# glmanhtu/vit-ed

Hardware: AMD Instinct MI355X
Metric: patch-pairs/sec fwd+bwd, div2k_erosion7_4bin_patch8_64 ViT-ED (higher is better)
Workload: dtype bf16

## Files before the change

include/vited.h:

```cpp
#ifndef VITED_H
#define VITED_H

#include <stdint.h>

#ifdef __cplusplus
extern "C" {
#endif

#define VITED_ABI_VERSION 1

#define VITED_OK 0
#define VITED_ERR_BAD_ARG 1
#define VITED_ERR_UNSUPPORTED 2
#define VITED_ERR_LAUNCH 3
#define VITED_ERR_WORKSPACE 4

#define VITED_F32 0
#define VITED_BF16 1
#define VITED_F16 2
#define VITED_I32 3
#define VITED_I64 4

#define VITED_EPI_STORE 0
#define VITED_EPI_GELU 1
#define VITED_EPI_RESIDUAL 2
#define VITED_EPI_MUL_GELU_GRAD 3
#define VITED_EPI_STORE_F32 4
#define VITED_EPI_MUL 5
#define VITED_EPI_GELU_GRAD 6

#define VITED_B_NK 0
#define VITED_B_KN 1

int vited_abi_version(void);
const char* vited_strerror(int code);

int vited_last_gemm_path(void);
int vited_last_attention_path(void);


int vited_cast(const void* src, int src_dtype, void* dst, int dst_dtype, int64_t n, void* stream);

int vited_cast_transpose(const float* src, void* dst, int dst_dtype, int64_t rows, int64_t cols, void* stream);

int vited_cast_weights(const int64_t* desc, int count, int64_t total_tiles, void* stream);

int vited_patchify(const float* img, int64_t img_bs, const int64_t* batch_index, void* out, int out_dtype,
                   int64_t batch, int chans, int img_size, int patch, void* stream);

int vited_patchify_u8(const uint8_t* img, int64_t img_bs, const int64_t* batch_index, void* out, int out_dtype,
                      int64_t batch, int chans, int img_size, int patch, const float* mean, const float* std, void* stream);

int vited_crop_pairs_u8(const uint8_t* src, int64_t src_bs, const int* cells, const int* erode, uint8_t* out, int64_t batch,
                        int chans, int img_size, void* stream);

int vited_div2k_regions_u8(const uint8_t* store, const int64_t* img_off, const int* img_hw, int n_images, const int* image,
                           const int* flags, const double* minv, const float* rgb, const int* crop, uint8_t* out, int64_t batch,
                           int img_size, void* stream);

int vited_hisfrag_windows_u8(const uint8_t* store, const int64_t* img_off, const int* img_hw, int n_images, const int* image,
                             const int* flags, const int64_t* afix, const double* minv, const int* origin, uint8_t* out, int64_t batch,
                             int img_size, void* stream);

int vited_hisfrag_jitter_u8(const uint8_t* in, const int* flags, const int* order, const float* factors, const int* hue, int64_t* sums,
                            uint8_t* out, int64_t batch, int img_size, void* stream);

int vited_hisfrag_blur_u8(const uint8_t* in, const int* flags, const float* weights, uint8_t* out, int64_t batch, int img_size,
                          void* stream);

int vited_michigan_windows_u8(const uint8_t* store, const int64_t* img_off, const int* img_hw, int n_images, const int* image,
                              const int* flags, const int* origin, const int* x0, const int* kx, const int* y0, const int* ky,
                              const int* holes, const int* n_holes, uint8_t* out, int64_t batch, int img_size, void* stream);

int vited_michigan_blur_gray_u8(const uint8_t* in, const int* flags, const int* weights, uint8_t* out, int64_t batch, int img_size,
                                void* stream);

int vited_slice_rows_cast(const float* in, void* out, int out_dtype, int64_t batch, int64_t in_rows,
                          int64_t row_offset, int64_t rows, int64_t dim, void* stream);

int vited_write_cls_row(float* x, const float* cls, const float* pos, int64_t batch, int64_t rows_per_batch,
                        int64_t dim, void* stream);

int64_t vited_sum_rows_workspace_bytes(int64_t batch, int64_t width);
int vited_sum_rows(const void* in, int in_dtype, int64_t in_ld, float* out, int64_t batch, int64_t width,
                   float* workspace, int64_t workspace_bytes, void* stream);


int vited_layernorm_fwd(const float* x, int64_t x_ld, const float* gamma, const float* beta, void* y,
                        int y_dtype, int64_t y_ld, float* mean, float* rstd, int64_t rows, int64_t dim,
                        float eps, void* stream);

int64_t vited_layernorm_bwd_workspace_bytes(int64_t rows, int64_t dim);
int vited_layernorm_bwd(const void* dy, int dy_dtype, int64_t dy_ld, const float* x, int64_t x_ld,
                        const float* gamma, const float* mean, const float* rstd, const float* dx_in,
                        int64_t dx_in_ld, float* dx_out, int64_t dx_out_ld, void* dx_lp, int dx_lp_dtype,
                        int64_t dx_lp_ld, float* dgamma, float* dbeta, int accumulate, int64_t rows, int64_t dim,
                        float* workspace, int64_t workspace_bytes, void* stream);

int vited_layernorm_bwd_scaled(const void* dy, int dy_dtype, int64_t dy_ld, const float* x, int64_t x_ld,
                               const float* gamma, const float* mean, const float* rstd, const float* dx_in,
                               int64_t dx_in_ld, float* dx_out, int64_t dx_out_ld, void* dx_lp, int dx_lp_dtype,
                               int64_t dx_lp_ld, const float* lp_scale, float* dgamma, float* dbeta, int accumulate,
                               int64_t rows, int64_t dim, float* workspace, int64_t workspace_bytes, void* stream);

int vited_scale_rows_cast(const float* src, int64_t src_ld, const float* row_scale, void* dst, int dst_dtype, int64_t dst_ld,
                          int64_t rows, int64_t dim, void* stream);


int vited_gemm(const void* A, int64_t lda, const void* B, int64_t ldb, int b_layout, int dtype, int64_t M,
               int64_t N, int64_t K, int epilogue, const float* bias, const void* aux,
               const float* residual, void* out, void* out2, int64_t ldo, int64_t rows_per_batch,
               int64_t out_rows_per_batch, int64_t row_offset, int residual_bcast, void* stream);

int vited_gemm_scaled(const void* A, int64_t lda, const void* B, int64_t ldb, int b_layout, int dtype, int64_t M, int64_t N,
                      int64_t K, const float* bias, const float* residual, const float* row_scale, float* out, int64_t ldo,
                      void* stream);

int64_t vited_linear_bwd_weight_workspace_bytes(int64_t M, int64_t N, int64_t K);
int vited_linear_bwd_weight(const void* dY, int64_t lddy, const void* X, int64_t ldx, int dtype, int64_t M,
                            int64_t N, int64_t K, float* dW, float* dbias, int accumulate, float* workspace,
                            int64_t workspace_bytes, void* stream);

int vited_linear_bwd_weight_batched_supported(int count, const int64_t* M, const int64_t* N, const int64_t* K, int dtype);
int64_t vited_linear_bwd_weight_batched_workspace_bytes(int count, const int64_t* M, const int64_t* N, const int64_t* K);
int vited_linear_bwd_weight_batched(int count, const void* const* dY, const int64_t* lddy, const void* const* X,
                                    const int64_t* ldx, const int64_t* M, const int64_t* N, const int64_t* K, float* const* dW,
                                    float* const* dbias, int dtype, int accumulate, float* workspace, int64_t workspace_bytes,
                                    void* stream);

int vited_linear_layernorm_supported(int64_t M, int64_t N, int64_t K);

int vited_linear_residual_layernorm_fwd(const void* a, int64_t lda, const void* w, int64_t ldw, const float* bias,
                                        const float* residual, int64_t ldr, float* y, int64_t ldy, const float* gamma,
                                        const float* beta, float eps, void* h, int64_t ldh, float* mean, float* rstd,
                                        int64_t M, int64_t N, int64_t K, void* stream);

int vited_linear_residual_layernorm_fwd_scaled(const void* a, int64_t lda, const void* w, int64_t ldw, const float* bias,
                                               const float* residual, int64_t ldr, const float* row_scale, float* y, int64_t ldy,
                                               const float* gamma, const float* beta, float eps, void* h, int64_t ldh, float* mean,
                                               float* rstd, int64_t M, int64_t N, int64_t K, void* stream);

int vited_linear_layernorm_bwd_segmented(const void* dy, int64_t lddy, int64_t seg_k, int64_t seg_stride, int64_t segments,
                                         const void* wt, int64_t ldwt, const float* x, int64_t ldx, const float* gamma,
                                         const float* mean, const float* rstd, const float* dx_in, int64_t dx_in_ld,
                                         float* dx_out, int64_t dx_out_ld, void* dx_lp, int64_t dx_lp_ld, float* dgamma,
                                         float* dbeta, int accumulate, int64_t M, int64_t N, float* workspace,
                                         int64_t workspace_bytes, void* stream);
int64_t vited_linear_layernorm_bwd_partial_rows(int64_t M);
int vited_layernorm_bwd_finish_batched(int count, const float* const* partial, const int* nparts, float* const* dgamma,
                                       float* const* dbeta, const int* accumulate, int64_t dim, void* stream);
int64_t vited_linear_layernorm_bwd_workspace_bytes(int64_t M, int64_t N);
int vited_linear_layernorm_bwd(const void* dy, int64_t lddy, const void* wt, int64_t ldwt, const float* x, int64_t ldx,
                               const float* gamma, const float* mean, const float* rstd, const float* dx_in,
                               int64_t dx_in_ld, float* dx_out, int64_t dx_out_ld, void* dx_lp, int64_t dx_lp_ld,
                               float* dgamma, float* dbeta, int accumulate, int64_t M, int64_t N, int64_t K,
                               float* workspace, int64_t workspace_bytes, void* stream);

int vited_linear_layernorm_bwd_scaled(const void* dy, int64_t lddy, const void* wt, int64_t ldwt, const float* x, int64_t ldx,
                                      const float* gamma, const float* mean, const float* rstd, const float* dx_in,
                                      int64_t dx_in_ld, float* dx_out, int64_t dx_out_ld, void* dx_lp, int64_t dx_lp_ld,
                                      const float* lp_scale, float* dgamma, float* dbeta, int accumulate, int64_t M, int64_t N,
                                      int64_t K, float* workspace, int64_t workspace_bytes, void* stream);

int vited_fold_context_weights(int count, const float* const* w, const float* const* bias, const float* const* gamma,
                               const float* const* beta, int64_t N, int64_t K, void* w_out, void* wt_out, float* bias_out,
                               void* stream);
int vited_unfold_context_grads(int count, const float* dwf, const float* dbf, const float* const* w, const float* const* gamma,
                               const float* const* beta, float* const* dw, float* const* dbias, float* const* dgamma, float* const* dbeta, int64_t N,
                               int64_t K, int accumulate, void* stream);


int vited_mlp_fwd(const float* x, int64_t ldx, const float* gamma, const float* beta, const void* w1, const float* b1,
                  const void* w2, const float* b2, float* y, int64_t ldy, void* h, void* gd, void* u, float* mean,
                  float* rstd, int64_t rows, int64_t dim, int64_t hidden, float eps, void* stream);

int64_t vited_block_workspace_bytes(int64_t batch, int64_t tokens, int64_t dim, int64_t hidden, int heads);
int vited_block_fwd(const float* x, float* y, int64_t batch, int64_t tokens, int64_t dim, int heads, int64_t hidden,
                    const float* ln1_g, const float* ln1_b, const void* wqkv, const float* bqkv, const void* wproj,
                    const float* bproj, const float* ln2_g, const float* ln2_b, const void* w1, const float* b1,
                    const void* w2, const float* b2, float eps, void* workspace, int64_t workspace_bytes, void* stream);

int64_t vited_cross_block_workspace_bytes(int64_t batch, int64_t tokens, int64_t ctx_tokens, int64_t dim, int64_t hidden, int heads);
int vited_cross_block_fwd(const float* x, const float* context, float* y, int64_t batch, int64_t tokens, int64_t ctx_tokens,
                          int64_t dim, int heads, int64_t hidden, const float* ln1_g, const float* ln1_b, const void* wqkv,
                          const float* bqkv, const void* wproj, const float* bproj, const float* lnq_g, const float* lnq_b,
                          const float* lnc_g, const float* lnc_b, const void* wq, const float* bq, const void* wkv,
                          const float* bkv, const void* wcproj, const float* bcproj, const float* ln2_g, const float* ln2_b,
                          const void* w1, const float* b1, const void* w2, const float* b2, float eps, void* workspace,
                          int64_t workspace_bytes, void* stream);


int64_t vited_adamw_workspace_bytes(void);
int vited_adamw_step(const int64_t* desc, int count, int64_t total_tiles, const float* grad_flat, int64_t grad_numel,
                     float* hyper, float max_norm, int zero_grad, float* norm_out, float* workspace,
                     int64_t workspace_bytes, void* stream);

int vited_sgd_step(const int64_t* desc, int count, int64_t total_tiles, const float* grad_flat, int64_t grad_numel,
                   float* hyper, float max_norm, int zero_grad, float* norm_out, float* workspace,
                   int64_t workspace_bytes, void* stream);


int vited_attention_fwd(const void* q, int64_t q_bs, int64_t q_ts, const void* k, int64_t k_bs, int64_t k_ts,
                        const void* v, int64_t v_bs, int64_t v_ts, void* o, int64_t o_bs, int64_t o_ts,
                        float* lse, int dtype, int64_t batch, int heads, int64_t nq, int64_t nk, int head_dim,
                        float scale, void* stream);

int vited_attention_fwd_indexed(const void* q, int64_t q_bs, int64_t q_ts, const void* k, int64_t k_bs, int64_t k_ts,
                                const void* v, int64_t v_bs, int64_t v_ts, const int64_t* kv_index, void* o, int64_t o_bs,
                                int64_t o_ts, float* lse, int dtype, int64_t batch, int heads, int64_t nq, int64_t nk,
                                int head_dim, float scale, void* stream);

int vited_attention_bwd(const void* q, int64_t q_bs, int64_t q_ts, const void* k, int64_t k_bs, int64_t k_ts,
                        const void* v, int64_t v_bs, int64_t v_ts, const void* o, const void* d_o,
                        int64_t o_bs, int64_t o_ts, const float* lse, float* delta, void* dq, int64_t dq_bs,
                        int64_t dq_ts, void* dk, int64_t dk_bs, int64_t dk_ts, void* dv, int64_t dv_bs,
                        int64_t dv_ts, int dtype, int64_t batch, int heads, int64_t nq, int64_t nk,
                        int head_dim, float scale, void* stream);

int64_t vited_attention_bwd_indexed_workspace_bytes(int dtype, int64_t batch, int heads, int64_t nk, int head_dim);
int vited_attention_bwd_indexed(const void* q, int64_t q_bs, int64_t q_ts, const void* k, int64_t k_bs, int64_t k_ts,
                                const void* v, int64_t v_bs, int64_t v_ts, const int64_t* kv_index, const int64_t* seg_order,
                                const int64_t* seg_offsets, int64_t kv_items, const void* o, const void* d_o, int64_t o_bs,
                                int64_t o_ts, const float* lse, float* delta, void* dq, int64_t dq_bs, int64_t dq_ts, void* dk,
                                int64_t dk_bs, int64_t dk_ts, void* dv, int64_t dv_bs, int64_t dv_ts, int dtype, int64_t batch,
                                int heads, int64_t nq, int64_t nk, int head_dim, float scale, void* workspace,
                                int64_t workspace_bytes, void* stream);

enum { VITED_CAM_GRAD = 0, VITED_CAM_PROB = 1 };
int vited_attention_cam(const void* q, int64_t q_bs, int64_t q_ts, const void* k, int64_t k_bs, int64_t k_ts,
                        const void* v, int64_t v_bs, int64_t v_ts, const void* d_o, int64_t do_bs, int64_t do_ts,
                        const float* lse, const float* head_weight, float* cam, int64_t cam_bs, int64_t cam_ld,
                        int mode, int dtype, int64_t batch, int heads, int64_t nq, int64_t nk, int head_dim,
                        float scale, void* stream);


int vited_retrieval_metrics(const void* D, int dtype, int64_t ld, int64_t n, int64_t r0, int64_t r1, const int* labels,
                            const int* offsets, const int* members, int num_classes, int remove_self_column, int from_similarity,
                            double* rows_out, double* sums, void* stream);


int vited_group_retrieval_metrics(const void* D, int dtype, int64_t ld, int64_t n, int64_t r0, int64_t r1, const int* labels,
                                  int num_labels, const int* col_offsets, const int* col_members, const int* pos_offsets,
                                  const int* pos_labels, const int* neg_offsets, const int* neg_labels, const int* ks, int nk,
                                  double* rows_out, double* sums, void* stream);


// ... 29 lines not shown
```

vit-ed_amd/csrc/context_fold.hip:

```cpp
#include "common.h"

#define CF_MAX_BLOCKS 16

struct FoldArgs {
    const float* w[CF_MAX_BLOCKS];
    const float* bias[CF_MAX_BLOCKS];
    const float* gamma[CF_MAX_BLOCKS];
    const float* beta[CF_MAX_BLOCKS];
    bf16* w_out;
    bf16* wt_out;
    float* bias_out;
    int count, N, K;
};

__global__ void __launch_bounds__(256) fold_context_kernel(const FoldArgs a) {
    const int lane = threadIdx.x & 63;
    const int row = blockIdx.x * 4 + (threadIdx.x >> 6);
    if (row >= a.count * a.N) return;
    const int l = row / a.N, n = row - l * a.N;
    const float* __restrict__ w = a.w[l] + (int64_t)n * a.K;
    const float* __restrict__ g = a.gamma[l];
    const float* __restrict__ be = a.beta[l];
    const int64_t ldt = (int64_t)a.count * a.N;
    float dot = 0.f;
    for (int k = lane; k < a.K; k += 64) {
        const float wv = w[k];
        const bf16 f = (bf16)(wv * g[k]);
        a.w_out[(int64_t)row * a.K + k] = f;
        a.wt_out[(int64_t)k * ldt + row] = f;
        dot = fmaf(wv, be[k], dot);
    }
    dot = wave_sum(dot);
    if (lane == 0) a.bias_out[row] = dot + (a.bias[l] ? a.bias[l][n] : 0.f);
}

extern "C" int vited_fold_context_weights(int count, const float* const* w, const float* const* bias, const float* const* gamma,
                                          const float* const* beta, int64_t N, int64_t K, void* w_out, void* wt_out, float* bias_out,
                                          void* stream) {
    if (count < 1 || count > CF_MAX_BLOCKS || !w || !bias || !gamma || !beta || !w_out || !wt_out || !bias_out || N <= 0 || K <= 0)
        return VITED_ERR_BAD_ARG;
    FoldArgs a = {};
    for (int i = 0; i < count; ++i) {
        if (!w[i] || !gamma[i] || !beta[i]) return VITED_ERR_BAD_ARG;
        a.w[i] = w[i]; a.bias[i] = bias[i]; a.gamma[i] = gamma[i]; a.beta[i] = beta[i];
    }
    a.w_out = (bf16*)w_out; a.wt_out = (bf16*)wt_out; a.bias_out = bias_out;
    a.count = count; a.N = (int)N; a.K = (int)K;
    hipLaunchKernelGGL(fold_context_kernel, dim3((unsigned)ceil_div64((int64_t)count * N, 4)), dim3(256), 0, (hipStream_t)stream, a);
    return vited_check_launch();
}

struct UnfoldArgs {
    const float* w[CF_MAX_BLOCKS];
    const float* gamma[CF_MAX_BLOCKS];
    const float* beta[CF_MAX_BLOCKS];
    float* dw[CF_MAX_BLOCKS];
    float* dbias[CF_MAX_BLOCKS];
    float* dgamma[CF_MAX_BLOCKS];
    float* dbeta[CF_MAX_BLOCKS];
    const float* dwf;
    const float* dbf;
    int count, N, K, accumulate;
};

#define UF_GROUPS 16
__global__ void __launch_bounds__(64 * UF_GROUPS) unfold_context_kernel(const UnfoldArgs a) {
    __shared__ float red[2][UF_GROUPS][64];
    const int l = blockIdx.y, kx = threadIdx.x & 63, ng = threadIdx.x >> 6;
    const int k = blockIdx.x * 64 + kx;
    const bool ok = k < a.K;
    const float* __restrict__ w = a.w[l];
    const float* __restrict__ dwf = a.dwf + (int64_t)l * a.N * a.K;
    const float* __restrict__ dbf = a.dbf + (int64_t)l * a.N;
    float* __restrict__ dw = a.dw[l];
    const float g = ok ? a.gamma[l][k] : 0.f, be = ok ? a.beta[l][k] : 0.f;
    float sg = 0.f, sb = 0.f;
#pragma unroll 4
    for (int n = ng; n < a.N; n += UF_GROUPS) {
        if (ok) {
            const int64_t o = (int64_t)n * a.K + k;
            const float d = dwf[o], wv = w[o], dbn = dbf[n];
            sg = fmaf(d, wv, sg);
            sb = fmaf(dbn, wv, sb);
            const float v = fmaf(d, g, dbn * be);
            dw[o] = a.accumulate ? dw[o] + v : v;
        }
    }
    red[0][ng][kx] = sg;
    red[1][ng][kx] = sb;
    __syncthreads();
    if (ng == 0 && ok) {
        float tg = 0.f, tb = 0.f;
#pragma unroll
        for (int w = 0; w < UF_GROUPS; ++w) {
            tg += red[0][w][kx];
            tb += red[1][w][kx];
        }
        a.dgamma[l][k] = a.accumulate ? a.dgamma[l][k] + tg : tg;
        a.dbeta[l][k] = a.accumulate ? a.dbeta[l][k] + tb : tb;
    }
    if (blockIdx.x == 0 && a.dbias[l]) {
        for (int n = threadIdx.x; n < a.N; n += 64 * UF_GROUPS) a.dbias[l][n] = a.accumulate ? a.dbias[l][n] + dbf[n] : dbf[n];
    }
}

extern "C" int vited_unfold_context_grads(int count, const float* dwf, const float* dbf, const float* const* w, const float* const* gamma,
                                          const float* const* beta, float* const* dw, float* const* dbias, float* const* dgamma, float* const* dbeta, int64_t N,
                                          int64_t K, int accumulate, void* stream) {
    if (count < 1 || count > CF_MAX_BLOCKS || !dwf || !dbf || !w || !gamma || !beta || !dw || !dbias || !dgamma || !dbeta || N <= 0 || K <= 0)
        return VITED_ERR_BAD_ARG;
    UnfoldArgs a = {};
    for (int i = 0; i < count; ++i) {
        if (!w[i] || !gamma[i] || !beta[i] || !dw[i] || !dgamma[i] || !dbeta[i]) return VITED_ERR_BAD_ARG;
        a.w[i] = w[i]; a.gamma[i] = gamma[i]; a.beta[i] = beta[i]; a.dw[i] = dw[i]; a.dbias[i] = dbias[i]; a.dgamma[i] = dgamma[i]; a.dbeta[i] = dbeta[i];
    }
    a.dwf = dwf; a.dbf = dbf; a.count = count; a.N = (int)N; a.K = (int)K; a.accumulate = accumulate;
    hipLaunchKernelGGL(unfold_context_kernel, dim3((unsigned)ceil_div64(K, 64), (unsigned)count), dim3(64 * UF_GROUPS), 0, (hipStream_t)stream, a);
    return vited_check_launch();
}
```

vit-ed_amd/csrc/elementwise.hip:

```cpp
#include "common.h"

template <typename S, typename D>
__global__ void cast_kernel(const S* __restrict__ src, D* __restrict__ dst, int64_t n) {
    int64_t i = ((int64_t)blockIdx.x * blockDim.x + threadIdx.x) * 4;
    const int64_t stride = (int64_t)gridDim.x * blockDim.x * 4;
    for (; i + 3 < n; i += stride) {
        S a = src[i], b = src[i + 1], c = src[i + 2], d = src[i + 3];
        dst[i] = from_f32<D>(to_f32(a));
        dst[i + 1] = from_f32<D>(to_f32(b));
        dst[i + 2] = from_f32<D>(to_f32(c));
        dst[i + 3] = from_f32<D>(to_f32(d));
    }
    for (; i < n; ++i) dst[i] = from_f32<D>(to_f32(src[i]));
}

extern "C" int vited_cast(const void* src, int src_dtype, void* dst, int dst_dtype, int64_t n, void* stream) {
    if (!src || !dst || n < 0) return VITED_ERR_BAD_ARG;
    if (n == 0) return VITED_OK;
    hipStream_t s = (hipStream_t)stream;
    const int threads = 256;
    int64_t blocks = ceil_div64(n, threads * 4);
    if (blocks > 4096) blocks = 4096;
    if (src_dtype == VITED_F32 && dst_dtype == VITED_BF16)
        hipLaunchKernelGGL((cast_kernel<float, bf16>), dim3(blocks), dim3(threads), 0, s, (const float*)src, (bf16*)dst, n);
// ... 84 lines not shown
        const int mid = (lo + hi + 1) >> 1;
        if (desc[(int64_t)mid * WS_DESC_WORDS + 5] <= blk) lo = mid; else hi = mid - 1;
    }
    const int64_t* d = desc + (int64_t)lo * WS_DESC_WORDS;
    const float* __restrict__ src = (const float*)d[0];
    bf16* __restrict__ dst = (bf16*)d[1];
    bf16* __restrict__ dst_t = (bf16*)d[2];
    const int64_t rows = d[3], cols = d[4];
    const int64_t t = blk - d[5], tiles_c = (cols + 63) >> 6;
    const int64_t r0 = (t / tiles_c) << 6, c0 = (t % tiles_c) << 6;
    const int tx = threadIdx.x & 15, ty = threadIdx.x >> 4;
    const bool vec = (cols & 3) == 0;
#pragma unroll
    for (int j = 0; j < 4; ++j) {
        const int lr = ty + 16 * j;
        const int64_t r = r0 + lr, c = c0 + tx * 4;
        float v[4] = {0.f, 0.f, 0.f, 0.f};
        if (r < rows) {
            if (vec && c + 3 < cols) {
                const f32x4 q = *(const f32x4*)(src + r * cols + c);
                v[0] = q[0]; v[1] = q[1]; v[2] = q[2]; v[3] = q[3];
            } else {
#pragma unroll
                for (int e = 0; e < 4; ++e) if (c + e < cols) v[e] = src[r * cols + c + e];
            }
        }
        bf16 b[4];
#pragma unroll
        for (int e = 0; e < 4; ++e) { b[e] = (bf16)v[e]; tile[lr][tx * 4 + e] = b[e]; }
        if (dst && r < rows) {
            if (vec && c + 3 < cols) *(bf16x4*)(dst + r * cols + c) = bf16x4{b[0], b[1], b[2], b[3]};
            else {
#pragma unroll
                for (int e = 0; e < 4; ++e) if (c + e < cols) dst[r * cols + c + e] = b[e];
            }
        }
    }
    if (!dst_t) return;
    __syncthreads();
    const bool vec_t = (rows & 3) == 0;
#pragma unroll
    for (int j = 0; j < 4; ++j) {
        const int lc = ty + 16 * j;
        const int64_t c = c0 + lc, r = r0 + tx * 4;
        if (c >= cols) continue;
        bf16 b[4];
#pragma unroll
        for (int e = 0; e < 4; ++e) b[e] = tile[tx * 4 + e][lc];
        if (vec_t && r + 3 < rows) *(bf16x4*)(dst_t + c * rows + r) = bf16x4{b[0], b[1], b[2], b[3]};
        else {
#pragma unroll
            for (int e = 0; e < 4; ++e) if (r + e < rows) dst_t[c * rows + r + e] = b[e];
        }
    }
}

extern "C" int vited_cast_weights(const int64_t* desc, int count, int64_t total_tiles, void* stream) {
    if (!desc || count <= 0 || total_tiles <= 0 || total_tiles > 0x7fffffff) return VITED_ERR_BAD_ARG;
    hipLaunchKernelGGL(cast_weights_kernel, dim3((unsigned)total_tiles), dim3(256), 0, (hipStream_t)stream, desc, count);
    return vited_check_launch();
}

template <typename D>
__global__ void patchify_kernel(const float* __restrict__ img, int64_t img_bs, const int64_t* __restrict__ bidx,
                                D* __restrict__ out, int chans, int S, int p) {
    const int G = S / p;
    const int64_t b = blockIdx.y;
    const int py = blockIdx.x;
    const int64_t src_b = bidx ? bidx[b] : b;
    const float* base = img + src_b * img_bs;
    const int Kp = chans * p * p;
    const int total = chans * p * S;
    D* obase = out + (b * G * G + (int64_t)py * G) * Kp;
    for (int e = threadIdx.x; e < total; e += blockDim.x) {
        const int x = e % S;
        const int ci = e / S;
        const int i = ci % p, c = ci / p;
        const float v = base[((int64_t)c * S + (py * p + i)) * S + x];
        const int px = x / p, j = x - px * p;
        obase[(int64_t)px * Kp + (c * p + i) * p + j] = from_f32<D>(v);
    }
}

extern "C" int vited_patchify(const float* img, int64_t img_bs, const int64_t* batch_index, void* out, int out_dtype,
                              int64_t batch, int chans, int img_size, int patch, void* stream) {
    if (!img || !out || batch <= 0 || chans <= 0 || img_size <= 0 || patch <= 0 || img_size % patch) return VITED_ERR_BAD_ARG;
    dim3 grid(img_size / patch, (unsigned)batch);
    hipStream_t s = (hipStream_t)stream;
    if (out_dtype == VITED_BF16)
        hipLaunchKernelGGL((patchify_kernel<bf16>), grid, dim3(256), 0, s, img, img_bs, batch_index, (bf16*)out, chans, img_size, patch);
    else if (out_dtype == VITED_F32)
        hipLaunchKernelGGL((patchify_kernel<float>), grid, dim3(256), 0, s, img, img_bs, batch_index, (float*)out, chans, img_size, patch);
    else
        return VITED_ERR_UNSUPPORTED;
    return vited_check_launch();
}

struct U8Norm { float scale[4], shift[4]; };

template <typename D>
__global__ void patchify_u8_kernel(const uint8_t* __restrict__ img, int64_t img_bs, const int64_t* __restrict__ bidx,
                                   D* __restrict__ out, int chans, int S, int p, U8Norm nrm) {
    const int G = S / p;
    const int64_t b = blockIdx.y;
    const int py = blockIdx.x;
    const int64_t src_b = bidx ? bidx[b] : b;
    const uint8_t* base = img + src_b * img_bs;
    const int Kp = chans * p * p;
    const int total = chans * p * S;
    D* obase = out + (b * G * G + (int64_t)py * G) * Kp;
    for (int e = threadIdx.x; e < total; e += blockDim.x) {
        const int x = e % S;
        const int ci = e / S;
        const int i = ci % p, c = ci / p;
        const float v = fmaf((float)base[((int64_t)c * S + (py * p + i)) * S + x], nrm.scale[c], nrm.shift[c]);
        const int px = x / p, j = x - px * p;
        obase[(int64_t)px * Kp + (c * p + i) * p + j] = from_f32<D>(v);
    }
}

extern "C" int vited_patchify_u8(const uint8_t* img, int64_t img_bs, const int64_t* batch_index, void* out, int out_dtype,
                                 int64_t batch, int chans, int img_size, int patch, const float* mean, const float* std,
                                 void* stream) {
    if (!img || !out || !mean || !std || batch <= 0 || chans <= 0 || chans > 4 || img_size <= 0 || patch <= 0 || img_size % patch)
        return VITED_ERR_BAD_ARG;
    U8Norm nrm = {};
    for (int c = 0; c < chans; ++c) {
        if (!(std[c] > 0.f)) return VITED_ERR_BAD_ARG;
        nrm.scale[c] = 1.0f / (255.0f * std[c]);
        nrm.shift[c] = -mean[c] / std[c];
    }
    dim3 grid(img_size / patch, (unsigned)batch);
    hipStream_t s = (hipStream_t)stream;
    if (out_dtype == VITED_BF16)
        hipLaunchKernelGGL((patchify_u8_kernel<bf16>), grid, dim3(256), 0, s, img, img_bs, batch_index, (bf16*)out, chans, img_size, patch, nrm);
    else if (out_dtype == VITED_F32)
        hipLaunchKernelGGL((patchify_u8_kernel<float>), grid, dim3(256), 0, s, img, img_bs, batch_index, (float*)out, chans, img_size, patch, nrm);
    else
        return VITED_ERR_UNSUPPORTED;
    return vited_check_launch();
}

struct ResampleTaps {
    int x0, n;
    int k0, k1;
};

__device__ __forceinline__ ResampleTaps resample_taps(int xx, int in_size, int out_size) {
    constexpr int PRECISION_BITS = 32 - 8 - 2;
    const double scale = (double)in_size / (double)out_size;
    const double center = (xx + 0.5) * scale;
    int xmin = (int)(center - 1.0 + 0.5);
    xmin = xmin < 0 ? 0 : xmin;
    int xmax = (int)(center + 1.0 + 0.5);
    xmax = (xmax < in_size ? xmax : in_size) - xmin;
    double w0 = 1.0 - fabs((double)xmin - center + 0.5), w1 = xmax > 1 ? 1.0 - fabs((double)xmin + 1.0 - center + 0.5) : 0.0;
    w0 = w0 < 0.0 ? 0.0 : w0;
    w1 = w1 < 0.0 ? 0.0 : w1;
    const double ww = w0 + w1;
    ResampleTaps t;
    t.x0 = xmin;
    t.n = xmax > 1 ? 2 : 1;
    t.k0 = (int)(0.5 + (w0 / ww) * (double)(1 << PRECISION_BITS));
    t.k1 = (int)(0.5 + (w1 / ww) * (double)(1 << PRECISION_BITS));
    return t;
}

__device__ __forceinline__ int resample_px(int p0, int p1, const ResampleTaps& t) {
    constexpr int PRECISION_BITS = 32 - 8 - 2;
    int acc = (1 << (PRECISION_BITS - 1)) + p0 * t.k0 + (t.n > 1 ? p1 * t.k1 : 0);
    acc >>= PRECISION_BITS;
    return acc < 0 ? 0 : (acc > 255 ? 255 : acc);
}

__global__ void __launch_bounds__(256)
crop_pairs_u8_kernel(const uint8_t* __restrict__ src, int64_t src_bs, const int* __restrict__ cells, const int* __restrict__ erode,
                     uint8_t* __restrict__ out, int chans, int S) {
    const int64_t b = blockIdx.z;
    const int img = blockIdx.y / chans, c = blockIdx.y % chans;
    int cell = cells[b * 2 + img], e = erode[b];
    cell = cell < 0 ? 0 : (cell > 5 ? 5 : cell);
    e = e < 1 ? 1 : (e > S ? S : e);
    const int off = (int)rint((S - e) / 2.0);
    const int r0 = (cell / 3) * S + off, c0 = (cell % 3) * S + off;
    const uint8_t* base = src + b * src_bs + ((int64_t)c * 2 * S + r0) * (3 * S) + c0;
    uint8_t* o = out + (((b * 2 + img) * chans + c) * (int64_t)S) * S;
    for (int i = blockIdx.x * blockDim.x + threadIdx.x; i < S * S; i += gridDim.x * blockDim.x) {
        const int y = i / S, x = i - y * S;
        const ResampleTaps tx = resample_taps(x, e, S), ty = resample_taps(y, e, S);
        const uint8_t* ra = base + (int64_t)ty.x0 * (3 * S) + tx.x0;
        const int h0 = resample_px(ra[0], tx.n > 1 ? ra[1] : 0, tx);
        int h1 = 0;
        if (ty.n > 1) {
            const uint8_t* rb = ra + 3 * S;
            h1 = resample_px(rb[0], tx.n > 1 ? rb[1] : 0, tx);
        }
        o[i] = (uint8_t)resample_px(h0, h1, ty);
    }
}

extern "C" int vited_crop_pairs_u8(const uint8_t* src, int64_t src_bs, const int* cells, const int* erode, uint8_t* out, int64_t batch,
                                   int chans, int img_size, void* stream) {
    if (!src || !cells || !erode || !out || batch <= 0 || chans <= 0 || img_size <= 0 || batch > 65535) return VITED_ERR_BAD_ARG;
    if (src_bs < (int64_t)chans * 6 * img_size * img_size) return VITED_ERR_BAD_ARG;
    const int per = img_size * img_size;
    dim3 grid((unsigned)((per + 1023) / 1024 < 8 ? (per + 1023) / 1024 : 8), (unsigned)(2 * chans), (unsigned)batch);
    hipLaunchKernelGGL(crop_pairs_u8_kernel, grid, dim3(256), 0, (hipStream_t)stream, src, src_bs, cells, erode, out, chans, img_size);
    return vited_check_launch();
}

template <typename D>
__global__ void slice_rows_cast_kernel(const float* __restrict__ in, D* __restrict__ out, int64_t in_rows,
                                       int64_t row_offset, int64_t rows, int64_t dim, int64_t total) {
    int64_t i = (int64_t)blockIdx.x * blockDim.x + threadIdx.x;
    const int64_t stride = (int64_t)gridDim.x * blockDim.x;
    const int64_t per_b = rows * dim;
    for (; i < total; i += stride) {
        const int64_t b = i / per_b, rem = i - b * per_b;
        out[i] = from_f32<D>(in[(b * in_rows + row_offset) * dim + rem]);
    }
}

extern "C" int vited_slice_rows_cast(const float* in, void* out, int out_dtype, int64_t batch, int64_t in_rows,
                                     int64_t row_offset, int64_t rows, int64_t dim, void* stream) {
    if (!in || !out || batch <= 0 || rows <= 0 || dim <= 0 || row_offset < 0 || row_offset + rows > in_rows) return VITED_ERR_BAD_ARG;
    const int64_t total = batch * rows * dim;
    int64_t blocks = ceil_div64(total, 256);
    if (blocks > 8192) blocks = 8192;
    hipStream_t s = (hipStream_t)stream;
    if (out_dtype == VITED_BF16)
        hipLaunchKernelGGL((slice_rows_cast_kernel<bf16>), dim3(blocks), dim3(256), 0, s, in, (bf16*)out, in_rows, row_offset, rows, dim, total);
    else if (out_dtype == VITED_F32)
        hipLaunchKernelGGL((slice_rows_cast_kernel<float>), dim3(blocks), dim3(256), 0, s, in, (float*)out, in_rows, row_offset, rows, dim, total);
    else
        return VITED_ERR_UNSUPPORTED;
    return vited_check_launch();
}

__global__ void write_cls_row_kernel(float* __restrict__ x, const float* __restrict__ cls, const float* __restrict__ pos,
                                     int64_t batch, int64_t rows_per_batch, int64_t dim) {
    int64_t i = (int64_t)blockIdx.x * blockDim.x + threadIdx.x;
    const int64_t total = batch * dim;
    if (i >= total) return;
    const int64_t b = i / dim, d = i - b * dim;
    x[b * rows_per_batch * dim + d] = cls[d] + pos[d];
}

extern "C" int vited_write_cls_row(float* x, const float* cls, const float* pos, int64_t batch, int64_t rows_per_batch,
                                   int64_t dim, void* stream) {
    if (!x || !cls || !pos || batch <= 0 || rows_per_batch <= 0 || dim <= 0) return VITED_ERR_BAD_ARG;
    const int64_t total = batch * dim;
    hipLaunchKernelGGL(write_cls_row_kernel, dim3((unsigned)ceil_div64(total, 256)), dim3(256), 0, (hipStream_t)stream,
                       x, cls, pos, batch, rows_per_batch, dim);
    return vited_check_launch();
}

template <typename S_>
__global__ void sum_rows_kernel(const S_* __restrict__ in, int64_t in_ld, float* __restrict__ out, int64_t batch,
                                int64_t width, int64_t rows_per_split) {
    const int64_t r = (int64_t)blockIdx.x * blockDim.x + threadIdx.x;
    if (r >= width) return;
    const int64_t b0 = (int64_t)blockIdx.y * rows_per_split;
    int64_t b1 = b0 + rows_per_split;
    if (b1 > batch) b1 = batch;
    float acc0 = 0.f, acc1 = 0.f, acc2 = 0.f, acc3 = 0.f;
    int64_t b = b0;
    for (; b + 3 < b1; b += 4) {
        acc0 += to_f32(in[b * in_ld + r]);
        acc1 += to_f32(in[(b + 1) * in_ld + r]);
        acc2 += to_f32(in[(b + 2) * in_ld + r]);
        acc3 += to_f32(in[(b + 3) * in_ld + r]);
    }
    for (; b < b1; ++b) acc0 += to_f32(in[b * in_ld + r]);
    out[(int64_t)blockIdx.y * width + r] = (acc0 + acc1) + (acc2 + acc3);
}

static inline int64_t sum_rows_splits(int64_t batch, int64_t width) {
    const int64_t col_blocks = ceil_div64(width, 256);
    int64_t s = ceil_div64(1024, col_blocks);
    const int64_t max_s = ceil_div64(batch, 16);
    if (s > max_s) s = max_s;
    if (s < 1) s = 1;
    return s;
}

extern "C" int64_t vited_sum_rows_workspace_bytes(int64_t batch, int64_t width) {
    return sum_rows_splits(batch, width) * width * (int64_t)sizeof(float);
}

extern "C" int vited_sum_rows(const void* in, int in_dtype, int64_t in_ld, float* out, int64_t batch, int64_t width,
                              float* workspace, int64_t workspace_bytes, void* stream) {
    if (!in || !out || batch <= 0 || width <= 0 || in_ld < width) return VITED_ERR_BAD_ARG;
    const int64_t S = sum_rows_splits(batch, width);
    hipStream_t s = (hipStream_t)stream;
    const unsigned col_blocks = (unsigned)ceil_div64(width, 256);
    float* pass1_out = out;
    if (S > 1) {
        if (!workspace || workspace_bytes < S * width * (int64_t)sizeof(float)) return VITED_ERR_WORKSPACE;
        pass1_out = workspace;
    }
    const int64_t rps = ceil_div64(batch, S);
    if (in_dtype == VITED_F32)
        hipLaunchKernelGGL((sum_rows_kernel<float>), dim3(col_blocks, (unsigned)S), dim3(256), 0, s, (const float*)in, in_ld, pass1_out, batch, width, rps);
    else if (in_dtype == VITED_BF16)
        hipLaunchKernelGGL((sum_rows_kernel<bf16>), dim3(col_blocks, (unsigned)S), dim3(256), 0, s, (const bf16*)in, in_ld, pass1_out, batch, width, rps);
    else
        return VITED_ERR_UNSUPPORTED;
    if (S > 1)
        hipLaunchKernelGGL((sum_rows_kernel<float>), dim3(col_blocks, 1), dim3(256), 0, s, (const float*)workspace, width, out, S, width, S);
    return vited_check_launch();
}

__device__ __forceinline__ void sum_slabs_body(const float* __restrict__ in, int64_t in_ld, float* __restrict__ out, int64_t batch,
                                               int64_t width, int accumulate, int64_t r) {
    if (r >= width) return;
    if (r + 3 < width) {
        f32x4 acc = accumulate ? *(const f32x4*)(out + r) : f32x4{0.f, 0.f, 0.f, 0.f};
        int64_t b = 0;
        for (; b + 4 <= batch; b += 4) {
// ... 133 lines not shown
```

vit-ed_amd/csrc/gemm.hip:

```cpp
#include <stdlib.h>
#include <string.h>

#include "gemm_kernels.h"

static thread_local int g_last_gemm_path = 0;
extern "C" int vited_last_gemm_path(void) { return g_last_gemm_path; }

static int gemm_impl(const void* A, int64_t lda, const void* B, int64_t ldb, int b_layout, int dtype, int64_t M, int64_t N, int64_t K,
                     int epilogue, const float* bias, const void* aux, const float* residual, void* out, void* out2, int64_t ldo,
                     int64_t rows_per_batch, int64_t out_rows_per_batch, int64_t row_offset, int residual_bcast,
                     const float* row_scale, void* stream) {
    if (!A || !B || !out || M <= 0 || N <= 0 || K <= 0 || lda < K || ldo < N) return VITED_ERR_BAD_ARG;
    if (b_layout != VITED_B_NK && b_layout != VITED_B_KN) return VITED_ERR_BAD_ARG;
    if (ldb < (b_layout == VITED_B_NK ? K : N)) return VITED_ERR_BAD_ARG;
    if (epilogue < VITED_EPI_STORE || epilogue > VITED_EPI_GELU_GRAD) return VITED_ERR_BAD_ARG;
    if ((epilogue == VITED_EPI_GELU || epilogue == VITED_EPI_GELU_GRAD) && !out2) return VITED_ERR_BAD_ARG;
    if (epilogue == VITED_EPI_RESIDUAL && !residual) return VITED_ERR_BAD_ARG;
    if ((epilogue == VITED_EPI_MUL_GELU_GRAD || epilogue == VITED_EPI_MUL) && !aux) return VITED_ERR_BAD_ARG;
    if (rows_per_batch < 0 || (rows_per_batch > 0 && (out_rows_per_batch < rows_per_batch + row_offset || row_offset < 0)))
        return VITED_ERR_BAD_ARG;
    if (row_scale) {
        if (epilogue != VITED_EPI_RESIDUAL || rows_per_batch != 0) return VITED_ERR_BAD_ARG;
        epilogue = EPI_RESIDUAL_SCALED;
    }
// ... 47 lines not shown

extern "C" int64_t vited_linear_bwd_weight_workspace_bytes(int64_t M, int64_t N, int64_t K) {
    const int64_t s = max64(tn_portable_splits(M, N, K), gemm_tn_mfma_splits(M, N, K));
    return (s * N * K + s * N + N) * (int64_t)sizeof(float) + vited_sum_rows_workspace_bytes(M, N) + 256;
}

extern "C" int vited_linear_bwd_weight(const void* dY, int64_t lddy, const void* X, int64_t ldx, int dtype, int64_t M,
                                       int64_t N, int64_t K, float* dW, float* dbias, int accumulate, float* workspace,
                                       int64_t workspace_bytes, void* stream) {
    if (!dY || !X || !dW || M <= 0 || N <= 0 || K <= 0 || lddy < N || ldx < K) return VITED_ERR_BAD_ARG;
    if (dtype != VITED_F32 && dtype != VITED_BF16) return VITED_ERR_UNSUPPORTED;
    if (!workspace || workspace_bytes < vited_linear_bwd_weight_workspace_bytes(M, N, K)) return VITED_ERR_WORKSPACE;
    hipStream_t s = (hipStream_t)stream;
    const bool mfma = dtype == VITED_BF16 && gemm_tn_mfma_supported(dY, lddy, X, ldx, M, N, K);
    const int64_t splits = mfma ? gemm_tn_mfma_splits(M, N, K) : tn_portable_splits(M, N, K);
    const bool via_slabs = splits > 1 || accumulate;
    float* slab = via_slabs ? workspace : dW;
    float* bias_tmp = workspace + splits * N * K;
    int rc;
    if (mfma) {
        g_last_gemm_path = 2;
        float* bias_slab = !dbias ? nullptr : (via_slabs ? bias_tmp : dbias);
        rc = gemm_tn_mfma(dY, lddy, X, ldx, M, N, K, splits, slab, bias_slab, s);
        if (rc != VITED_OK) return rc;
        if (via_slabs) {
            rc = dbias ? sum_slabs_pair(workspace, N * K, dW, N * K, bias_slab, N, dbias, N, splits, s, accumulate)
                       : sum_rows_f32_single_pass(workspace, N * K, dW, splits, N * K, s, accumulate);
        }
        return rc;
    }
    g_last_gemm_path = 1;
    rc = gemm_tn_portable(dY, lddy, X, ldx, dtype, M, N, K, splits, slab, s);
    if (rc != VITED_OK) return rc;
    if (via_slabs) {
        rc = sum_rows_f32_single_pass(workspace, N * K, dW, splits, N * K, s, accumulate);
        if (rc != VITED_OK) return rc;
    }
    if (dbias) {
        float* ws2 = bias_tmp + N;
        const int64_t ws2_bytes = workspace_bytes - (splits * N * K + N) * (int64_t)sizeof(float);
        if (accumulate) {
            rc = vited_sum_rows(dY, dtype, lddy, bias_tmp, M, N, ws2, ws2_bytes, stream);
            if (rc == VITED_OK) rc = sum_rows_f32_single_pass(bias_tmp, N, dbias, 1, N, s, 1);
        } else {
            rc = vited_sum_rows(dY, dtype, lddy, dbias, M, N, ws2, ws2_bytes, stream);
        }
    }
    return rc;
}

extern "C" int vited_linear_bwd_weight_batched_supported(int count, const int64_t* M, const int64_t* N, const int64_t* K, int dtype) {
    return dtype == VITED_BF16 && gemm_tn_batch_supported(count, M, N, K) ? 1 : 0;
}

extern "C" int64_t vited_linear_bwd_weight_batched_workspace_bytes(int count, const int64_t* M, const int64_t* N, const int64_t* K) {
    if (!gemm_tn_batch_supported(count, M, N, K)) return 0;
    int64_t splits, ws, bs;
    gemm_tn_batch_layout(count, M, N, K, &splits, &ws, &bs);
    return splits * (ws + bs) * (int64_t)sizeof(float) + 256;
}

extern "C" int vited_linear_bwd_weight_batched(int count, const void* const* dY, const int64_t* lddy, const void* const* X,
                                               const int64_t* ldx, const int64_t* M, const int64_t* N, const int64_t* K,
                                               float* const* dW, float* const* dbias, int dtype, int accumulate, float* workspace,
                                               int64_t workspace_bytes, void* stream) {
    if (count < 1 || !dY || !lddy || !X || !ldx || !M || !N || !K || !dW || !dbias || !workspace) return VITED_ERR_BAD_ARG;
    if (dtype != VITED_BF16 || !gemm_tn_batch_supported(count, M, N, K)) return VITED_ERR_UNSUPPORTED;
    if (workspace_bytes < vited_linear_bwd_weight_batched_workspace_bytes(count, M, N, K)) return VITED_ERR_WORKSPACE;
    int64_t splits, ws, bs;
    gemm_tn_batch_layout(count, M, N, K, &splits, &ws, &bs);
    int has_bias[40];
    int64_t widths[40], nbias[40];
    for (int i = 0; i < count; ++i) {
        if (!dY[i] || !X[i] || !dW[i] || lddy[i] < N[i] || ldx[i] < K[i]) return VITED_ERR_BAD_ARG;
        has_bias[i] = dbias[i] != nullptr;
        widths[i] = N[i] * K[i];
        nbias[i] = N[i];
    }
    float* base = (float*)(((uintptr_t)workspace + 15) & ~(uintptr_t)15);
    float* slabs = base;
    float* bias_slabs = base + splits * ws;
    hipStream_t s = (hipStream_t)stream;
    g_last_gemm_path = 2;
    int rc = gemm_tn_batch(count, dY, lddy, X, ldx, M, N, K, has_bias, slabs, bias_slabs, s);
    if (rc != VITED_OK) return rc;
    return sum_slabs_batch(count, slabs, ws, bias_slabs, bs, splits, widths, dW, nbias, dbias, accumulate, s);
}
```

vit-ed_amd/csrc/gemm_kernels.h:

```cpp
#pragma once
#include "gemm_epilogue.h"

int gemm_portable(const void* A, int64_t lda, const void* B, int64_t ldb, int b_layout, int dtype, int64_t M, int64_t N,
                  int64_t K, int epilogue, const EpiParams& ep, hipStream_t s);
int gemm_tn_portable(const void* dY, int64_t lddy, const void* X, int64_t ldx, int dtype, int64_t M, int64_t N, int64_t K,
                     int64_t splits, float* out, hipStream_t s);

bool gemm_nt_mfma_supported(const void* A, int64_t lda, const void* B, int64_t ldb, int64_t M, int64_t N, int64_t K,
                            int epilogue, const EpiParams& ep);
int gemm_nt_mfma(const void* A, int64_t lda, const void* B, int64_t ldb, int64_t M, int64_t N, int64_t K, int epilogue,
                 const EpiParams& ep, hipStream_t s);
bool gemm_nt_areg_supported(int64_t ldw, int64_t M, int64_t N, int64_t K, int epilogue);
int gemm_nt_areg(const void* A, int64_t lda, const void* W, int64_t ldw, int64_t M, int64_t N, int epilogue, int waves,
                 const EpiParams& ep, hipStream_t s);
bool gemm_tn_mfma_supported(const void* dY, int64_t lddy, const void* X, int64_t ldx, int64_t M, int64_t N, int64_t K);
int64_t gemm_tn_mfma_splits(int64_t M, int64_t N, int64_t K);
int gemm_tn_mfma(const void* dY, int64_t lddy, const void* X, int64_t ldx, int64_t M, int64_t N, int64_t K, int64_t splits,
                 float* out, float* bias_out , hipStream_t s);

bool gemm_tn_batch_supported(int count, const int64_t* M, const int64_t* N, const int64_t* K);
void gemm_tn_batch_layout(int count, const int64_t* M, const int64_t* N, const int64_t* K, int64_t* splits, int64_t* slab_stride,
                          int64_t* bias_stride);
int gemm_tn_batch(int count, const void* const* dY, const int64_t* lddy, const void* const* X, const int64_t* ldx, const int64_t* M,
                  const int64_t* N, const int64_t* K, const int* has_bias, float* slabs, float* bias_slabs, hipStream_t s);
int sum_slabs_batch(int count, const float* slabs, int64_t slab_stride, const float* bias_slabs, int64_t bias_stride, int64_t splits,
                    const int64_t* widths, float* const* dW, const int64_t* nbias, float* const* dbias, int accumulate, hipStream_t s);

int sum_rows_f32_single_pass(const float* in, int64_t in_ld, float* out, int64_t batch, int64_t width, hipStream_t s,
                             int accumulate = 0);
int sum_slabs_pair(const float* in_a, int64_t ld_a, float* out_a, int64_t width_a, const float* in_b, int64_t ld_b, float* out_b,
                   int64_t width_b, int64_t batch, hipStream_t s, int accumulate);
```

vit-ed_amd/csrc/gemm_mfma.hip:

```cpp
#include <stdlib.h>

#include <mutex>

#include "gemm_kernels.h"
#include "gemm_nt_epilogue.h"
#include "gemm_lds.h"

template <int BKT, int WM, bool ASM_DMA = false>
__device__ __forceinline__ void nt_stage_load(const bf16* __restrict__ A, int64_t lda, const bf16* __restrict__ B,
                                              int64_t ldb, int64_t m0, int64_t n0, int64_t M, int64_t N, int64_t k0,
                                              char* stage, int wave, int lane) {
    using C = NtCfg<BKT, WM>;
    const int rsub = lane / C::CHUNKS, cp = lane % C::CHUNKS;
#ifndef NT_DBG_NO_A_DMA
#pragma unroll
    for (int i = 0; i < 32 / C::ROWS_PER_DMA; ++i) {
        const int r = wave * 32 + i * C::ROWS_PER_DMA + rsub;
        const int c = cp ^ C::swz(r);
        int64_t gm = m0 + r;
        gm = gm < M ? gm : M - 1;
        const bf16* asrc = A + gm * lda + k0 + c * 8;
        if constexpr (ASM_DMA) glds16_asm(asrc, stage + (wave * 32 + i * C::ROWS_PER_DMA) * C::ROW_BYTES);
        else glds16(asrc, stage + (wave * 32 + i * C::ROWS_PER_DMA) * C::ROW_BYTES);
    }
// ... 376 lines not shown
                for (int i = 0; i < 4; ++i) {
#pragma unroll
                    for (int e = 0; e < 4; ++e)
                        bsum[i] = __builtin_amdgcn_fdot2_f32_bf16(bf16x2_t{af[i][2 * e], af[i][2 * e + 1]}, one2, bsum[i], false);
                }
            }
        }
    }
    float* o = out + (int64_t)split * N * K;
    const int fr = lane & 15, fq = lane >> 4;
#pragma unroll
    for (int i = 0; i < 4; ++i) {
#pragma unroll
        for (int j = 0; j < 4; ++j) {
            const int64_t n = n0 + wr * 64 + i * 16 + fr;
            const int64_t k = kc0 + wc * 64 + j * 16 + fq * 4;
#ifdef TN_DBG_NO_STORE
            asm volatile("" ::"v"(acc[i][j]));
#else
            if (n < N && k < K) *(f32x4*)(o + n * K + k) = acc[i][j];
#endif
        }
    }
    if constexpr (BIAS) {
        if (kc0 == 0 && wc == 0) {
            float* bo = bias_out + (int64_t)split * N;
#pragma unroll
            for (int i = 0; i < 4; ++i) {
                float v = bsum[i];
                v += __shfl_xor(v, 16);
                v += __shfl_xor(v, 32);
                const int64_t n = n0 + wr * 64 + i * 16 + fr;
                if (fq == 0 && n < N) bo[n] = v;
            }
        }
    }
}

#define TW_STAGES 4
#define TW_PANEL_BYTES (32 * 256)
#define TW_STAGE_BYTES (4 * TW_PANEL_BYTES)
#define TW_PER 4

__device__ __forceinline__ void tw_stage_issue(const bf16* const (&src)[4], char* stage, int panel, int rbase) {
#pragma unroll
    for (int i = 0; i < 4; ++i) glds16_asm(src[i], stage + panel * TW_PANEL_BYTES + (rbase + i * 4) * 256);
}

struct TwFrags {
    bf16x8 a[4], b[6];
};

__device__ __forceinline__ void tw_read_frags(TwFrags& f, const char* st, const int (&ya_lo)[4], const int (&ya_hi)[4],
                                              const int (&xb_lo)[6], const int (&xb_hi)[6]) {
#pragma unroll
    for (int i = 0; i < 4; ++i) {
        const bf16x4 lo = tr_read(st + ya_lo[i]);
        const bf16x4 hi = tr_read(st + ya_hi[i]);
        f.a[i] = bf16x8{lo[0], lo[1], lo[2], lo[3], hi[0], hi[1], hi[2], hi[3]};
    }
#pragma unroll
    for (int j = 0; j < 6; ++j) {
        const bf16x4 lo = tr_read(st + xb_lo[j]);
        const bf16x4 hi = tr_read(st + xb_hi[j]);
        f.b[j] = bf16x8{lo[0], lo[1], lo[2], lo[3], hi[0], hi[1], hi[2], hi[3]};
    }
}

#define TW_MAX_PROBLEMS 40
struct TwProblem {
    const bf16* dY;
    const bf16* X;
    int64_t lddy, ldx, M, rows_per_split;
    int64_t slab_off, bias_off;
    int N, K, tiles_k, tile0;
    int has_bias, pad_;
};
struct TwBatch {
    TwProblem p[TW_MAX_PROBLEMS];
    int64_t slab_stride, bias_stride;
    int count, total_tiles;
};

template <bool BIAS>
__global__ void __launch_bounds__(512)
gemm_tn_wide_kernel(const TwBatch batch, float* __restrict__ out_base, float* __restrict__ bias_base) {
    extern __shared__ __attribute__((aligned(16))) char smem[];
    const int lane = threadIdx.x & 63;
    const int wave = __builtin_amdgcn_readfirstlane(threadIdx.x >> 6);
    const int wr = wave >> 2, wc = wave & 3;
    const int ntile = batch.total_tiles;
    const int lin = xcd_remap(blockIdx.x + blockIdx.y * ntile, ntile * gridDim.y);
    const int split = lin / ntile;
    int tile_id = lin - split * ntile;
    int pi = 0;
    for (int i = 1; i < batch.count; ++i)
        if (batch.p[i].tile0 <= tile_id) pi = i;
    const TwProblem& pr = batch.p[pi];
    tile_id -= pr.tile0;
    const bf16* __restrict__ dY = pr.dY;
    const bf16* __restrict__ X = pr.X;
    const int64_t lddy = pr.lddy, ldx = pr.ldx, M = pr.M, N = pr.N, K = pr.K, rows_per_split = pr.rows_per_split;
    const int tiles_k = pr.tiles_k;
    const bool with_bias = BIAS && pr.has_bias;
    float* __restrict__ out = out_base + pr.slab_off;
    float* __restrict__ bias_out = bias_base + pr.bias_off;
    const int64_t n0 = (int64_t)(tile_id / tiles_k) * 128, kc0 = (int64_t)(tile_id % tiles_k) * 384;
    const int64_t mb = (int64_t)split * rows_per_split;
    int64_t me = mb + rows_per_split;
    me = me < M ? me : M;
    const int nsteps = me > mb ? (int)((me - mb + 31) / 32) : 0;

    f32x4 acc[4][6];
    float bsum[4] = {0.f, 0.f, 0.f, 0.f};
#pragma unroll
    for (int i = 0; i < 4; ++i) {
#pragma unroll
        for (int j = 0; j < 6; ++j) acc[i][j] = f32x4{0.f, 0.f, 0.f, 0.f};
    }

    const int panel = wave >> 1, rbase = (wave & 1) * 16;
    const int rsub = lane >> 4, cp = lane & 15;
    const bf16* const pbase = panel == 0 ? dY : X;
    const int64_t ld = panel == 0 ? lddy : ldx;
    const int64_t col0 = panel == 0 ? n0 : kc0 + (panel - 1) * 128;
    const int64_t colmax = panel == 0 ? N - 8 : col0 + 120;
    int64_t coff[4];
#pragma unroll
    for (int i = 0; i < 4; ++i) {
        int64_t c = col0 + ((cp ^ tn_f(rbase + i * 4 + rsub)) << 3);
        coff[i] = c <= colmax ? c : colmax;
    }
    const bf16* p0[4];
#pragma unroll
    for (int i = 0; i < 4; ++i) p0[i] = pbase + (mb + rbase + i * 4 + rsub) * ld + coff[i];
    const int64_t stage_stride = 32 * ld;
    const int rows_here = (int)(me - mb);
    auto issue = [&](int stage_idx) {
        char* dst = smem + (stage_idx & (TW_STAGES - 1)) * TW_STAGE_BYTES;
        if ((stage_idx + 1) * 32 <= rows_here) {
            const int64_t adv = (int64_t)stage_idx * stage_stride;
            const bf16* src[4];
#pragma unroll
            for (int i = 0; i < 4; ++i) src[i] = p0[i] + adv;
            tw_stage_issue(src, dst, panel, rbase);
        } else {
            const bf16* src[4];
#pragma unroll
            for (int i = 0; i < 4; ++i) {
                int r = stage_idx * 32 + rbase + i * 4 + rsub;
                r = r < rows_here ? r : rows_here - 1;
                src[i] = pbase + (mb + r) * ld + coff[i];
            }
            tw_stage_issue(src, dst, panel, rbase);
        }
    };
    auto wait_landed = [&](int idx) {
        const int later = (nsteps - 1 < idx + TW_STAGES - 2 ? nsteps - 1 : idx + TW_STAGES - 2) - idx;
        if (later >= 3 && TW_STAGES > 4) asm volatile("s_waitcnt vmcnt(%0)" ::"n"(3 * TW_PER) : "memory");
        else if (later >= 2) asm volatile("s_waitcnt vmcnt(%0)" ::"n"(2 * TW_PER) : "memory");
        else if (later == 1) asm volatile("s_waitcnt vmcnt(%0)" ::"n"(TW_PER) : "memory");
        else asm volatile("s_waitcnt vmcnt(0)" ::: "memory");
        if ((idx + 1) * 32 > rows_here) {
            char* st = smem + (idx & (TW_STAGES - 1)) * TW_STAGE_BYTES;
#pragma unroll
            for (int i = 0; i < 4; ++i) {
                const int r = rbase + i * 4 + rsub;
                if (idx * 32 + r >= rows_here) *(f32x4*)(st + panel * TW_PANEL_BYTES + r * 256 + cp * 16) = f32x4{0.f, 0.f, 0.f, 0.f};
            }
        }
    };

    const int g = lane >> 4, q = (lane & 15) >> 2, p = lane & 3;
    const int r_lo = 8 * g + q, r_hi = r_lo + 4;
    const int f_lo = tn_f(r_lo), f_hi = tn_f(r_hi);
    int ya_lo[4], ya_hi[4], xb_lo[6], xb_hi[6];
#pragma unroll
    for (int i = 0; i < 4; ++i) {
        const int ch = ((wr * 64 + i * 16) >> 3) + (p >> 1);
        ya_lo[i] = r_lo * 256 + ((ch ^ f_lo) << 4) + 8 * (p & 1);
        ya_hi[i] = r_hi * 256 + ((ch ^ f_hi) << 4) + 8 * (p & 1);
    }
#pragma unroll
    for (int j = 0; j < 6; ++j) {
        const int col = wc * 96 + j * 16;
        const int ch = ((col & 127) >> 3) + (p >> 1);
        const int base = (1 + (col >> 7)) * TW_PANEL_BYTES;
        xb_lo[j] = base + r_lo * 256 + ((ch ^ f_lo) << 4) + 8 * (p & 1);
        xb_hi[j] = base + r_hi * 256 + ((ch ^ f_hi) << 4) + 8 * (p & 1);
    }

    auto slot_l = [&](int t, TwFrags& f) {
#ifndef TW_DBG_NO_READS
        tw_read_frags(f, smem + (t & (TW_STAGES - 1)) * TW_STAGE_BYTES, ya_lo, ya_hi, xb_lo, xb_hi);
#endif
#ifndef TW_DBG_NO_DMA
        if (t + TW_STAGES - 1 < nsteps) issue(t + TW_STAGES - 1);
#endif
        __builtin_amdgcn_s_waitcnt(0xc07f);
    };
    auto slot_m = [&](const TwFrags& cur) {
        __builtin_amdgcn_s_setprio(1);
#pragma unroll
        for (int j = 0; j < 6; ++j)
#pragma unroll
            for (int i = 0; i < 4; ++i) {
#ifdef TW_DBG_NO_MFMA
                asm volatile("" ::"v"(cur.b[j]), "v"(cur.a[i]));
#else
                acc[i][j] = __builtin_amdgcn_mfma_f32_16x16x32_bf16(cur.b[j], cur.a[i], acc[i][j], 0, 0, 0);
#endif
            }
        __builtin_amdgcn_s_setprio(0);
        if (with_bias && kc0 == 0) {
            typedef __attribute__((ext_vector_type(2))) __bf16 bf16x2_t;
            const bf16x2_t one2 = {(__bf16)1.0f, (__bf16)1.0f};
#pragma unroll
            for (int i = 0; i < 4; ++i) {
#pragma unroll
                for (int e = 0; e < 4; ++e)
                    bsum[i] = __builtin_amdgcn_fdot2_f32_bf16(bf16x2_t{cur.a[i][2 * e], cur.a[i][2 * e + 1]}, one2, bsum[i], false);
            }
        }
    };
    auto barrier = [&]() {
        __builtin_amdgcn_s_barrier();
        asm volatile("" ::: "memory");
    };
    auto certify_barrier = [&](int idx) {
        __builtin_amdgcn_sched_barrier(0);
        if (idx < nsteps) {
            wait_landed(idx);
            asm volatile("s_waitcnt lgkmcnt(0)" ::: "memory");
        }
        barrier();
    };

    if (nsteps > 0) {
#pragma unroll
        for (int pre = 0; pre < TW_STAGES - 1; ++pre)
            if (nsteps > pre) issue(pre);
        certify_barrier(0);
        TwFrags f;
        if (wr == 0) {
            for (int t = 0; t < nsteps; ++t) {
                slot_l(t, f);
                barrier();
                slot_m(f);
                certify_barrier(t + 1);
            }
            barrier();
        } else {
            barrier();
            for (int t = 0; t < nsteps; ++t) {
                slot_l(t, f);
                certify_barrier(t + 1);
                slot_m(f);
                barrier();
            }
        }
    }

    float* o = out + (int64_t)split * batch.slab_stride;
    const int fr = lane & 15, fq = lane >> 4;
#pragma unroll
    for (int i = 0; i < 4; ++i) {
        const int64_t n = n0 + wr * 64 + i * 16 + fr;
#pragma unroll
        for (int j = 0; j < 6; ++j) {
            const int64_t k = kc0 + wc * 96 + j * 16 + fq * 4;
            if (n < N) *(f32x4*)(o + n * K + k) = acc[i][j];
        }
    }
    if constexpr (BIAS) {
        if (with_bias && kc0 == 0 && wc == 0) {
            float* bo = bias_out + (int64_t)split * batch.bias_stride;
#pragma unroll
            for (int i = 0; i < 4; ++i) {
                float v = bsum[i];
                v += __shfl_xor(v, 16);
                v += __shfl_xor(v, 32);
                const int64_t n = n0 + wr * 64 + i * 16 + fr;
                if (fq == 0 && n < N) bo[n] = v;
            }
        }
    }
}

bool gemm_tn_mfma_supported(const void* dY, int64_t lddy, const void* X, int64_t ldx, int64_t M, int64_t N, int64_t K) {
    auto al16 = [](const void* p) { return ((uintptr_t)p & 15) == 0; };
    return N % 8 == 0 && K % 8 == 0 && N >= 8 && K >= 8 && lddy % 8 == 0 && ldx % 8 == 0 && al16(dY) && al16(X) && M >= 1;
}

static inline bool tn_use_ring(int64_t M, int64_t N, int64_t K) {
    if (TN_FORCE_TM) return TN_FORCE_STAGES >= 3;
#ifdef VITED_TUNING
    static const char* env = getenv("VITED_TN_RING");
    if (env) return atoi(env) != 0;
#endif
    return N * K >= 1536 * 384 && M >= 16384;
}

static inline bool tn_use_wide(int64_t M, int64_t N, int64_t K) {
    if (TN_FORCE_TM) return false;
    if (K % 384 != 0) return false;
#ifdef VITED_TUNING
    static const char* env = getenv("VITED_TN_WIDE");
    if (env) return atoi(env) != 0;
#endif
    return M >= 4096;
}

int64_t gemm_tn_mfma_splits(int64_t M, int64_t N, int64_t K) {
    if (tn_use_wide(M, N, K)) {
        const int64_t tiles = ceil_div64(N, 128) * (K / 384);
        int64_t slots = 256;
#ifdef VITED_TUNING
        static const int64_t slots_env = getenv("VITED_TN_WIDE_SLOTS") ? atoi(getenv("VITED_TN_WIDE_SLOTS")) : 0;
        if (slots_env) slots = slots_env;
#endif
        int64_t s = slots / tiles;
        const int64_t max_s = ceil_div64(M, 256);
        if (s > max_s) s = max_s;
        if (s < 1) s = 1;
        const int64_t rps = ceil_div64(ceil_div64(M, s), 32) * 32;
        return ceil_div64(M, rps);
    }
    const bool ring = tn_use_ring(M, N, K);
    const int tm = TN_FORCE_TM ? TN_FORCE_TM : (ring ? 32 : 64);
    const int64_t tiles = ceil_div64(N, 128) * ceil_div64(K, 128);
    int64_t slots = tm == 64 ? 512 : 768;
#ifdef VITED_TUNING
    static const int64_t slots_env = getenv("VITED_TN_SLOTS") ? atoi(getenv("VITED_TN_SLOTS")) : 0;
    if (slots_env) slots = slots_env;
#endif
    int64_t s = slots / tiles;
    const int64_t max_s = ceil_div64(M, 512);
    if (s > max_s) s = max_s;
    if (s < 1) s = 1;
    const int64_t rps = ceil_div64(ceil_div64(M, s), tm) * tm;
    return ceil_div64(M, rps);
}

template <int TM, int STAGES>
static int launch_tn(const void* dY, int64_t lddy, const void* X, int64_t ldx, int64_t M, int64_t N, int64_t K, int64_t splits,
                      float* out, float* bias_out, hipStream_t s) {
    constexpr int LDS = STAGES * 2 * TM * 128 * 2;
    const int tiles_k = (int)ceil_div64(K, 128);
    const int tiles = (int)ceil_div64(N, 128) * tiles_k;
    const int64_t rps = ceil_div64(ceil_div64(M, splits), TM) * TM;
    if (LDS > 65536) {
        static std::once_flag once;
        static hipError_t status = hipSuccess;
        std::call_once(once, [&] {
            status = hipFuncSetAttribute((const void*)gemm_tn_mfma_kernel<true, TM, STAGES>, hipFuncAttributeMaxDynamicSharedMemorySize, LDS);
            if (status == hipSuccess)
                status = hipFuncSetAttribute((const void*)gemm_tn_mfma_kernel<false, TM, STAGES>, hipFuncAttributeMaxDynamicSharedMemorySize, LDS);
        });
        if (status != hipSuccess) return VITED_ERR_LAUNCH;
    }
    if (bias_out)
        hipLaunchKernelGGL((gemm_tn_mfma_kernel<true, TM, STAGES>), dim3(tiles, (unsigned)splits), dim3(256), LDS, s,
                           (const bf16*)dY, lddy, (const bf16*)X, ldx, M, N, K, rps, tiles_k, out, bias_out);
    else
        hipLaunchKernelGGL((gemm_tn_mfma_kernel<false, TM, STAGES>), dim3(tiles, (unsigned)splits), dim3(256), LDS, s,
                           (const bf16*)dY, lddy, (const bf16*)X, ldx, M, N, K, rps, tiles_k, out, bias_out);
    return VITED_OK;
}

static int launch_tn_wide_batch(const TwBatch& b, int64_t splits, bool any_bias, float* out, float* bias_out, hipStream_t s) {
    constexpr int LDS = TW_STAGES * TW_STAGE_BYTES;
    static std::once_flag once;
    static hipError_t status = hipSuccess;
    std::call_once(once, [&] {
        status = hipFuncSetAttribute((const void*)gemm_tn_wide_kernel<true>, hipFuncAttributeMaxDynamicSharedMemorySize, LDS);
        if (status == hipSuccess)
            status = hipFuncSetAttribute((const void*)gemm_tn_wide_kernel<false>, hipFuncAttributeMaxDynamicSharedMemorySize, LDS);
    });
    if (status != hipSuccess) return VITED_ERR_LAUNCH;
    if (any_bias)
        hipLaunchKernelGGL((gemm_tn_wide_kernel<true>), dim3(b.total_tiles, (unsigned)splits), dim3(512), LDS, s, b, out, bias_out);
    else
        hipLaunchKernelGGL((gemm_tn_wide_kernel<false>), dim3(b.total_tiles, (unsigned)splits), dim3(512), LDS, s, b, out, bias_out);
    return VITED_OK;
}

static int launch_tn_wide(const void* dY, int64_t lddy, const void* X, int64_t ldx, int64_t M, int64_t N, int64_t K, int64_t splits,
                          float* out, float* bias_out, hipStream_t s) {
    TwBatch b = {};
    TwProblem& p = b.p[0];
    p.dY = (const bf16*)dY; p.X = (const bf16*)X; p.lddy = lddy; p.ldx = ldx; p.M = M;
    p.rows_per_split = ceil_div64(ceil_div64(M, splits), 32) * 32;
    p.N = (int)N; p.K = (int)K; p.tiles_k = (int)(K / 384); p.tile0 = 0; p.has_bias = bias_out != nullptr;
    b.count = 1;
    b.total_tiles = (int)ceil_div64(N, 128) * p.tiles_k;
    b.slab_stride = N * K;
    b.bias_stride = N;
    return launch_tn_wide_batch(b, splits, bias_out != nullptr, out, bias_out, s);
}

bool gemm_tn_batch_supported(int count, const int64_t* M, const int64_t* N, const int64_t* K) {
    if (count < 1 || count > TW_MAX_PROBLEMS) return false;
    for (int i = 0; i < count; ++i)
        if (!tn_use_wide(M[i], N[i], K[i]) || N[i] % 8 || N[i] > (1 << 20) || K[i] > (1 << 20)) return false;
    return true;
}

static inline int64_t tn_batch_splits(int count, const int64_t* M, const int64_t* N, const int64_t* K) {
    int64_t tiles = 0, mmin = M[0];
    for (int i = 0; i < count; ++i) {
        tiles += ceil_div64(N[i], 128) * (K[i] / 384);
        mmin = M[i] < mmin ? M[i] : mmin;
    }
    int64_t s = 256 / tiles;
    const int64_t max_s = ceil_div64(mmin, 256);
    if (s > max_s) s = max_s;
    return s < 1 ? 1 : s;
}

void gemm_tn_batch_layout(int count, const int64_t* M, const int64_t* N, const int64_t* K, int64_t* splits, int64_t* slab_stride,
                          int64_t* bias_stride) {
    *splits = tn_batch_splits(count, M, N, K);
    int64_t w = 0, b = 0;
    for (int i = 0; i < count; ++i) {
        w += N[i] * K[i];
        b += N[i];
    }
    *slab_stride = w;
    *bias_stride = b;
}

int gemm_tn_batch(int count, const void* const* dY, const int64_t* lddy, const void* const* X, const int64_t* ldx, const int64_t* M,
                  const int64_t* N, const int64_t* K, const int* has_bias, float* slabs, float* bias_slabs, hipStream_t s) {
    TwBatch b = {};
    int64_t splits;
    gemm_tn_batch_layout(count, M, N, K, &splits, &b.slab_stride, &b.bias_stride);
    int tile = 0;
    int64_t woff = 0, boff = 0;
    bool any_bias = false;
    for (int i = 0; i < count; ++i) {
        TwProblem& p = b.p[i];
        if (!gemm_tn_mfma_supported(dY[i], lddy[i], X[i], ldx[i], M[i], N[i], K[i])) return VITED_ERR_UNSUPPORTED;
        p.dY = (const bf16*)dY[i]; p.X = (const bf16*)X[i]; p.lddy = lddy[i]; p.ldx = ldx[i]; p.M = M[i];
        p.rows_per_split = ceil_div64(ceil_div64(M[i], splits), 32) * 32;
        p.N = (int)N[i]; p.K = (int)K[i]; p.tiles_k = (int)(K[i] / 384); p.tile0 = tile; p.has_bias = has_bias[i];
        p.slab_off = woff; p.bias_off = boff;
        tile += (int)ceil_div64(N[i], 128) * p.tiles_k;
        woff += N[i] * K[i];
        boff += N[i];
        any_bias = any_bias || has_bias[i];
    }
    b.count = count;
    b.total_tiles = tile;
    const int rc = launch_tn_wide_batch(b, splits, any_bias, slabs, bias_slabs, s);
    return rc != VITED_OK ? rc : vited_check_launch();
}

int gemm_tn_mfma(const void* dY, int64_t lddy, const void* X, int64_t ldx, int64_t M, int64_t N, int64_t K, int64_t splits,
                 float* out, float* bias_out, hipStream_t s) {
    int rc;
    if (tn_use_wide(M, N, K)) rc = launch_tn_wide(dY, lddy, X, ldx, M, N, K, splits, out, bias_out, s);
#if TN_FORCE_TM
    else rc = launch_tn<TN_FORCE_TM, TN_FORCE_STAGES>(dY, lddy, X, ldx, M, N, K, splits, out, bias_out, s);
#else
    else if (tn_use_ring(M, N, K)) rc = launch_tn<32, 3>(dY, lddy, X, ldx, M, N, K, splits, out, bias_out, s);
    else rc = launch_tn<64, 2>(dY, lddy, X, ldx, M, N, K, splits, out, bias_out, s);
#endif
    return rc != VITED_OK ? rc : vited_check_launch();
}
```

vit-ed_amd/csrc/gemm_row.hip:

```cpp
#include <mutex>
#include <type_traits>

#include "gemm_kernels.h"
#include "gemm_lds.h"

#define ROW_N 384
#define ROW_LD 388

enum { ROW_MODE_FWD = 0, ROW_MODE_BWD = 1 };

struct RowArgs {
    const bf16* A; int64_t lda;
    int seg_k; int64_t seg_stride;
    const bf16* W; int64_t ldw;
    int64_t M; int K;
    const float* bias; const float* residual; int64_t ldr;
    float* y; int64_t ldy;
    const float* gamma; const float* beta; float eps;
    bf16* h; int64_t ldh; float* mean; float* rstd;
    const float* x; int64_t ldx; const float* mean_in; const float* rstd_in;
    const float* dx_in; int64_t ldxi; float* dx; int64_t lddx; bf16* dx_lp; int64_t ldlp;
    float* partial;
    const float* row_scale;
    const float* lp_scale;
};

template <int MT> struct RowCfg {
    static_assert(MT == 6 || MT == 8 || MT == 9 || MT == 10, "tile heights: 96, 128, 144 or 160 rows");
    static constexpr int BM = 16 * MT;
    static constexpr int A_BYTES = BM * 128;
    static constexpr int W_BYTES = ROW_N * 128;
    static constexpr int W_BASE = 3 * A_BYTES;
    static constexpr int LDS_BYTES = 3 * A_BYTES + 2 * W_BYTES;
    static constexpr int P0 = (MT + 1) / 2;
    static constexpr int A_PIECES = 2 * MT;
    static constexpr int A_J = (A_PIECES + 3) / 4;
    static constexpr int PASS_SUB = MT == 8 ? 4 : MT == 10 ? 5 : 3;
    static constexpr int PASS_ROWS = 16 * PASS_SUB;
    static constexpr int NPASS = MT / PASS_SUB;
    static constexpr int ROWS_PER_HALF = PASS_ROWS / 16;
    static constexpr bool EPI_ALL_ROWS = MT <= 9;
    static_assert(MT % PASS_SUB == 0, "passes cover the tile");
    static_assert(LDS_BYTES <= 160 * 1024, "LDS");
    static_assert(LDS_BYTES >= PASS_ROWS * ROW_LD * 4, "epilogue scratch must fit the staging buffers");
    static_assert(LDS_BYTES >= 16 * 2 * ROW_N * 4, "column-partial combine must fit the staging buffers");
};

__device__ __forceinline__ float row_half_sum(float v) { return half_wave_sum(v); }

#define ROW_STORE(ptr, val) __builtin_nontemporal_store(val, ptr)
#define ROW_STORE_LP(ptr, val) (*(ptr) = (val))
#define ROW_LOAD(ptr) __builtin_nontemporal_load(ptr)

template <int SC> struct RowFwdIn { f32x4 res[3]; float scale[SC]; };
template <int SC> struct RowBwdIn { f32x4 x[3], din[3]; float mu, rs; float lps[SC]; };

template <int MODE, int MT, bool SCALED>
__global__ void __launch_bounds__(512)
gemm_row_kernel(const RowArgs a) {
    extern __shared__ __attribute__((aligned(16))) char smem[];
    using R = RowCfg<MT>;
    const int lane = threadIdx.x & 63;
    const int wave = __builtin_amdgcn_readfirstlane(threadIdx.x >> 6);
    const int64_t m0 = (int64_t)blockIdx.x * R::BM;

    f32x4 acc[MT][3];
#pragma unroll
    for (int i = 0; i < MT; ++i)
#pragma unroll
        for (int j = 0; j < 3; ++j) acc[i][j] = f32x4{0.f, 0.f, 0.f, 0.f};

    const int grp = wave >> 2, u = wave & 3;
    const int nt = a.K / 64;
    const int r8 = lane >> 3, c8 = lane & 7;
    const int cs_even = (c8 ^ (r8 >> 1)) * 8, cs_odd = (c8 ^ (r8 >> 1) ^ 4) * 8;
    const int cs_u = (u & 1) ? cs_odd : cs_even;
    const int a_per = (R::A_PIECES - u + 3) / 4;
    const bf16* pa[R::A_J];
#pragma unroll
    for (int j = 0; j < R::A_J; ++j) {
        int64_t ar = m0 + 8 * (4 * j + u) + r8;
#ifdef ROW_DBG_A_RESIDENT
        ar -= m0;
#endif
        ar = ar < a.M ? ar : a.M - 1;
        pa[j] = a.A + ar * a.lda + cs_u;
    }
    const bf16* pw = a.W + (int64_t)(8 * u + r8) * a.ldw + cs_u;
    auto issue_a = [&](int t) {
#ifdef ROW_DBG_NO_DMA
        return;
#endif
        if (t >= nt) return;
        char* dst = smem + (t % 3) * R::A_BYTES;
        const int k0 = t * 64;
        const int seg = k0 / a.seg_k;
        const int64_t ka = (int64_t)seg * a.seg_stride + (k0 - seg * a.seg_k);
#pragma unroll
        for (int j = 0; j < R::A_J; ++j)
            if (4 * j + 3 < R::A_PIECES || j < a_per) glds16_asm(pa[j] + ka, dst + (4 * j + u) * 1024);
    };
    auto issue_w = [&](int t, int part) {
#ifdef ROW_DBG_NO_DMA
        return;
#endif
        if (t >= nt) return;
        char* dst = smem + R::W_BASE + (t & 1) * R::W_BYTES + (16 * part + u) * 1024;
        const int64_t off = (int64_t)(128 * part) * a.ldw + t * 64;
#pragma unroll
        for (int j = 0; j < 4; ++j) glds16_asm(pw + off + (int64_t)(32 * j) * a.ldw, dst + 4 * j * 1024);
    };
    const int fr = lane & 15, fq = lane >> 4;
    const int loff0 = fr * 128 + ((fq ^ ((fr >> 1) & 7)) << 4), loff1 = fr * 128 + (((4 + fq) ^ ((fr >> 1) & 7)) << 4);
    bf16x8 fa[R::P0][2] = {}, fb[3][2] = {};
    auto read_b = [&](int t) {
#ifdef ROW_DBG_NO_READS
        return;
#endif
        const char* wb = smem + R::W_BASE + (t & 1) * R::W_BYTES + wave * 48 * 128;
#pragma unroll
        for (int j = 0; j < 3; ++j) {
            fb[j][0] = *(const bf16x8*)(wb + j * 2048 + loff0);
            fb[j][1] = *(const bf16x8*)(wb + j * 2048 + loff1);
        }
    };
    auto read_a = [&](int t, auto i0_tag, auto n_tag) {
        constexpr int I0 = decltype(i0_tag)::value, NR = decltype(n_tag)::value;
#ifdef ROW_DBG_NO_READS
        return;
#endif
        const char* ab = smem + (t % 3) * R::A_BYTES + I0 * 2048;
#pragma unroll
        for (int i = 0; i < NR; ++i) {
            fa[i][0] = *(const bf16x8*)(ab + i * 2048 + loff0);
            fa[i][1] = *(const bf16x8*)(ab + i * 2048 + loff1);
        }
    };
    auto mfmas = [&](auto i0_tag, auto n_tag) {
        constexpr int I0 = decltype(i0_tag)::value, NR = decltype(n_tag)::value;
        __builtin_amdgcn_s_setprio(1);
// ... 29 lines not shown
    };
    using I0 = std::integral_constant<int, 0>;
    using IP0 = std::integral_constant<int, R::P0>;
    using IP1 = std::integral_constant<int, MT - R::P0>;
    if (grp == 0) {
        issue_a(0);
        issue_w(0, 1);
        issue_a(1);
        certify_barrier(nt > 1);
        for (int t = 0; t < nt; ++t) {
            read_b(t);
            read_a(t, I0{}, IP0{});
            issue_w(t + 1, 1);
            landed();
            barrier();
            mfmas(I0{}, IP0{});
            barrier();
            read_a(t, IP0{}, IP1{});
            issue_a(t + 2);
            landed();
            barrier();
            mfmas(IP0{}, IP1{});
            certify_barrier(t + 2 < nt);
        }
        barrier();
    } else {
        issue_w(0, 0);
        issue_w(0, 2);
        issue_w(1, 0);
        certify_barrier(nt > 1);
        barrier();
        for (int t = 0; t < nt; ++t) {
            read_b(t);
            read_a(t, I0{}, IP0{});
            issue_w(t + 1, 2);
            landed();
            barrier();
            mfmas(I0{}, IP0{});
            barrier();
            read_a(t, IP0{}, IP1{});
            issue_w(t + 2, 0);
            landed();
            certify_barrier(t + 2 < nt);
            mfmas(IP0{}, IP1{});
            barrier();
        }
    }
#ifdef ROW_DBG_NO_EPI
#pragma unroll
    for (int i = 0; i < MT; ++i)
#pragma unroll
        for (int j = 0; j < 3; ++j) asm volatile("" ::"v"(acc[i][j]));
    return;
#endif

    float* sc = (float*)smem;
    const int hl = lane & 31;
    const int hw = wave * 2 + (lane >> 5);
    const float inv_d = 1.0f / ROW_N;
    f32x4 gm[3], bt[3], bs[3];
#pragma unroll
    for (int j = 0; j < 3; ++j) {
        const int c = (j * 32 + hl) * 4;
        gm[j] = a.gamma ? *(const f32x4*)(a.gamma + c) : f32x4{1.f, 1.f, 1.f, 1.f};
        bt[j] = (MODE == ROW_MODE_FWD && a.beta) ? *(const f32x4*)(a.beta + c) : f32x4{0.f, 0.f, 0.f, 0.f};
        bs[j] = (MODE == ROW_MODE_FWD && a.bias) ? *(const f32x4*)(a.bias + c) : f32x4{0.f, 0.f, 0.f, 0.f};
    }
    f32x4 dg[3], db[3];
#pragma unroll
    for (int j = 0; j < 3; ++j) {
        dg[j] = f32x4{0.f, 0.f, 0.f, 0.f};
        db[j] = f32x4{0.f, 0.f, 0.f, 0.f};
    }
    auto load_fwd = [&](RowFwdIn<SCALED>& in, int64_t m) {
        const bool ok = m < a.M;
        if constexpr (SCALED) in.scale[0] = ok ? a.row_scale[m] : 0.f;
#pragma unroll
        for (int j = 0; j < 3; ++j)
            in.res[j] = ok ? ROW_LOAD((const f32x4*)(a.residual + m * a.ldr + (j * 32 + hl) * 4)) : f32x4{0.f, 0.f, 0.f, 0.f};
    };
    auto load_bwd = [&](RowBwdIn<SCALED>& in, int64_t m) {
        const bool ok = m < a.M;
        if constexpr (SCALED) in.lps[0] = ok ? a.lp_scale[m] : 0.f;
#pragma unroll
        for (int j = 0; j < 3; ++j) {
            const int c = (j * 32 + hl) * 4;
            in.x[j] = ok ? ROW_LOAD((const f32x4*)(a.x + m * a.ldx + c)) : f32x4{0.f, 0.f, 0.f, 0.f};
            in.din[j] = (ok && a.dx_in) ? ROW_LOAD((const f32x4*)(a.dx_in + m * a.ldxi + c)) : f32x4{0.f, 0.f, 0.f, 0.f};
        }
        in.mu = ok ? a.mean_in[m] : 0.f;
        in.rs = ok ? a.rstd_in[m] : 0.f;
    };
    auto row_fwd = [&](const RowFwdIn<SCALED>& in, int r, int64_t m) {
        if (m >= a.M) return;
        f32x4 v[3];
        float s = 0.f;
#pragma unroll
        for (int j = 0; j < 3; ++j) {
            const int c = (j * 32 + hl) * 4;
            v[j] = *(const f32x4*)(sc + r * ROW_LD + c);
#pragma unroll
            for (int e = 0; e < 4; ++e) {
                v[j][e] += bs[j][e];
                if constexpr (SCALED) v[j][e] = in.res[j][e] + in.scale[0] * v[j][e];
                else v[j][e] += in.res[j][e];
            }
            ROW_STORE((f32x4*)(a.y + m * a.ldy + c), v[j]);
            s += (v[j][0] + v[j][1]) + (v[j][2] + v[j][3]);
        }
        if (!a.h) return;
        const float mu = row_half_sum(s) * inv_d;
        float q = 0.f;
#pragma unroll
        for (int j = 0; j < 3; ++j)
#pragma unroll
            for (int e = 0; e < 4; ++e) {
                const float d = v[j][e] - mu;
                q = fmaf(d, d, q);
            }
        const float rs = rsqrtf(row_half_sum(q) * inv_d + a.eps);
#pragma unroll
        for (int j = 0; j < 3; ++j) {
            const int c = (j * 32 + hl) * 4;
            bf16x4 o;
#pragma unroll
            for (int e = 0; e < 4; ++e) o[e] = (bf16)((v[j][e] - mu) * rs * gm[j][e] + bt[j][e]);
            ROW_STORE_LP((bf16x4*)(a.h + m * a.ldh + c), o);
        }
        if (hl == 0) {
            a.mean[m] = mu;
            a.rstd[m] = rs;
        }
    };
    auto row_bwd = [&](const RowBwdIn<SCALED>& in, int r, int64_t m) {
        if (m >= a.M) return;
        f32x4 xh[3], gg[3];
        float s1 = 0.f, s2 = 0.f;
#pragma unroll
        for (int j = 0; j < 3; ++j) {
            const int c = (j * 32 + hl) * 4;
            const f32x4 d = *(const f32x4*)(sc + r * ROW_LD + c);
#pragma unroll
            for (int e = 0; e < 4; ++e) {
                xh[j][e] = (in.x[j][e] - in.mu) * in.rs;
                gg[j][e] = d[e] * gm[j][e];
                s1 += gg[j][e];
                s2 = fmaf(gg[j][e], xh[j][e], s2);
                dg[j][e] = fmaf(d[e], xh[j][e], dg[j][e]);
                db[j][e] += d[e];
            }
        }
        const float c1 = row_half_sum(s1) * inv_d, c2 = row_half_sum(s2) * inv_d;
#pragma unroll
        for (int j = 0; j < 3; ++j) {
            const int c = (j * 32 + hl) * 4;
            f32x4 v;
#pragma unroll
            for (int e = 0; e < 4; ++e) v[e] = in.rs * (gg[j][e] - c1 - xh[j][e] * c2) + in.din[j][e];
            ROW_STORE((f32x4*)(a.dx + m * a.lddx + c), v);
            if constexpr (SCALED) {
#pragma unroll
                for (int e = 0; e < 4; ++e) v[e] *= in.lps[0];
            }
            if (a.dx_lp) ROW_STORE_LP((bf16x4*)(a.dx_lp + m * a.ldlp + c), (bf16x4{(bf16)v[0], (bf16)v[1], (bf16)v[2], (bf16)v[3]}));
        }
    };

#pragma unroll
    for (int p = 0; p < R::NPASS; ++p) {
        const int64_t mp = m0 + p * R::PASS_ROWS;
        constexpr int AHEAD = R::EPI_ALL_ROWS ? R::ROWS_PER_HALF : 1;
        RowFwdIn<SCALED> fin[AHEAD + (R::EPI_ALL_ROWS ? 0 : 1)];
        RowBwdIn<SCALED> bin[AHEAD + (R::EPI_ALL_ROWS ? 0 : 1)];
#pragma unroll
        for (int k = 0; k < AHEAD; ++k) {
            if (MODE == ROW_MODE_FWD) load_fwd(fin[k], mp + hw + 16 * k);
            else load_bwd(bin[k], mp + hw + 16 * k);
        }
        __syncthreads();
#pragma unroll
        for (int ii = 0; ii < R::PASS_SUB; ++ii) {
            const int i = R::PASS_SUB * p + ii;
#pragma unroll
            for (int j = 0; j < 3; ++j) *(f32x4*)(sc + (ii * 16 + fr) * ROW_LD + wave * 48 + j * 16 + fq * 4) = acc[i][j];
        }
        __syncthreads();
#pragma unroll
        for (int k = 0; k < R::ROWS_PER_HALF; ++k) {
            const int r = hw + 16 * k;
            if constexpr (R::EPI_ALL_ROWS) {
                if (MODE == ROW_MODE_FWD) row_fwd(fin[k], r, mp + r);
                else row_bwd(bin[k], r, mp + r);
            } else {
                const bool more = k + 1 < R::ROWS_PER_HALF;
                if (MODE == ROW_MODE_FWD) {
                    if (more) load_fwd(fin[(k + 1) & 1], mp + r + 16);
                    row_fwd(fin[k & 1], r, mp + r);
                } else {
                    if (more) load_bwd(bin[(k + 1) & 1], mp + r + 16);
                    row_bwd(bin[k & 1], r, mp + r);
                }
            }
        }
    }

    if (MODE == ROW_MODE_BWD) {
        __syncthreads();
        float* my = sc + hw * 2 * ROW_N;
#pragma unroll
        for (int j = 0; j < 3; ++j) {
            const int c = (j * 32 + hl) * 4;
            *(f32x4*)(my + c) = dg[j];
            *(f32x4*)(my + ROW_N + c) = db[j];
        }
        __syncthreads();
        float* out = a.partial + (int64_t)blockIdx.x * 2 * ROW_N;
        for (int c = threadIdx.x; c < 2 * ROW_N; c += 512) {
            float s = 0.f;
#pragma unroll
            for (int w = 0; w < 16; ++w) s += sc[w * 2 * ROW_N + c];
            out[c] = s;
        }
    }
}

static inline int row_mt(int64_t M) {
    static const int heights[] = {10, 9, 8, 6};
    int best = 8;
    int64_t cost = -1;
    for (int mt : heights) {
        const int64_t c = ceil_div64(ceil_div64(M, 16 * mt), 256) * mt;
        if (cost < 0 || c < cost) {
            cost = c;
            best = mt;
        }
    }
    return best;
}

static inline int64_t row_tiles(int64_t M) { return ceil_div64(M, 16 * row_mt(M)); }

static bool row_shape_ok(int64_t M, int64_t N, int64_t K) { return N == ROW_N && K >= 64 && K % 64 == 0 && K <= (1 << 20) && M >= 1 && M < ((int64_t)1 << 31); }

extern "C" int vited_linear_layernorm_supported(int64_t M, int64_t N, int64_t K) { return row_shape_ok(M, N, K) ? 1 : 0; }

template <int MODE, int MT, bool SCALED>
static int row_launch_scaled(const RowArgs& a, unsigned tiles, hipStream_t s) {
    auto kernel = gemm_row_kernel<MODE, MT, SCALED>;
    static std::once_flag once;
    static hipError_t status = hipSuccess;
    std::call_once(once, [&] { status = hipFuncSetAttribute((const void*)kernel, hipFuncAttributeMaxDynamicSharedMemorySize, RowCfg<MT>::LDS_BYTES); });
    if (status != hipSuccess) return VITED_ERR_LAUNCH;
    hipLaunchKernelGGL(kernel, dim3(tiles), dim3(512), RowCfg<MT>::LDS_BYTES, s, a);
    return vited_check_launch();
}

template <int MODE, int MT>
static int row_launch_mt(const RowArgs& a, unsigned tiles, hipStream_t s) {
    if (MODE == ROW_MODE_FWD ? a.row_scale != nullptr : a.lp_scale != nullptr) return row_launch_scaled<MODE, MT, true>(a, tiles, s);
    return row_launch_scaled<MODE, MT, false>(a, tiles, s);
}

template <int MODE>
static int row_launch(const RowArgs& a, hipStream_t s) {
    const unsigned tiles = (unsigned)row_tiles(a.M);
    switch (row_mt(a.M)) {
        case 6: return row_launch_mt<MODE, 6>(a, tiles, s);
        case 9: return row_launch_mt<MODE, 9>(a, tiles, s);
        case 10: return row_launch_mt<MODE, 10>(a, tiles, s);
        default: return row_launch_mt<MODE, 8>(a, tiles, s);
    }
}

static inline bool al16(const void* p) { return ((uintptr_t)p & 15) == 0; }

static int linear_residual_layernorm_fwd_impl(const void* a, int64_t lda, const void* w, int64_t ldw, const float* bias,
                                             const float* residual, int64_t ldr, const float* row_scale, float* y, int64_t ldy,
                                             const float* gamma, const float* beta, float eps, void* h, int64_t ldh, float* mean,
                                             float* rstd, int64_t M, int64_t N, int64_t K, void* stream) {
    if (!a || !w || !residual || !y || M <= 0 || N <= 0 || K <= 0 || lda < K || ldw < K || ldr < N || ldy < N) return VITED_ERR_BAD_ARG;
    if (h && (!gamma || !beta || !mean || !rstd || ldh < N)) return VITED_ERR_BAD_ARG;
    if (!row_shape_ok(M, N, K)) return VITED_ERR_UNSUPPORTED;
    if ((lda & 7) || (ldw & 7) || (ldr & 3) || (ldy & 3) || (h && (ldh & 3))) return VITED_ERR_UNSUPPORTED;
    if (!al16(a) || !al16(w) || !al16(residual) || !al16(y) || !al16(bias) || !al16(gamma) || !al16(beta) || ((uintptr_t)h & 7))
        return VITED_ERR_BAD_ARG;
    RowArgs r = {};
    r.A = (const bf16*)a; r.lda = lda; r.seg_k = (int)K; r.seg_stride = 0; r.W = (const bf16*)w; r.ldw = ldw; r.M = M; r.K = (int)K;
    r.bias = bias; r.residual = residual; r.ldr = ldr; r.y = y; r.ldy = ldy;
    r.gamma = gamma; r.beta = beta; r.eps = eps; r.h = (bf16*)h; r.ldh = ldh; r.mean = mean; r.rstd = rstd;
    r.row_scale = row_scale;
    return row_launch<ROW_MODE_FWD>(r, (hipStream_t)stream);
}

extern "C" int vited_linear_residual_layernorm_fwd(const void* a, int64_t lda, const void* w, int64_t ldw, const float* bias,
                                                   const float* residual, int64_t ldr, float* y, int64_t ldy, const float* gamma,
                                                   const float* beta, float eps, void* h, int64_t ldh, float* mean, float* rstd,
                                                   int64_t M, int64_t N, int64_t K, void* stream) {
    return linear_residual_layernorm_fwd_impl(a, lda, w, ldw, bias, residual, ldr, nullptr, y, ldy, gamma, beta, eps, h, ldh, mean, rstd,
                                              M, N, K, stream);
}

extern "C" int vited_linear_residual_layernorm_fwd_scaled(const void* a, int64_t lda, const void* w, int64_t ldw, const float* bias,
                                                          const float* residual, int64_t ldr, const float* row_scale, float* y,
                                                          int64_t ldy, const float* gamma, const float* beta, float eps, void* h,
                                                          int64_t ldh, float* mean, float* rstd, int64_t M, int64_t N, int64_t K,
                                                          void* stream) {
    return linear_residual_layernorm_fwd_impl(a, lda, w, ldw, bias, residual, ldr, row_scale, y, ldy, gamma, beta, eps, h, ldh, mean,
                                              rstd, M, N, K, stream);
}

int ln_bwd_finish(const float* partial, int nparts, int dim, float* dgamma, float* dbeta, int accumulate, hipStream_t s);

extern "C" int64_t vited_linear_layernorm_bwd_partial_rows(int64_t M) { return M >= 1 ? row_tiles(M) : 0; }

extern "C" int64_t vited_linear_layernorm_bwd_workspace_bytes(int64_t M, int64_t N) {
    return N == ROW_N && M >= 1 ? row_tiles(M) * 2 * ROW_N * (int64_t)sizeof(float) : 0;
}

static int linear_layernorm_bwd_impl(const void* dy, int64_t lddy, int64_t seg_k, int64_t seg_stride, const void* wt, int64_t ldwt,
                                    const float* x, int64_t ldx, const float* gamma, const float* mean, const float* rstd,
                                    const float* dx_in, int64_t dx_in_ld, float* dx_out, int64_t dx_out_ld, void* dx_lp, int64_t dx_lp_ld,
                                    const float* lp_scale, float* dgamma, float* dbeta, int accumulate, int64_t M, int64_t N, int64_t K,
                                    float* workspace, int64_t workspace_bytes, void* stream) {
    if (lp_scale && !dx_lp) return VITED_ERR_BAD_ARG;
    if (!dy || !wt || !x || !gamma || !mean || !rstd || !dx_out || M <= 0 || N <= 0 || K <= 0) return VITED_ERR_BAD_ARG;
    if ((dgamma == nullptr) != (dbeta == nullptr)) return VITED_ERR_BAD_ARG;
    if (seg_k <= 0 || K % seg_k || lddy < seg_k || ldwt < K || ldx < N || dx_out_ld < N || (dx_in && dx_in_ld < N) || (dx_lp && dx_lp_ld < N))
        return VITED_ERR_BAD_ARG;
    if (!row_shape_ok(M, N, K) || seg_k % 64 || (seg_stride & 7)) return VITED_ERR_UNSUPPORTED;
    if ((lddy & 7) || (ldwt & 7) || (ldx & 3) || (dx_out_ld & 3) || (dx_in && (dx_in_ld & 3)) || (dx_lp && (dx_lp_ld & 3))) return VITED_ERR_UNSUPPORTED;
    if (!al16(dy) || !al16(wt) || !al16(x) || !al16(gamma) || !al16(dx_in) || !al16(dx_out) || ((uintptr_t)dx_lp & 7)) return VITED_ERR_BAD_ARG;
    if (!workspace || workspace_bytes < vited_linear_layernorm_bwd_workspace_bytes(M, N)) return VITED_ERR_WORKSPACE;
    RowArgs r = {};
    r.A = (const bf16*)dy; r.lda = lddy; r.seg_k = (int)seg_k; r.seg_stride = seg_stride; r.W = (const bf16*)wt; r.ldw = ldwt; r.M = M; r.K = (int)K;
    r.gamma = gamma; r.x = x; r.ldx = ldx; r.mean_in = mean; r.rstd_in = rstd;
    r.dx_in = dx_in; r.ldxi = dx_in_ld; r.dx = dx_out; r.lddx = dx_out_ld; r.dx_lp = (bf16*)dx_lp; r.ldlp = dx_lp_ld;
    r.partial = workspace;
    r.lp_scale = lp_scale;
    const int rc = row_launch<ROW_MODE_BWD>(r, (hipStream_t)stream);
    if (rc != VITED_OK || !dgamma) return rc;
    return ln_bwd_finish(workspace, (int)row_tiles(M), ROW_N, dgamma, dbeta, accumulate, (hipStream_t)stream);
}

extern "C" int vited_linear_layernorm_bwd(const void* dy, int64_t lddy, const void* wt, int64_t ldwt, const float* x, int64_t ldx,
                                          const float* gamma, const float* mean, const float* rstd, const float* dx_in,
                                          int64_t dx_in_ld, float* dx_out, int64_t dx_out_ld, void* dx_lp, int64_t dx_lp_ld,
                                          float* dgamma, float* dbeta, int accumulate, int64_t M, int64_t N, int64_t K,
                                          float* workspace, int64_t workspace_bytes, void* stream) {
    return linear_layernorm_bwd_impl(dy, lddy, K, 0, wt, ldwt, x, ldx, gamma, mean, rstd, dx_in, dx_in_ld, dx_out, dx_out_ld, dx_lp, dx_lp_ld,
                                     nullptr, dgamma, dbeta, accumulate, M, N, K, workspace, workspace_bytes, stream);
}

extern "C" int vited_linear_layernorm_bwd_segmented(const void* dy, int64_t lddy, int64_t seg_k, int64_t seg_stride, int64_t segments,
                                                    const void* wt, int64_t ldwt, const float* x, int64_t ldx, const float* gamma,
                                                    const float* mean, const float* rstd, const float* dx_in, int64_t dx_in_ld,
                                                    float* dx_out, int64_t dx_out_ld, void* dx_lp, int64_t dx_lp_ld, float* dgamma,
                                                    float* dbeta, int accumulate, int64_t M, int64_t N, float* workspace,
                                                    int64_t workspace_bytes, void* stream) {
    if (segments <= 0) return VITED_ERR_BAD_ARG;
    return linear_layernorm_bwd_impl(dy, lddy, seg_k, seg_stride, wt, ldwt, x, ldx, gamma, mean, rstd, dx_in, dx_in_ld, dx_out, dx_out_ld, dx_lp,
                                     dx_lp_ld, nullptr, dgamma, dbeta, accumulate, M, N, segments * seg_k, workspace, workspace_bytes, stream);
}

extern "C" int vited_linear_layernorm_bwd_scaled(const void* dy, int64_t lddy, const void* wt, int64_t ldwt, const float* x, int64_t ldx,
                                                 const float* gamma, const float* mean, const float* rstd, const float* dx_in,
                                                 int64_t dx_in_ld, float* dx_out, int64_t dx_out_ld, void* dx_lp, int64_t dx_lp_ld,
                                                 const float* lp_scale, float* dgamma, float* dbeta, int accumulate, int64_t M, int64_t N,
                                                 int64_t K, float* workspace, int64_t workspace_bytes, void* stream) {
    return linear_layernorm_bwd_impl(dy, lddy, K, 0, wt, ldwt, x, ldx, gamma, mean, rstd, dx_in, dx_in_ld, dx_out, dx_out_ld, dx_lp, dx_lp_ld,
                                     lp_scale, dgamma, dbeta, accumulate, M, N, K, workspace, workspace_bytes, stream);
}
```

vit-ed_amd/functions.py:

```python
from __future__ import annotations

import contextlib
import os
from collections import namedtuple

import torch

from . import ops
from ._lib import (B_KN, B_NK, EPI_GELU_GRAD, EPI_MUL, EPI_RESIDUAL, EPI_STORE, EPI_STORE_F32)

LN_EPS = 1e-6


def _bundle(name, table):
    fields, keys = zip(*(pair.split('=') for pair in table.split()))
    return namedtuple(name, fields), keys


_ATTN = 'g1=norm1.weight b1=norm1.bias wqkv=attn.qkv.weight bqkv=attn.qkv.bias wproj=attn.proj.weight bproj=attn.proj.bias '
_CROSS = ('gc=norm_cross.weight bc=norm_cross.bias gx=norm_context.weight bx=norm_context.bias wq=cross_attn.q.weight '
          'bq=cross_attn.q.bias wkv=cross_attn.kv.weight bkv=cross_attn.kv.bias wcp=cross_attn.proj.weight bcp=cross_attn.proj.bias ')
_MLP = 'g2=norm2.weight b2=norm2.bias w1=mlp.fc1.weight bb1=mlp.fc1.bias w2=mlp.fc2.weight bb2=mlp.fc2.bias'
_PATCH = 'pw=patch_embed.proj.weight pb=patch_embed.proj.bias pos=pos_embed '
EncBlock, ENC_BLOCK_KEYS = _bundle('EncBlock', _ATTN + _MLP)
# ... 224 lines not shown

    def __enter__(self):
        self.outer = self.rt.dw_queue
        self.rt.dw_queue = [] if (self.rt.batch_dw and not self.rt.exact) else None
        self.mark = 0
        return self

    @contextlib.contextmanager
    def block(self):
        yield
        self._end_of_block()

    @staticmethod
    def _tiles(items):
        return sum(-(-dy.shape[1] // 128) * (x.shape[1] // 384) for dy, x, _dw, _db, _a in items)

    def _end_of_block(self):
        q = self.rt.dw_queue
        if q is None:
            return
        if not self.blocks:
            self.flush()
            return
        this, count = self._tiles(q[self.mark:]), len(q) - self.mark
        self.mark = len(q)
        if self._tiles(q) + this > self.ROUND or len(q) + count > ops.MAX_BATCHED_WEIGHT_GRADS:
            self.flush()

    def flush(self):
        q = self.rt.dw_queue
        if not q:
            return
        self.rt.dw_queue, self.mark = [], 0
        with _BlockSpan(self.rt, self.kind, len(q), 'dw'):
            for acc in (True, False):
                _launch_weight_grads([(dy, x, dw, db) for dy, x, dw, db, a in q if a == acc], acc)

    def __exit__(self, exc_type, *exc):
        if exc_type is None:
            self.flush()
        self.rt.dw_queue = self.outer
        return False


def _launch_weight_grads(items, accumulate):
    for i in range(0, len(items), ops.MAX_BATCHED_WEIGHT_GRADS):
        part = items[i: i + ops.MAX_BATCHED_WEIGHT_GRADS]
        if len(part) > 1 and ops.linear_bwd_weight_batched(part, accumulate):
            continue
        for dy, x, dw, db in part:
            if accumulate:
                ops.linear_bwd_weight(dy, x, want_bias=db is not None, dw_out=dw, db_out=db)
                continue
            got_w, got_b = ops.linear_bwd_weight(dy, x, want_bias=db is not None)
            dw.copy_(got_w)
            if db is not None:
                db.copy_(got_b)


def _linear_bwd(rt, dy, x_saved, w, b=None, aux=None):
    wt, layout = rt.weight_t(w)
    if aux is not None:
        dx = ops.gemm(dy, wt, b_layout=layout, epilogue=EPI_MUL, aux=aux)
    else:
        dx = ops.gemm(dy, wt, b_layout=layout)
    dw, db = _weight_grads(rt, dy, x_saved, w, b)
    return dx, dw, db


def _row_kernel_ok(rt, m, n, k, dtype, *rowwise):
    return (rt.fused_ln and not rt.exact and ops.linear_layernorm_supported(m, n, k, dtype)
            and all(t is None or (t.dim() == 2 and t.stride(1) == 1 and t.stride(0) % 4 == 0) for t in rowwise))


def _res_linear(rt, a, w, bias, residual, ln=None, scale=None):
    wsh = rt.weight(w)
    if ln is not None and _row_kernel_ok(rt, a.shape[0], wsh.shape[0], a.shape[1], a.dtype, a, residual):
        y, h, mean, rstd = ops.linear_residual_layernorm_fwd(a, wsh, bias, residual, ln[0], ln[1], LN_EPS, row_scale=scale)
        return y, (h, mean, rstd)
    y = ops.gemm(a, wsh, epilogue=EPI_RESIDUAL, bias=bias, residual=residual, row_scale=scale)
    return y, (ops.layernorm_fwd(y, ln[0], ln[1], LN_EPS, rt.act_dtype) if ln is not None else None)


def _linear_ln_bwd(rt, dy, h_saved, w, bias, x, gamma, beta, mean, rstd, dx_in=None, dx_out=None, want_lp=True, lp_scale=None):
    want_lp = want_lp and not rt.exact
    wt, layout = rt.weight_t(w)
    if layout == B_NK and _row_kernel_ok(rt, dy.shape[0], wt.shape[0], dy.shape[1], dy.dtype, dy, x, dx_in, dx_out):
        gg, gb = _gtarget(rt, gamma), _gtarget(rt, beta)
        direct = gg is not None and gb is not None
        dx, dx_lp, dg, db = ops.linear_layernorm_bwd(dy, wt, x, gamma, mean, rstd, dx_in=dx_in, dx_out=dx_out, want_lp=want_lp,
                                                     dgamma=gg if direct else None, dbeta=gb if direct else None, defer=rt.ln_queue,
                                                     lp_scale=lp_scale)
        if direct:
            dg = db = None
    else:
        dh = ops.gemm(dy, wt, b_layout=layout)
        dx, dx_lp, dg, db = _ln_bwd(rt, dh, x, gamma, beta, mean, rstd, dx_in=dx_in, dx_out=dx_out, want_lp=want_lp, lp_scale=lp_scale,
                                    lp_dtype=rt.act_dtype)
    dw, dbias = _weight_grads(rt, dy, h_saved, w, bias)
    return dx, (dx if rt.exact and lp_scale is None else dx_lp), dg, db, dw, dbias


@contextlib.contextmanager
def _ln_sums(rt):
    rt.ln_queue = [] if not rt.exact else None
    try:
        yield
        ops.layernorm_bwd_finish(rt.ln_queue)
    finally:
        rt.ln_queue = None


def _keep_attention(rt, key, q, k):
    b, nq, d = q.shape
    qh = q.float().reshape(b, nq, rt.heads, rt.head_dim).transpose(1, 2)
    kh = k.float().reshape(b, k.shape[1], rt.heads, rt.head_dim).transpose(1, 2)
    rt.attn_store.setdefault(key, {})['attn'] = torch.softmax((qh * rt.scale) @ kh.transpose(-2, -1), dim=-1)


def _keep_attention_grad(rt, key, do, v):
    b, nq, d = do.shape
    doh = do.float().reshape(b, nq, rt.heads, rt.head_dim).transpose(1, 2)
    vh = v.float().reshape(b, v.shape[1], rt.heads, rt.head_dim).transpose(1, 2)
    rt.attn_store.setdefault(key, {})['grad'] = doh @ vh.transpose(-2, -1)


def _keep_attention_cam(rt, key, q, k, v, do, lse):
    ent = rt.attn_store.setdefault(key, {})
    ent['cam'] = ops.attention_cam(q, k, v, do, lse, rt.heads, rt.scale, mode='grad')
    if key == ('cross_blocks', rt.c_depth - 1, 'cross_attn'):
        ent['cam_operands'] = (q, k, v, do, lse)


def _cam_only(rt, grads):
    return [None] * len(grads) if rt.keep_cam else grads


def _self_attn_fwd(rt, h, wqkv, bqkv, batch, n, key=None):
    d = rt.dim
    qkv = ops.gemm(h, rt.weight(wqkv), bias=bqkv)
    qkv3 = qkv.view(batch, n, 3 * d)
    o, lse = ops.attention_fwd(qkv3[:, :, 0:d], qkv3[:, :, d:2 * d], qkv3[:, :, 2 * d:3 * d], rt.heads, rt.scale)
    if rt.keep_attn and key is not None:
        _keep_attention(rt, key, qkv3[:, :, 0:d], qkv3[:, :, d:2 * d])
    return qkv, o.view(batch * n, d), lse


def _self_attn_bwd(rt, do, qkv, o, lse, batch, n, key=None):
    d = rt.dim
    qkv3 = qkv.view(batch, n, 3 * d)
    if rt.keep_attn and key is not None:
        _keep_attention_grad(rt, key, do.view(batch, n, d), qkv3[:, :, 2 * d:3 * d])
    if rt.keep_cam and key is not None:
        _keep_attention_cam(rt, key, qkv3[:, :, 0:d], qkv3[:, :, d:2 * d], qkv3[:, :, 2 * d:3 * d], do.view(batch, n, d), lse)
    dqkv = torch.empty_like(qkv)
    dqkv3 = dqkv.view(batch, n, 3 * d)
    ops.attention_bwd(qkv3[:, :, 0:d], qkv3[:, :, d:2 * d], qkv3[:, :, 2 * d:3 * d], o.view(batch, n, d),
                      do.view(batch, n, d), lse, rt.heads, rt.scale, dqkv3[:, :, 0:d], dqkv3[:, :, d:2 * d],
                      dqkv3[:, :, 2 * d:3 * d])
    return dqkv


FUSED_MLP_TILE = 128
FUSED_MLP_CUS = 256


def _fused_mlp_rows(rt, x, w1, grad):
    if grad or rt.exact or not rt.fused_mlp or x.shape[1] != 384 or tuple(w1.shape) != (1536, 384) or x.stride(0) != 384:
        return 0
    tiles = x.shape[0] // FUSED_MLP_TILE
    rem = tiles % FUSED_MLP_CUS
    if tiles >= FUSED_MLP_CUS and rem < FUSED_MLP_CUS // 4:
        tiles -= rem
    elif x.shape[0] % FUSED_MLP_TILE:
        tiles += 1
    return min(tiles * FUSED_MLP_TILE, x.shape[0])


def _hand_over_ln(rt, x, P, grad):
    return grad or not _fused_mlp_rows(rt, x, P.w1, grad)


def _mlp_fwd(rt, x, P, grad=True, ln=None, next_ln=None, scale=None):
    g, b, w1, b1, w2, b2 = P.g2, P.b2, P.w1, P.bb1, P.w2, P.bb2
    rows = _fused_mlp_rows(rt, x, w1, grad) if ln is None and scale is None else 0
    if rows:
        y = torch.empty_like(x)
        ops.mlp_fwd(x[:rows], g, b, rt.weight(w1), b1, rt.weight(w2), b2, LN_EPS, save=False, out=(y[:rows], None, None, None, None, None))
        if rows < x.shape[0]:
            xt = x[rows:]
            ht, _, _ = ops.layernorm_fwd(xt, g, b, LN_EPS, rt.act_dtype)
            _, ut = ops.gemm(ht, rt.weight(w1), epilogue=EPI_GELU_GRAD, bias=b1)
            ops.gemm(ut, rt.weight(w2), epilogue=EPI_RESIDUAL, bias=b2, residual=xt, out=y[rows:])
        nxt = ops.layernorm_fwd(y, next_ln[0], next_ln[1], LN_EPS, rt.act_dtype) if next_ln is not None else None
        return y, None, nxt
    h, mean, rstd = ln if ln is not None else ops.layernorm_fwd(x, g, b, LN_EPS, rt.act_dtype)
    gd, u = ops.gemm(h, rt.weight(w1), epilogue=EPI_GELU_GRAD, bias=b1)
    y, nxt = _res_linear(rt, u, w2, b2, x, next_ln, scale)
    return y, (mean, rstd, h, gd, u), nxt


def _mlp_bwd(rt, dy, dy_lp, x, P, saved, lp_scale=None):
    mean, rstd, h, gd, u = saved
    dz, dw2, dbb2 = _linear_bwd(rt, dy_lp, u, P.w2, P.bb2, aux=gd)
    dx, dx_lp, dg2, db2, dw1, dbb1 = _linear_ln_bwd(rt, dz, h, P.w1, P.bb1, x, P.g2, P.b2, mean, rstd, dx_in=dy, lp_scale=lp_scale)
    return dx, dx_lp, dict(g2=dg2, b2=db2, w1=dw1, bb1=dbb1, w2=dw2, bb2=dbb2)


def _attn_branch_fwd(rt, x, P, batch, n, key=None, ln=None, next_ln=None, scale=None):
    h, mean, rstd = ln if ln is not None else ops.layernorm_fwd(x, P.g1, P.b1, LN_EPS, rt.act_dtype)
    qkv, o, lse = _self_attn_fwd(rt, h, P.wqkv, P.bqkv, batch, n, key)
    y, nxt = _res_linear(rt, o, P.wproj, P.bproj, x, next_ln, scale)
    return y, (mean, rstd, h, qkv, o, lse), nxt


def _attn_branch_bwd(rt, dy, dy_lp, x, P, saved, batch, n, key=None, lp_scale=None):
    mean, rstd, h, qkv, o, lse = saved
    do, dwproj, dbproj = _linear_bwd(rt, dy_lp, o, P.wproj, P.bproj)
    dqkv = _self_attn_bwd(rt, do, qkv, o, lse, batch, n, key)
    dx, dx_lp, dg1, db1, dwqkv, dbqkv = _linear_ln_bwd(rt, dqkv, h, P.wqkv, P.bqkv, x, P.g1, P.b1, mean, rstd, dx_in=dy, lp_scale=lp_scale)
    return dx, dx_lp, dict(g1=dg1, b1=db1, wqkv=dwqkv, bqkv=dbqkv, wproj=dwproj, bproj=dbproj)


def _patch_tokens_fwd(rt, img, S, with_cls, batch_index=None):
    patches = ops.patchify(img, rt.patch_size, rt.act_dtype, batch_index, mean=rt.input_mean, std=rt.input_std)
    batch = patches.shape[0] // rt.n1
    pos2 = S.pos.view(rt.n2, rt.dim)
    rows, first = (rt.n2, 1) if with_cls else (rt.n1, 0)
    x = ops.gemm(patches, rt.weight(S.pw), epilogue=EPI_RESIDUAL, bias=S.pb, residual=pos2[1 - first:], rows_per_batch=rt.n1,
                 out_rows_per_batch=rows, row_offset=first, residual_bcast=True, out_rows=batch * rows)
    if with_cls:
        ops.write_cls_row(x.view(batch, rt.n2, rt.dim), S.cls.view(-1), pos2)
    return x, patches, batch, rows


def _patch_tokens_bwd(rt, dx, patches, S, with_cls, batch):
    rows = rt.n2 if with_cls else rt.n1
    dx3 = dx.view(batch, rows, rt.dim)
    dpos_rows = ops.sum_rows(dx3.view(batch, rows * rt.dim)).view(rows, rt.dim)
    dpos = torch.zeros_like(S.pos)
    grads = dict(pos=dpos)
    if with_cls:
        dpos[0] = dpos_rows
        grads['cls'] = dpos_rows[0].clone().view_as(S.cls)
        dtok = ops.slice_rows_cast(dx3, 1, rt.n1, rt.act_dtype)
    else:
        dpos[0, 1:] = dpos_rows
        dtok = dx if rt.exact else ops.cast(dx, rt.act_dtype)
    grads['pw'], grads['pb'] = _weight_grads(rt, dtok, patches, S.pw, S.pb)
    return grads


def _norm1_of(blocks, i):
    return (blocks[i].g1, blocks[i].b1) if i < len(blocks) else None


class EncoderFn(torch.autograd.Function):
    @staticmethod
    def forward(ctx, rt: Runtime, img, *params):
        shared, blocks = split_params(params, EncShared, EncBlock)
        grad = any(ctx.needs_input_grad)
        x, patches, batch, n = _patch_tokens_fwd(rt, img, shared, with_cls=False)
        drop = _take_drop_rows(rt, 0, len(blocks), 2, batch, n, x.device)
        tape = []
        ln1 = None
        for i, P in enumerate(blocks):
            s_attn, s_mlp = drop.block(i) if drop is not None else (None, None)
            chain = _hand_over_ln(rt, x, P, grad or s_mlp is not None)
            with _BlockSpan(rt, 'enc', i, 'fwd'):
                xa, sa, ln2 = _attn_branch_fwd(rt, x, P, batch, n, key=('blocks', i, 'attn'), ln=ln1, next_ln=(P.g2, P.b2) if chain else None,
                                               scale=s_attn)
                xb, sm, ln1 = _mlp_fwd(rt, xa, P, grad, ln=ln2, next_ln=_norm1_of(blocks, i + 1) if chain else None, scale=s_mlp)
            if grad:
                tape.append((x, sa, xa, sm))
            x = xb
            if rt.tap is not None:
                rt.tap[f'enc.x.{len(tape) - 1 if grad else 0}'] = x.clone()
        if grad:
            ctx.rt, ctx.tape, ctx.patches, ctx.batch, ctx.params = rt, tape, patches, batch, (shared, blocks)
            ctx.drop = drop
        return x.view(batch, n, rt.dim)

    @staticmethod
    def backward(ctx, dout):
        rt, batch, n = ctx.rt, ctx.batch, ctx.rt.n1
        shared, blocks = ctx.params
        dx = dout.contiguous().view(batch * n, rt.dim).float()
        drop = ctx.drop
        scale_of = (lambda i, j: drop.get(i, j)) if drop is not None else (lambda i, j: None)
        dx_lp = _lp_scaled(rt, dx, scale_of(len(blocks) - 1, 1))
        gblocks = [None] * len(blocks)
        with _ln_sums(rt), _DwBatch(rt, kind='enc') as dwg:
            for i in reversed(range(len(blocks))):
                x, sa, xa, sm = ctx.tape[i]
                ctx.tape[i] = None
                with _BlockSpan(rt, 'enc', i, 'bwd'), dwg.block():
                    dx, dx_lp, gm = _mlp_bwd(rt, dx, dx_lp, xa, blocks[i], sm, lp_scale=scale_of(i, 0))
                    dx, dx_lp, ga = _attn_branch_bwd(rt, dx, dx_lp, x, blocks[i], sa, batch, n, key=('blocks', i, 'attn'),
                                                     lp_scale=scale_of(i - 1, 1))
                if rt.tap is not None:
                    rt.tap[f'enc.dx.{i}'] = dx.clone()
                gblocks[i] = EncBlock(**ga, **gm)
        gshared = EncShared(**_patch_tokens_bwd(rt, dx, ctx.patches, shared, with_cls=False, batch=batch))
        ctx.tape = ctx.patches = ctx.drop = None
        return (None, None, *_cam_only(rt, flatten_params(gshared, gblocks)))


def _dense_rows(t):
    out = torch.empty(t.shape, dtype=t.dtype, device=t.device)
    out.copy_(t)
    return out


def _dec_self_fwd(rt, x, P, batch, n, cls_only, key=None, ln1=None, fuse_ln=True, scale=None):
    next_ln = (P.gc, P.bc) if fuse_ln else None
    if not cls_only:
        return _attn_branch_fwd(rt, x, P, batch, n, key=key, ln=ln1, next_ln=next_ln, scale=scale)
    d = rt.dim
    h1, m1, r1 = ln1 if ln1 is not None else ops.layernorm_fwd(x, P.g1, P.b1, LN_EPS, rt.act_dtype)
    qkv = ops.gemm(h1, rt.weight(P.wqkv), bias=P.bqkv)
    qkv3 = qkv.view(batch, n, 3 * d)
    o0, lse0 = ops.attention_fwd(qkv3[:, 0:1, 0:d], qkv3[:, :, d:2 * d], qkv3[:, :, 2 * d:3 * d], rt.heads, rt.scale)
    o0 = o0.view(batch, d)
    x0 = _dense_rows(x.view(batch, n, d)[:, 0, :])
    xa, lnq = _res_linear(rt, o0, P.wproj, P.bproj, x0, next_ln, scale)
    return xa, (m1, r1, h1, qkv, o0, lse0), lnq


def _dec_self_bwd(rt, dx, dx_lp, x, P, saved, batch, n, cls_only, key=None, lp_scale=None):
    if not cls_only:
        return _attn_branch_bwd(rt, dx, dx_lp, x, P, saved, batch, n, key=key, lp_scale=lp_scale)
    d = rt.dim
    m1, r1, h1, qkv, o0, lse0 = saved
    do0, dwproj, dbproj = _linear_bwd(rt, dx_lp, o0, P.wproj, P.bproj)
    qkv3 = qkv.view(batch, n, 3 * d)
    dqkv = torch.zeros_like(qkv)
    dqkv3 = dqkv.view(batch, n, 3 * d)
    ops.attention_bwd(qkv3[:, 0:1, 0:d], qkv3[:, :, d:2 * d], qkv3[:, :, 2 * d:3 * d], o0.view(batch, 1, d), do0.view(batch, 1, d),
                      lse0, rt.heads, rt.scale, dqkv3[:, 0:1, 0:d], dqkv3[:, :, d:2 * d], dqkv3[:, :, 2 * d:3 * d])
    dres = torch.zeros((batch * n, d), dtype=torch.float32, device=dx.device)
    dres.view(batch, n, d)[:, 0, :].copy_(dx)
    dx, dx_lp, dg1, db1, dwqkv, dbqkv = _linear_ln_bwd(rt, dqkv, h1, P.wqkv, P.bqkv, x, P.g1, P.b1, m1, r1, dx_in=dres, lp_scale=lp_scale)
    return dx, dx_lp, dict(g1=dg1, b1=db1, wqkv=dwqkv, bqkv=dbqkv, wproj=dwproj, bproj=dbproj)


def _cross_q(rt, xa, P, lnq=None):
    hq, mq, rq = lnq if lnq is not None else ops.layernorm_fwd(xa, P.gc, P.bc, LN_EPS, rt.act_dtype)
    return ops.gemm(hq, rt.weight(P.wq), bias=P.bq), (hq, mq, rq)


def _dec_cross_fwd(rt, xa, P, batch, lnq=None, q=None, kv3=None, ctxf=None, kv_index=None, key=None, fuse_ln=True, scale=None, items=None):
    d, nq = rt.dim, xa.shape[0] // batch
    hq = mq = rq = hc = mc = rc = None
    if q is None:
        q, (hq, mq, rq) = _cross_q(rt, xa, P, lnq)
    kv = kv3
    if kv3 is None:
        hc, mc, rc = ops.layernorm_fwd(ctxf, P.gx, P.bx, LN_EPS, rt.act_dtype)
        kv = ops.gemm(hc, rt.weight(P.wkv), bias=P.bkv)
        kv3 = kv.view(batch if items is None else items, rt.n1, 2 * d)
    oc, lse_c = ops.attention_fwd(q.view(batch, nq, d), kv3[:, :, 0:d], kv3[:, :, d:2 * d], rt.heads, rt.scale, kv_index=kv_index)
    if rt.keep_attn and key is not None:
        _keep_attention(rt, key, q.view(batch, nq, d), kv3[:, :, 0:d])
    oc = oc.view(batch * nq, d)
    xb, ln2 = _res_linear(rt, oc, P.wcp, P.bcp, xa, (P.g2, P.b2) if fuse_ln else None, scale)
    return xb, (mq, rq, hq, mc, rc, hc, q, kv, oc, lse_c), ln2


def _dec_cross_bwd(rt, dx, dx_lp, xa, P, saved, ctxf, dctx, batch, index, dkv3=None, lp_scale=None, seg=None):
    d, nq = rt.dim, xa.shape[0] // batch
    items = batch if seg is None else seg.items
    mq, rq, hq, mc, rc, hc, q, kv, oc, lse_c = saved
    doc, dwcp, dbcp = _linear_bwd(rt, dx_lp, oc, P.wcp, P.bcp)
    dq = torch.empty_like(q)
    folded = hc is None
    if folded:
        kv3, dkv = kv, dkv3
    else:
        dkv = torch.empty_like(kv)
        kv3, dkv3 = kv.view(items, rt.n1, 2 * d), dkv.view(items, rt.n1, 2 * d)
    if rt.keep_attn:
        _keep_attention_grad(rt, ('cross_blocks', index, 'cross_attn'), doc.view(batch, nq, d), kv3[:, :, d:2 * d])
    if rt.keep_cam:
        _keep_attention_cam(rt, ('cross_blocks', index, 'cross_attn'), q.view(batch, nq, d), kv3[:, :, 0:d], kv3[:, :, d:2 * d],
                            doc.view(batch, nq, d), lse_c)
    ops.attention_bwd(q.view(batch, nq, d), kv3[:, :, 0:d], kv3[:, :, d:2 * d], oc.view(batch, nq, d),
                      doc.view(batch, nq, d), lse_c, rt.heads, rt.scale, dq.view(batch, nq, d), dkv3[:, :, 0:d],
                      dkv3[:, :, d:2 * d], segments=seg)
    if rt.tap is not None:
        i = index
        rt.tap[f'dec.doc.{i}'], rt.tap[f'dec.dq.{i}'], rt.tap[f'dec.dkv.{i}'] = doc.clone(), dq.clone(), dkv.clone()
        rt.tap[f'dec.q.{i}'], rt.tap[f'dec.kv.{i}'], rt.tap[f'dec.oc.{i}'] = q.clone(), kv.clone(), oc.clone()
    dx, dx_lp, dgc, dbc, dwq, dbq = _linear_ln_bwd(rt, dq, hq, P.wq, P.bq, xa, P.gc, P.bc, mq, rq, dx_in=dx, lp_scale=lp_scale)
    dgx = dbx = dwkv = dbkv = None
    if not folded:
        dctx, _, dgx, dbx, dwkv, dbkv = _linear_ln_bwd(rt, dkv, hc, P.wkv, P.bkv, ctxf, P.gx, P.bx, mc, rc, dx_in=dctx, dx_out=dctx, want_lp=False)
    return dx, dx_lp, dctx, dict(gc=dgc, bc=dbc, gx=dgx, bx=dbx, wq=dwq, bq=dbq, wkv=dwkv, bkv=dbkv, wcp=dwcp, bcp=dbcp)


def _dec_block_fwd(rt, x, ctxf, P, batch, n, grad, cls_only, index=0, ln1=None, next_ln=None, kv3=None, scales=(None, None, None),
                   seg=None):
    xa, sa, lnq = _dec_self_fwd(rt, x, P, batch, n, cls_only, key=('cross_blocks', index, 'attn'), ln1=ln1, scale=scales[0])
    xb, sc, ln2 = _dec_cross_fwd(rt, xa, P, batch, lnq=lnq, kv3=kv3, ctxf=ctxf, key=('cross_blocks', index, 'cross_attn'),
                                 fuse_ln=_hand_over_ln(rt, xa, P, grad or scales[2] is not None), scale=scales[1],
                                 kv_index=seg.index if seg is not None else None, items=seg.items if seg is not None else None)
    xc, sm, nxt = _mlp_fwd(rt, xb, P, grad, ln=ln2, next_ln=next_ln, scale=scales[2])
    return xc, ((x, sa, xa, sc, xb, sm) if grad else None), nxt


def _dec_block_bwd(rt, dx, dx_lp, ctxf, dctx, P, entry, batch, n, cls_only, index, dkv3=None, lp_scales=(None, None, None), seg=None):
    x, sa, xa, sc, xb, sm = entry
    dx, dx_lp, gm = _mlp_bwd(rt, dx, dx_lp, xb, P, sm, lp_scale=lp_scales[0])
    dx, dx_lp, dctx, gc = _dec_cross_bwd(rt, dx, dx_lp, xa, P, sc, ctxf, dctx, batch, index, dkv3, lp_scale=lp_scales[1], seg=seg)
    dx, dx_lp, ga = _dec_self_bwd(rt, dx, dx_lp, x, P, sa, batch, n, cls_only, key=('cross_blocks', index, 'attn'), lp_scale=lp_scales[2])
    return dx, dx_lp, dctx, DecBlock(**ga, **gc, **gm)


@torch.no_grad()
def image2_tokens(rt: Runtime, img, params):
    shared, blocks = split_params(params, DecShared, DecBlock)
    x, _, batch, _ = _patch_tokens_fwd(rt, img, shared, with_cls=True)
    if not blocks or (rt.cls_tail and rt.c_depth == 1):
        return x.view(batch, rt.n2, rt.dim), None
    xa, _, lnq = _dec_self_fwd(rt, x, blocks[0], batch, rt.n2, cls_only=False)
    q, _ = _cross_q(rt, xa, blocks[0], lnq)
# ... 100 lines not shown
        d = rt.dim
        cls_tail = rt.cls_tail and rt.c_depth > 0 and not (rt.keep_attn or rt.keep_cam)
        drop = _take_drop_rows(rt, 1, len(blocks), 3, batch, n, x.device, cls_block=rt.c_depth - 1 if cls_tail else None)
        ln1 = None
        fold = rt.fold_context and not rt.exact and rt.c_depth > 1 and rt.c_depth <= ops.MAX_FOLDED_BLOCKS and rt.dim % 32 == 0
        kv_all = kv_saved = fold_bufs = None
        if fold:
            kv_all, kv_saved, fold_bufs = _context_kv_folded(rt, ctxf, blocks)
        for i, P in enumerate(blocks):
            x, entry, ln1 = _dec_block_fwd(rt, x, ctxf, P, batch, n, grad, cls_tail and i == rt.c_depth - 1, index=i, ln1=ln1,
                                           next_ln=_norm1_of(blocks, i + 1), kv3=kv_all[i].view(b1, rt.n1, 2 * d) if fold else None,
                                           scales=drop.block(i) if drop is not None else (None, None, None), seg=seg)
            if grad:
                tape.append(entry)
            if rt.tap is not None:
                rt.tap[f'dec.x.{i}'] = x.clone()
        xcls = x if cls_tail else x.view(batch, n, d)[:, 0, :]
        y, mN, rN = ops.layernorm_fwd(xcls, shared.gN, shared.bN, LN_EPS, rt.act_dtype)
        logits = ops.gemm(y, rt.weight(shared.wh), epilogue=EPI_STORE_F32, bias=shared.bh)
        if grad:
            ctx.rt, ctx.tape, ctx.patches, ctx.batch, ctx.params = rt, tape, patches, batch, (shared, blocks)
            ctx.ctxf, ctx.final, ctx.cls_tail = ctxf, (xcls, y, mN, rN), cls_tail
            ctx.feats_needs_grad = feats.requires_grad
            ctx.fold = (kv_all, kv_saved, fold_bufs) if fold else None
            ctx.drop = drop
            ctx.seg = seg
        return logits

    @staticmethod
    def backward(ctx, dlogits):
        rt, batch, n, d = ctx.rt, ctx.batch, ctx.rt.n2, ctx.rt.dim
        shared, blocks = ctx.params
        xcls, y, mN, rN = ctx.final
        dl = _lp(rt, dlogits.contiguous().float())
        wh_act = rt.weight(shared.wh)
        dy = ops.gemm(dl, wh_act, b_layout=B_KN)
        dwh, dbh = _weight_grads(rt, dl, y, shared.wh, shared.bh)
        drop, last = ctx.drop, len(blocks) - 1
        seg = ctx.seg
        b1 = batch if seg is None else seg.items
        scale_of = (lambda i, j: drop.get(i, j)) if drop is not None else (lambda i, j: None)
        s_head = drop.per_sample[last, 2] if drop is not None and drop.live[last][2] else None
        if s_head is not None:
            lp_dtype = rt.act_dtype
            if ctx.cls_tail:
                dx, dx_lp, dgN, dbN = _ln_bwd(rt, dy, xcls, shared.gN, shared.bN, mN, rN, lp_scale=s_head, lp_dtype=lp_dtype)
            else:
                dx = torch.zeros((batch * n, d), dtype=torch.float32, device=dy.device)
                dx_lp = torch.zeros((batch * n, d), dtype=lp_dtype, device=dy.device)
                _, _, dgN, dbN = _ln_bwd(rt, dy, xcls, shared.gN, shared.bN, mN, rN, dx_out=dx.view(batch, n, d)[:, 0, :],
                                         dx_lp=dx_lp.view(batch, n, d)[:, 0, :], lp_scale=s_head, lp_dtype=lp_dtype)
        elif ctx.cls_tail:
            dx, dx_lp, dgN, dbN = _ln_bwd(rt, dy, xcls, shared.gN, shared.bN, mN, rN, want_lp=not rt.exact)
        else:
            dx = torch.zeros((batch * n, d), dtype=torch.float32, device=dy.device)
            dx_lp = dx_lp3 = None
            if not rt.exact:
                dx_lp = torch.zeros((batch * n, d), dtype=rt.act_dtype, device=dy.device)
                dx_lp3 = dx_lp.view(batch, n, d)[:, 0, :]
            _, _, dgN, dbN = _ln_bwd(rt, dy, xcls, shared.gN, shared.bN, mN, rN, dx_out=dx.view(batch, n, d)[:, 0, :], dx_lp=dx_lp3)
        if rt.exact and s_head is None:
            dx_lp = dx
        dctx = None
        gblocks = [None] * len(blocks)
        dkv_all = torch.empty_like(ctx.fold[0]) if ctx.fold is not None else None
        with _ln_sums(rt):
            with _DwBatch(rt, kind='dec') as dwg:
                for i in reversed(range(len(blocks))):
                    entry = ctx.tape[i]
                    ctx.tape[i] = None
                    with dwg.block():
                        dx, dx_lp, dctx, gblocks[i] = _dec_block_bwd(rt, dx, dx_lp, ctx.ctxf, dctx, blocks[i], entry, batch, n,
                                                                     ctx.cls_tail and i == rt.c_depth - 1, i,
                                                                     dkv3=dkv_all[i].view(b1, rt.n1, 2 * d) if dkv_all is not None else None,
                                                                     lp_scales=(scale_of(i, 1), scale_of(i, 0), scale_of(i - 1, 2)), seg=seg)
                    if rt.tap is not None:
                        rt.tap[f'dec.dx.{i}'] = dx.clone()
                        if dctx is not None:
                            rt.tap[f'dec.dctx.{i}'] = dctx.clone()
            if dkv_all is not None:
                dctx, kv_grads = _context_kv_folded_bwd(rt, dkv_all, ctx.ctxf, ctx.fold[1], ctx.fold[2], blocks)
                gblocks = [g._replace(**kv) for g, kv in zip(gblocks, kv_grads)]
                ctx.fold = None
        gshared = DecShared(**_patch_tokens_bwd(rt, dx, ctx.patches, shared, with_cls=True, batch=batch), gN=dgN, bN=dbN, wh=dwh, bh=dbh)
        dfeats = dctx.view(b1, rt.n1, d) if ctx.feats_needs_grad and dctx is not None else None
        ctx.tape = ctx.patches = ctx.ctxf = ctx.final = ctx.drop = ctx.seg = None
        return (None, dfeats, None, None, None, *_cam_only(rt, flatten_params(gshared, gblocks)))
```

vit-ed_amd/ops.py:

```python
from __future__ import annotations

import ctypes as C
from typing import NamedTuple

import torch

from . import _lib
from ._lib import (B_KN, B_NK, BF16, EPI_GELU, EPI_GELU_GRAD, EPI_MUL, EPI_MUL_GELU_GRAD, EPI_RESIDUAL, EPI_STORE, EPI_STORE_F32, F16,
                   F32, I32, I64)

_DTYPE = {torch.float32: F32, torch.bfloat16: BF16, torch.float16: F16, torch.int32: I32, torch.int64: I64}
_FLOATS = (torch.float32, torch.bfloat16, torch.float16)


def _code(dtype: torch.dtype) -> int:
    if dtype not in (torch.float32, torch.bfloat16):
        raise TypeError(f'vited ops support float32 and bfloat16 activations, got {dtype}')
    return _DTYPE[dtype]


def _need_gpu(*tensors):
    for t in tensors:
        if t is not None and not t.is_cuda:
            raise RuntimeError('vited ops run on the MI355X HIP kernels only: got a CPU tensor '
# ... 173 lines not shown
    for t, dtype, shape in specs:
        assert t.dtype == dtype and tuple(t.shape) == (b, *shape) and t.is_contiguous(), (t.dtype, tuple(t.shape), dtype, (b, *shape))


def hisfrag_windows_u8(store: torch.Tensor, img_off: torch.Tensor, img_hw: torch.Tensor, image: torch.Tensor, flags: torch.Tensor,
                       afix: torch.Tensor, minv: torch.Tensor, origin: torch.Tensor, img_size: int,
                       out: torch.Tensor | None = None) -> torch.Tensor:
    _need_gpu(store, img_off, img_hw, image, flags, afix, minv, origin, out)
    s = int(img_size)
    n, b = img_off.numel(), image.numel()
    assert store.dtype == torch.uint8 and store.dim() == 1 and store.is_contiguous()
    assert img_off.dtype == torch.int64 and img_off.dim() == 1 and img_off.is_contiguous()
    assert img_hw.dtype == torch.int32 and img_hw.shape == (n, 2) and img_hw.is_contiguous()
    _batch_args(b, (image, torch.int32, ()), (flags, torch.int32, ()), (afix, torch.int64, (6,)), (minv, torch.float64, (6,)),
                (origin, torch.int32, (2,)))
    if out is None:
        out = torch.empty((b, 3, s, s), dtype=torch.uint8, device=store.device)
    assert out.dtype == torch.uint8 and tuple(out.shape) == (b, 3, s, s) and out.is_contiguous()
    _lib.call('vited_hisfrag_windows_u8', _ptr(store), _ptr(img_off), _ptr(img_hw), n, _ptr(image), _ptr(flags), _ptr(afix), _ptr(minv),
              _ptr(origin), _ptr(out), b, s, _stream())
    return out


def hisfrag_jitter_u8(img: torch.Tensor, flags: torch.Tensor, order: torch.Tensor, factors: torch.Tensor, hue: torch.Tensor,
                      out: torch.Tensor | None = None) -> torch.Tensor:
    _need_gpu(img, flags, order, factors, hue, out)
    assert img.dtype == torch.uint8 and img.dim() == 4 and img.shape[1] == 3 and img.shape[2] == img.shape[3] and img.is_contiguous()
    b, s = img.shape[0], img.shape[2]
    _batch_args(b, (flags, torch.int32, ()), (order, torch.int32, (4,)), (factors, torch.float32, (3,)), (hue, torch.int32, ()))
    if out is None:
        out = torch.empty_like(img)
    assert out.dtype == torch.uint8 and out.shape == img.shape and out.is_contiguous()
    sums = torch.empty(b, dtype=torch.int64, device=img.device)
    _lib.call('vited_hisfrag_jitter_u8', _ptr(img), _ptr(flags), _ptr(order), _ptr(factors), _ptr(hue), _ptr(sums), _ptr(out), b, s, _stream())
    return out


def hisfrag_blur_u8(img: torch.Tensor, flags: torch.Tensor, weights: torch.Tensor, out: torch.Tensor | None = None) -> torch.Tensor:
    _need_gpu(img, flags, weights, out)
    assert img.dtype == torch.uint8 and img.dim() == 4 and img.shape[1] == 3 and img.shape[2] == img.shape[3] and img.is_contiguous()
    b, s = img.shape[0], img.shape[2]
    _batch_args(b, (flags, torch.int32, ()), (weights, torch.float32, (2,)))
    if out is None:
        out = torch.empty_like(img)
    assert out.dtype == torch.uint8 and out.shape == img.shape and out.is_contiguous() and out.data_ptr() != img.data_ptr()
    _lib.call('vited_hisfrag_blur_u8', _ptr(img), _ptr(flags), _ptr(weights), _ptr(out), b, s, _stream())
    return out


def michigan_windows_u8(store: torch.Tensor, img_off: torch.Tensor, img_hw: torch.Tensor, image: torch.Tensor, flags: torch.Tensor,
                        origin: torch.Tensor, x0: torch.Tensor, kx: torch.Tensor, y0: torch.Tensor, ky: torch.Tensor, holes: torch.Tensor,
                        n_holes: torch.Tensor, img_size: int, out: torch.Tensor | None = None) -> torch.Tensor:
    _need_gpu(store, img_off, img_hw, image, flags, origin, x0, kx, y0, ky, holes, n_holes, out)
    s = int(img_size)
    n, b = img_off.numel(), image.numel()
    assert store.dtype == torch.uint8 and store.dim() == 1 and store.is_contiguous()
    assert img_off.dtype == torch.int64 and img_off.dim() == 1 and img_off.is_contiguous()
    assert img_hw.dtype == torch.int32 and img_hw.shape == (n, 2) and img_hw.is_contiguous()
    i32 = torch.int32
    _batch_args(b, (image, i32, ()), (flags, i32, ()), (origin, i32, (2,)), (x0, i32, (s,)), (kx, i32, (s, 3)), (y0, i32, (s,)),
                (ky, i32, (s, 3)), (holes, i32, (16, 4)), (n_holes, i32, ()))
    if out is None:
        out = torch.empty((b, 3, s, s), dtype=torch.uint8, device=store.device)
    assert out.dtype == torch.uint8 and tuple(out.shape) == (b, 3, s, s) and out.is_contiguous()
    _lib.call('vited_michigan_windows_u8', _ptr(store), _ptr(img_off), _ptr(img_hw), n, _ptr(image), _ptr(flags), _ptr(origin), _ptr(x0),
              _ptr(kx), _ptr(y0), _ptr(ky), _ptr(holes), _ptr(n_holes), _ptr(out), b, s, _stream())
    return out


def michigan_blur_gray_u8(img: torch.Tensor, flags: torch.Tensor, weights: torch.Tensor, out: torch.Tensor | None = None) -> torch.Tensor:
    _need_gpu(img, flags, weights, out)
    assert img.dtype == torch.uint8 and img.dim() == 4 and img.shape[1] == 3 and img.shape[2] == img.shape[3] and img.is_contiguous()
    b, s = img.shape[0], img.shape[2]
    _batch_args(b, (flags, torch.int32, ()), (weights, torch.int32, (2,)))
    if out is None:
        out = torch.empty_like(img)
    assert out.dtype == torch.uint8 and out.shape == img.shape and out.is_contiguous() and out.data_ptr() != img.data_ptr()
    _lib.call('vited_michigan_blur_gray_u8', _ptr(img), _ptr(flags), _ptr(weights), _ptr(out), b, s, _stream())
    return out


def slice_rows_cast(x: torch.Tensor, row_offset: int, rows: int, dtype: torch.dtype) -> torch.Tensor:
    _need_gpu(x)
    assert x.dtype == torch.float32 and x.dim() == 3 and x.is_contiguous()
    b, r, d = x.shape
    out = torch.empty((b * rows, d), dtype=dtype, device=x.device)
    _lib.call('vited_slice_rows_cast', _ptr(x), _ptr(out), _code(dtype), b, r, row_offset, rows, d, _stream())
    return out


def write_cls_row(x: torch.Tensor, cls: torch.Tensor, pos: torch.Tensor):
    _need_gpu(x, cls, pos)
    assert x.dtype == torch.float32 and x.is_contiguous() and x.dim() == 3
    b, r, d = x.shape
    _lib.call('vited_write_cls_row', _ptr(x), _ptr(cls), _ptr(pos), b, r, d, _stream())


def sum_rows(x: torch.Tensor) -> torch.Tensor:
    _need_gpu(x)
    ld = _rows2d(x)
    b, w = x.shape
    out = torch.empty(w, dtype=torch.float32, device=x.device)
    ws = _scratch(_lib.load().vited_sum_rows_workspace_bytes(b, w), x.device)
    _lib.call('vited_sum_rows', _ptr(x), _code(x.dtype), ld, _ptr(out), b, w, *ws, _stream())
    return out


def layernorm_fwd(x: torch.Tensor, gamma: torch.Tensor, beta: torch.Tensor, eps: float, out_dtype: torch.dtype, out=None):
    _need_gpu(x, gamma, beta)
    assert x.dtype == torch.float32 and gamma.dtype == torch.float32 and beta.dtype == torch.float32
    ld = _rows2d(x)
    rows, dim = x.shape
    if out is not None:
        y, mean, rstd = out
        assert y.shape == (rows, dim) and y.dtype == out_dtype and _rows2d(y) == dim and mean.numel() == rows and rstd.numel() == rows
    else:
        y = torch.empty((rows, dim), dtype=out_dtype, device=x.device)
        mean = torch.empty(rows, dtype=torch.float32, device=x.device)
        rstd = torch.empty(rows, dtype=torch.float32, device=x.device)
    _lib.call('vited_layernorm_fwd', _ptr(x), ld, _ptr(gamma), _ptr(beta), _ptr(y), _code(out_dtype), dim, _ptr(mean), _ptr(rstd), rows,
              dim, float(eps), _stream())
    return y, mean, rstd


def layernorm_bwd(dy, x, gamma, mean, rstd, dx_in=None, dx_out=None, want_lp: bool = False, dx_lp=None, dgamma=None,
                  dbeta=None, lp_scale=None, lp_dtype=torch.bfloat16):
    _need_gpu(dy, x, gamma, mean, rstd, dx_in, dx_out, dx_lp, lp_scale)
    dy_ld, x_ld = _rows2d(dy), _rows2d(x)
    rows, dim = x.shape
    assert dy.shape == x.shape and x.dtype == torch.float32
    if dx_out is None:
        dx_out = torch.empty((rows, dim), dtype=torch.float32, device=x.device)
    if lp_scale is not None:
        _check_row_scale(lp_scale, rows)
        want_lp = True
    else:
        lp_dtype = torch.bfloat16
    if want_lp and dx_lp is None:
        dx_lp = torch.empty((rows, dim), dtype=lp_dtype, device=x.device)
    assert dx_lp is None or dx_lp.dtype == lp_dtype
    if dx_in is not None:
        assert dx_in.dtype == torch.float32 and dx_in.shape == x.shape
    accumulate = dgamma is not None
    if accumulate:
        assert dbeta is not None and dgamma.dtype == dbeta.dtype == torch.float32 and dgamma.is_contiguous() and dbeta.is_contiguous()
    else:
        dgamma = torch.empty(dim, dtype=torch.float32, device=x.device)
        dbeta = torch.empty(dim, dtype=torch.float32, device=x.device)
    ws = _scratch(_lib.load().vited_layernorm_bwd_workspace_bytes(rows, dim), x.device)
    head = (_ptr(dy), _code(dy.dtype), dy_ld, _ptr(x), x_ld, _ptr(gamma), _ptr(mean), _ptr(rstd),
            _ptr(dx_in), _rows2d(dx_in) if dx_in is not None else 0, _ptr(dx_out), _rows2d(dx_out),
            _ptr(dx_lp), _code(lp_dtype), _rows2d(dx_lp) if dx_lp is not None else 0)
    tail = (_ptr(dgamma), _ptr(dbeta), int(accumulate), rows, dim, *ws, _stream())
    if lp_scale is not None:
        _lib.call('vited_layernorm_bwd_scaled', *head, _ptr(lp_scale), *tail)
    else:
        _lib.call('vited_layernorm_bwd', *head, *tail)
    return dx_out, dx_lp, dgamma, dbeta


def gemm(a: torch.Tensor, b: torch.Tensor, *, b_layout: int = B_NK, epilogue: int = EPI_STORE, bias=None, aux=None,
         residual=None, out=None, out2=None, rows_per_batch: int = 0, out_rows_per_batch: int = 0, row_offset: int = 0,
         residual_bcast: bool = False, out_rows: int | None = None, row_scale=None):
    _need_gpu(a, b, bias, aux, residual, out)
    assert a.dtype == b.dtype, f'operand dtypes differ: {a.dtype} vs {b.dtype}'
    lda, ldb = _rows2d(a), _rows2d(b)
    m, k = a.shape
    n = b.shape[0] if b_layout == B_NK else b.shape[1]
    kb = b.shape[1] if b_layout == B_NK else b.shape[0]
    if kb != k:
        raise ValueError(f'contraction mismatch: A is [{m},{k}], B gives K={kb}')
    f32_out = epilogue in (EPI_RESIDUAL, EPI_STORE_F32)
    if out is None:
        rows = m if out_rows is None else out_rows
        out = torch.empty((rows, n), dtype=torch.float32 if f32_out else a.dtype, device=a.device)
    ldo = _rows2d(out)
    if epilogue in (EPI_GELU, EPI_GELU_GRAD):
        if out2 is None:
            out2 = torch.empty_like(out)
        assert out2.dtype == out.dtype and out2.shape == out.shape and _rows2d(out2) == ldo
    else:
        out2 = None
    if aux is not None:
        assert aux.dtype == a.dtype and _rows2d(aux) == ldo
    if residual is not None:
# ... 13 lines not shown
    _lib.call('vited_gemm', _ptr(a), lda, _ptr(b), ldb, b_layout, _code(a.dtype), m, n, k, epilogue, _ptr(bias), _ptr(aux), _ptr(residual),
              _ptr(out), _ptr(out2), ldo, rows_per_batch, out_rows_per_batch, row_offset, int(bool(residual_bcast)), _stream())
    return (out, out2) if epilogue in (EPI_GELU, EPI_GELU_GRAD) else out


def linear_bwd_weight(dy: torch.Tensor, x: torch.Tensor, want_bias: bool = True, dw_out=None, db_out=None):
    _need_gpu(dy, x)
    assert dy.dtype == x.dtype and dy.shape[0] == x.shape[0]
    lddy, ldx = _rows2d(dy), _rows2d(x)
    m, n = dy.shape
    k = x.shape[1]
    accumulate = dw_out is not None
    if accumulate:
        assert dw_out.dtype == torch.float32 and dw_out.is_contiguous() and dw_out.numel() == n * k
        dw, db = dw_out, (db_out if want_bias else None)
        assert db is None or (db.dtype == torch.float32 and db.is_contiguous() and db.numel() == n)
    else:
        dw = torch.empty((n, k), dtype=torch.float32, device=x.device)
        db = torch.empty(n, dtype=torch.float32, device=x.device) if want_bias else None
    ws = _scratch(_lib.load().vited_linear_bwd_weight_workspace_bytes(m, n, k), x.device)
    _lib.call('vited_linear_bwd_weight', _ptr(dy), lddy, _ptr(x), ldx, _code(x.dtype), m, n, k, _ptr(dw), _ptr(db), int(accumulate), *ws,
              _stream())
    return dw, db


MAX_BATCHED_WEIGHT_GRADS = 40


def linear_bwd_weight_batched(items, accumulate: bool) -> bool:
    n = len(items)
    if n < 1 or n > MAX_BATCHED_WEIGHT_GRADS:
        return False
    for dy, x, dw, db in items:
        _need_gpu(dy, x, dw, db)
        if dy.dtype != torch.bfloat16 or x.dtype != torch.bfloat16 or dy.shape[0] != x.shape[0]:
            return False
        assert dw.dtype == torch.float32 and dw.is_contiguous() and dw.numel() == dy.shape[1] * x.shape[1]
        assert db is None or (db.dtype == torch.float32 and db.is_contiguous() and db.numel() == dy.shape[1])
        if dw.data_ptr() % 16 or (db is not None and db.data_ptr() % 16) or dy.data_ptr() % 16 or x.data_ptr() % 16:
            return False
    dys, xs, dws, dbs = zip(*items)
    M = _host_array(C.c_int64, [dy.shape[0] for dy in dys])
    N = _host_array(C.c_int64, [dy.shape[1] for dy in dys])
    K = _host_array(C.c_int64, [x.shape[1] for x in xs])
    lib = _lib.load()
    if not lib.vited_linear_bwd_weight_batched_supported(n, M, N, K, BF16):
        return False
    lddy, ldx = _host_array(C.c_int64, map(_rows2d, dys)), _host_array(C.c_int64, map(_rows2d, xs))
    ws = _scratch(lib.vited_linear_bwd_weight_batched_workspace_bytes(n, M, N, K), dys[0].device)
    _lib.call('vited_linear_bwd_weight_batched', n, _host_array(C.c_void_p, dys), lddy, _host_array(C.c_void_p, xs), ldx, M, N, K,
              _host_array(C.c_void_p, dws), _host_array(C.c_void_p, dbs), BF16, int(bool(accumulate)), *ws, _stream())
    return True


def linear_layernorm_supported(m: int, n: int, k: int, dtype: torch.dtype) -> bool:
    return dtype == torch.bfloat16 and bool(_lib.load().vited_linear_layernorm_supported(int(m), int(n), int(k)))


def linear_residual_layernorm_fwd(a, w, bias, residual, gamma=None, beta=None, eps: float = 1e-6, out=None, row_scale=None):
    _need_gpu(a, w, bias, residual, gamma, beta, out, row_scale)
    assert a.dtype == w.dtype == torch.bfloat16 and residual.dtype == torch.float32
    lda, ldw, ldr = _rows2d(a), _rows2d(w), _rows2d(residual)
    m, k = a.shape
    n = w.shape[0]
    assert w.shape[1] == k and residual.shape == (m, n)
    y = out if out is not None else torch.empty((m, n), dtype=torch.float32, device=a.device)
    assert y.dtype == torch.float32 and y.shape == (m, n)
    h = mean = rstd = None
    if gamma is not None:
        h = torch.empty((m, n), dtype=torch.bfloat16, device=a.device)
        mean = torch.empty(m, dtype=torch.float32, device=a.device)
        rstd = torch.empty(m, dtype=torch.float32, device=a.device)
    tail = (_ptr(y), _rows2d(y), _ptr(gamma), _ptr(beta), float(eps), _ptr(h), n, _ptr(mean), _ptr(rstd), m, n, k, _stream())
    if row_scale is not None:
        _check_row_scale(row_scale, m)
        _lib.call('vited_linear_residual_layernorm_fwd_scaled', _ptr(a), lda, _ptr(w), ldw, _ptr(bias), _ptr(residual), ldr, _ptr(row_scale),
                  *tail)
    else:
        _lib.call('vited_linear_residual_layernorm_fwd', _ptr(a), lda, _ptr(w), ldw, _ptr(bias), _ptr(residual), ldr, *tail)
    return y, h, mean, rstd


def linear_layernorm_bwd(dy, wt, x, gamma, mean, rstd, dx_in=None, dx_out=None, want_lp: bool = False, dgamma=None, dbeta=None,
                         defer=None, lp_scale=None):
    _need_gpu(dy, wt, x, gamma, mean, rstd, dx_in, dx_out, lp_scale)
    assert dy.dtype == wt.dtype == torch.bfloat16 and x.dtype == torch.float32
    segments = 1
    if dy.dim() == 3:
        assert dy.stride(2) == 1 and dy.stride(0) % 8 == 0
        segments, m, seg_k = dy.shape
        lddy, seg_stride, k = dy.stride(1), dy.stride(0), segments * seg_k
    else:
        lddy = _rows2d(dy)
        m, k = dy.shape
    ldwt, ldx = _rows2d(wt), _rows2d(x)
    n = wt.shape[0]
    assert wt.shape[1] == k and x.shape == (m, n)
    lib = _lib.load()
    if dx_out is None:
        dx_out = torch.empty((m, n), dtype=torch.float32, device=x.device)
    if lp_scale is not None:
        _check_row_scale(lp_scale, m)
        assert segments == 1
        want_lp = True
    dx_lp = torch.empty((m, n), dtype=torch.bfloat16, device=x.device) if want_lp else None
    accumulate = dgamma is not None
    if accumulate:
        assert dbeta is not None and dgamma.dtype == dbeta.dtype == torch.float32 and dgamma.is_contiguous() and dbeta.is_contiguous()
    else:
        dgamma = torch.empty(n, dtype=torch.float32, device=x.device)
        dbeta = torch.empty(n, dtype=torch.float32, device=x.device)
    if defer is not None:
        rows = int(lib.vited_linear_layernorm_bwd_partial_rows(m))
        part = torch.empty(rows * 2 * n, dtype=torch.float32, device=x.device)
        defer.append((part, rows, dgamma, dbeta, accumulate))
        ws = (part.data_ptr(), part.numel() * 4)
    else:
        ws = _scratch(lib.vited_linear_layernorm_bwd_workspace_bytes(m, n), x.device)
    dx_args = (_ptr(x), ldx, _ptr(gamma), _ptr(mean), _ptr(rstd), _ptr(dx_in), _rows2d(dx_in) if dx_in is not None else 0, _ptr(dx_out),
               _rows2d(dx_out), _ptr(dx_lp), n)
    sum_args = (0 if defer is not None else _ptr(dgamma), 0 if defer is not None else _ptr(dbeta), int(accumulate))
    tail = dx_args + sum_args
    if lp_scale is not None:
        _lib.call('vited_linear_layernorm_bwd_scaled', _ptr(dy), lddy, _ptr(wt), ldwt, *dx_args, _ptr(lp_scale), *sum_args, m, n, k, *ws,
                  _stream())
    elif segments > 1:
        _lib.call('vited_linear_layernorm_bwd_segmented', _ptr(dy), lddy, seg_k, seg_stride, segments, _ptr(wt), ldwt, *tail, m, n, *ws,
                  _stream())
    else:
        _lib.call('vited_linear_layernorm_bwd', _ptr(dy), lddy, _ptr(wt), ldwt, *tail, m, n, k, *ws, _stream())
    return dx_out, dx_lp, dgamma, dbeta


def layernorm_bwd_finish(entries):
    if not entries:
        return
    parts, rows, dgammas, dbetas, accumulate = zip(*entries)
    _lib.call('vited_layernorm_bwd_finish_batched', len(entries), _host_array(C.c_void_p, parts), _host_array(C.c_int, rows),
              _host_array(C.c_void_p, dgammas), _host_array(C.c_void_p, dbetas), _host_array(C.c_int, map(int, accumulate)),
              dgammas[0].numel(), _stream())
    entries.clear()


MAX_FOLDED_BLOCKS = 16


def fold_context_weights(ws, biases, gammas, betas, out=None):
    n_blk = len(ws)
    _need_gpu(*ws, *gammas, *betas)
    n, k = ws[0].shape
    dev = ws[0].device
    if out is None:
        out = (torch.empty((n_blk * n, k), dtype=torch.bfloat16, device=dev), torch.empty((k, n_blk * n), dtype=torch.bfloat16, device=dev),
               torch.empty(n_blk * n, dtype=torch.float32, device=dev))
    for t in list(ws) + list(gammas) + list(betas):
        assert t.dtype == torch.float32 and t.is_contiguous()
    _lib.call('vited_fold_context_weights', n_blk, *(_host_array(C.c_void_p, ts) for ts in (ws, biases, gammas, betas)), n, k,
              _ptr(out[0]), _ptr(out[1]), _ptr(out[2]), _stream())
    return out


def unfold_context_grads(dwf, dbf, ws, gammas, betas, dws, dbiases, dgammas, dbetas, accumulate: bool):
    n_blk = len(ws)
    n, k = ws[0].shape
    assert dwf.dtype == dbf.dtype == torch.float32 and dwf.is_contiguous() and dbf.is_contiguous()
    assert dwf.shape == (n_blk * n, k) and dbf.numel() == n_blk * n
    _lib.call('vited_unfold_context_grads', n_blk, _ptr(dwf), _ptr(dbf),
              *(_host_array(C.c_void_p, ts) for ts in (ws, gammas, betas, dws, dbiases, dgammas, dbetas)), n, k, int(bool(accumulate)),
              _stream())


def mlp_fwd(x, gamma, beta, w1, b1, w2, b2, eps: float, save: bool = True, out=None):
    _need_gpu(x, gamma, beta, w1, b1, w2, b2)
    assert x.dtype == torch.float32 and w1.dtype == w2.dtype == torch.bfloat16 and w1.is_contiguous() and w2.is_contiguous()
    ldx = _rows2d(x)
    rows, dim = x.shape
    hidden = w1.shape[0]
    assert w1.shape == (hidden, dim) and w2.shape == (dim, hidden)
    dev = x.device
    if out is not None:
        y, mean, rstd, h, gd, u = out
    else:
        y = torch.empty((rows, dim), dtype=torch.float32, device=dev)
        mean = rstd = h = gd = u = None
        if save:
            mean = torch.empty(rows, dtype=torch.float32, device=dev)
            rstd = torch.empty(rows, dtype=torch.float32, device=dev)
            h = torch.empty((rows, dim), dtype=torch.bfloat16, device=dev)
            gd = torch.empty((rows, hidden), dtype=torch.bfloat16, device=dev)
            u = torch.empty((rows, hidden), dtype=torch.bfloat16, device=dev)
    if save:
        assert h.is_contiguous() and gd.is_contiguous() and u.is_contiguous() and h.shape == (rows, dim) and gd.shape == u.shape == (rows, hidden)
    _lib.call('vited_mlp_fwd', _ptr(x), ldx, _ptr(gamma), _ptr(beta), _ptr(w1), _ptr(b1), _ptr(w2), _ptr(b2), _ptr(y), _rows2d(y),
              _ptr(h) if save else 0, _ptr(gd) if save else 0, _ptr(u) if save else 0, _ptr(mean) if save else 0, _ptr(rstd) if save else 0,
              rows, dim, hidden, float(eps), _stream())
    return y, ((mean, rstd, h, gd, u) if save else None)


def block_fwd(x, heads: int, ln1_g, ln1_b, wqkv, bqkv, wproj, bproj, ln2_g, ln2_b, w1, b1, w2, b2, eps: float = 1e-6):
    _need_gpu(x, wqkv, wproj, w1, w2)
    assert x.dtype == torch.float32 and x.dim() == 3 and x.is_contiguous()
    assert all(t.dtype == torch.bfloat16 and t.is_contiguous() for t in (wqkv, wproj, w1, w2))
    b, n, d = x.shape
    hidden = w1.shape[0]
    y = torch.empty_like(x)
    ws, nbytes = _scratch(_lib.load().vited_block_workspace_bytes(b, n, d, hidden, heads) + 256, x.device)
# ... 437 lines not shown
```

Baseline: 43280.

## Vectorize patchify/slice kernels, fuse periodic residual into LN bwd, direct weight-grad writes

Several independent changes. Patchify and bf16 row slicing get 8-wide vectorized kernels. The layernorm backward gains a periodic dx_in mode, so the decoder no longer materializes a zero-filled dense residual. The weight-gradient GEMM writes straight into dW when there is one split, and patch-token backward reuses the existing bf16 dx instead of recasting. The unfold kernel's block shape and unroll are also retuned; the added code paths and conditions raise the risk of alignment-dependent fallbacks.

Measured after the change: 43600, median of 6. About the same (+0.7%).

```diff
diff --git a/include/vited.h b/include/vited.h
--- a/include/vited.h
+++ b/include/vited.h
@@ -77,6 +77,8 @@
 
 int vited_slice_rows_cast(const float* in, void* out, int out_dtype, int64_t batch, int64_t in_rows,
                           int64_t row_offset, int64_t rows, int64_t dim, void* stream);
+int vited_slice_rows_cast_from(const void* in, int in_dtype, void* out, int out_dtype, int64_t batch, int64_t in_rows,
+                               int64_t row_offset, int64_t rows, int64_t dim, void* stream);
 
 int vited_write_cls_row(float* x, const float* cls, const float* pos, int64_t batch, int64_t rows_per_batch,
                         int64_t dim, void* stream);
@@ -162,6 +164,12 @@
                                       const float* lp_scale, float* dgamma, float* dbeta, int accumulate, int64_t M, int64_t N,
                                       int64_t K, float* workspace, int64_t workspace_bytes, void* stream);
 
+int vited_linear_layernorm_bwd_periodic(const void* dy, int64_t lddy, const void* wt, int64_t ldwt, const float* x, int64_t ldx,
+                                        const float* gamma, const float* mean, const float* rstd, const float* dx_in,
+                                        int64_t dx_in_ld, float* dx_out, int64_t dx_out_ld, void* dx_lp, int64_t dx_lp_ld,
+                                        const float* lp_scale, float* dgamma, float* dbeta, int accumulate, int64_t M, int64_t N,
+                                        int64_t K, float* workspace, int64_t workspace_bytes, void* stream, int64_t dx_in_period);
+
 int vited_fold_context_weights(int count, const float* const* w, const float* const* bias, const float* const* gamma,
                                const float* const* beta, int64_t N, int64_t K, void* w_out, void* wt_out, float* bias_out,
                                void* stream);
diff --git a/profiles/step_thin.py b/profiles/step_thin.py
--- /dev/null
+++ b/profiles/step_thin.py
@@ -0,0 +1,48 @@
+#!/usr/bin/env python3
+import csv
+import re
+import sys
+
+BIG = (('row-complete', r'^(void )?gemm_row_kernel'), ('NT GEMM', r'^(void )?gemm_nt_'), ('weight gradient', r'^(void )?gemm_tn_wide_kernel'),
+       ('attention', r'^(void )?attn_'))
+
+
+def short(name):
+    name = re.sub(r'^void ', '', name)
+    depth, out = 0, []
+    for ch in name:
+        if ch == '(' and depth == 0:
+            break
+        depth += ch == '<'
+        depth -= ch == '>'
+        out.append(ch)
+    return ''.join(out)[:100]
+
+
+rows = sorted(csv.DictReader(open(sys.argv[1])), key=lambda r: int(r['Start_Timestamp']))
+ends = [i for i, r in enumerate(rows) if 'optim_update_kernel' in r['Kernel_Name']]
+if len(ends) < 2:
+    sys.exit('the trace holds fewer than two optimizer updates')
+step = rows[ends[-2] + 1:ends[-1] + 1]
+t0, t1 = int(step[0]['Start_Timestamp']), int(step[-1]['End_Timestamp'])
+sums = {name: [0, 0.0] for name, _ in BIG}
+sums['everything else'] = [0, 0.0]
+print('# one replayed step: launches outside the four big classes, in launch order')
+print('index_in_step,kernel,grid_x,duration_us')
+for i, r in enumerate(step):
+    us = (int(r['End_Timestamp']) - int(r['Start_Timestamp'])) / 1e3
+    for name, pat in BIG:
+        if re.search(pat, r['Kernel_Name']):
+            sums[name][0] += 1
+            sums[name][1] += us
+            break
+    else:
+        sums['everything else'][0] += 1
+        sums['everything else'][1] += us
+        print(f'{i},"{short(r["Kernel_Name"])}",{r["Grid_Size_X"]},{us:.1f}')
+print('# class sums of the step')
+print('class,launches,total_us')
+for name, (n, us) in sums.items():
+    print(f'"{name}",{n},{us:.1f}')
+print(f'"all",{len(step)},{sum(v[1] for v in sums.values()):.1f}')
+print(f'"wall (first start to last end)",{len(step)},{(t1 - t0) / 1e3:.1f}')
diff --git a/vit-ed_amd/csrc/context_fold.hip b/vit-ed_amd/csrc/context_fold.hip
--- a/vit-ed_amd/csrc/context_fold.hip
+++ b/vit-ed_amd/csrc/context_fold.hip
@@ -64,10 +64,13 @@
 };
 
 #define UF_GROUPS 16
-__global__ void __launch_bounds__(64 * UF_GROUPS) unfold_context_kernel(const UnfoldArgs a) {
-    __shared__ float red[2][UF_GROUPS][64];
-    const int l = blockIdx.y, kx = threadIdx.x & 63, ng = threadIdx.x >> 6;
-    const int k = blockIdx.x * 64 + kx;
+#ifndef UF_COLS
+#define UF_COLS 16
+#endif
+__global__ void __launch_bounds__(UF_COLS * UF_GROUPS) unfold_context_kernel(const UnfoldArgs a) {
+    __shared__ float red[2][UF_GROUPS][UF_COLS];
+    const int l = blockIdx.y, kx = threadIdx.x % UF_COLS, ng = threadIdx.x / UF_COLS;
+    const int k = blockIdx.x * UF_COLS + kx;
     const bool ok = k < a.K;
     const float* __restrict__ w = a.w[l];
     const float* __restrict__ dwf = a.dwf + (int64_t)l * a.N * a.K;
@@ -75,7 +78,7 @@
     float* __restrict__ dw = a.dw[l];
     const float g = ok ? a.gamma[l][k] : 0.f, be = ok ? a.beta[l][k] : 0.f;
     float sg = 0.f, sb = 0.f;
-#pragma unroll 4
+#pragma unroll 8
     for (int n = ng; n < a.N; n += UF_GROUPS) {
         if (ok) {
             const int64_t o = (int64_t)n * a.K + k;
@@ -100,7 +103,7 @@
         a.dbeta[l][k] = a.accumulate ? a.dbeta[l][k] + tb : tb;
     }
     if (blockIdx.x == 0 && a.dbias[l]) {
-        for (int n = threadIdx.x; n < a.N; n += 64 * UF_GROUPS) a.dbias[l][n] = a.accumulate ? a.dbias[l][n] + dbf[n] : dbf[n];
+        for (int n = threadIdx.x; n < a.N; n += UF_COLS * UF_GROUPS) a.dbias[l][n] = a.accumulate ? a.dbias[l][n] + dbf[n] : dbf[n];
     }
 }
 
@@ -115,6 +118,6 @@
         a.w[i] = w[i]; a.gamma[i] = gamma[i]; a.beta[i] = beta[i]; a.dw[i] = dw[i]; a.dbias[i] = dbias[i]; a.dgamma[i] = dgamma[i]; a.dbeta[i] = dbeta[i];
     }
     a.dwf = dwf; a.dbf = dbf; a.count = count; a.N = (int)N; a.K = (int)K; a.accumulate = accumulate;
-    hipLaunchKernelGGL(unfold_context_kernel, dim3((unsigned)ceil_div64(K, 64), (unsigned)count), dim3(64 * UF_GROUPS), 0, (hipStream_t)stream, a);
+    hipLaunchKernelGGL(unfold_context_kernel, dim3((unsigned)ceil_div64(K, UF_COLS), (unsigned)count), dim3(UF_COLS * UF_GROUPS), 0, (hipStream_t)stream, a);
     return vited_check_launch();
 }
diff --git a/vit-ed_amd/csrc/elementwise.hip b/vit-ed_amd/csrc/elementwise.hip
--- a/vit-ed_amd/csrc/elementwise.hip
+++ b/vit-ed_amd/csrc/elementwise.hip
@@ -190,12 +190,57 @@
     }
 }
 
+struct U8Norm { float scale[4], shift[4]; };
+
+template <bool U8>
+__global__ void __launch_bounds__(256)
+patchify_piece_kernel(const void* __restrict__ img, int64_t img_bs, const int64_t* __restrict__ bidx, bf16* __restrict__ out,
+                      int chans, int S, int p, int64_t pieces, U8Norm nrm) {
+    const int64_t q = (int64_t)blockIdx.x * blockDim.x + threadIdx.x;
+    if (q >= pieces) return;
+    const int p8 = p >> 3, G = S / p;
+    const int per_token = chans * p * p8;
+    const int64_t t = q / per_token;
+    const int rem = (int)(q - t * per_token);
+    const int ci = rem / p8, j8 = rem - ci * p8;
+    const int c = ci / p, i = ci - c * p;
+    const int64_t b = t / (G * G);
+    const int cell = (int)(t - b * (G * G));
+    const int py = cell / G, px = cell - py * G;
+    const int64_t src_b = bidx ? bidx[b] : b;
+    const int64_t o = src_b * img_bs + ((int64_t)c * S + (py * p + i)) * S + px * p + j8 * 8;
+    float v[8];
+    if constexpr (U8) {
+        const uint2 w = *(const uint2*)((const uint8_t*)img + o);
+#pragma unroll
+        for (int e = 0; e < 4; ++e) {
+            v[e] = fmaf((float)((w.x >> (8 * e)) & 0xffu), nrm.scale[c], nrm.shift[c]);
+            v[4 + e] = fmaf((float)((w.y >> (8 * e)) & 0xffu), nrm.scale[c], nrm.shift[c]);
+        }
+    } else {
+        const f32x4 a = *(const f32x4*)((const float*)img + o), d = *(const f32x4*)((const float*)img + o + 4);
+#pragma unroll
+        for (int e = 0; e < 4; ++e) { v[e] = a[e]; v[4 + e] = d[e]; }
+    }
+    *(bf16x8*)(out + q * 8) = bf16x8{(bf16)v[0], (bf16)v[1], (bf16)v[2], (bf16)v[3], (bf16)v[4], (bf16)v[5], (bf16)v[6], (bf16)v[7]};
+}
+
+static inline bool patchify_pieces_ok(const void* img, int64_t img_bs, const void* out, int out_dtype, int patch, int src_bytes) {
+    const int64_t load = src_bytes == 4 ? 16 : 8;
+    return out_dtype == VITED_BF16 && patch % 8 == 0 && ((uintptr_t)out & 15) == 0 && ((uintptr_t)img % load) == 0 &&
+           (img_bs * src_bytes) % load == 0;
+}
+
 extern "C" int vited_patchify(const float* img, int64_t img_bs, const int64_t* batch_index, void* out, int out_dtype,
                               int64_t batch, int chans, int img_size, int patch, void* stream) {
     if (!img || !out || batch <= 0 || chans <= 0 || img_size <= 0 || patch <= 0 || img_size % patch) return VITED_ERR_BAD_ARG;
     dim3 grid(img_size / patch, (unsigned)batch);
     hipStream_t s = (hipStream_t)stream;
-    if (out_dtype == VITED_BF16)
+    const int64_t pieces = batch * chans * img_size * (img_size / 8);
+    if (patchify_pieces_ok(img, img_bs, out, out_dtype, patch, 4) && ceil_div64(pieces, 256) <= 0x7fffffff)
+        hipLaunchKernelGGL((patchify_piece_kernel<false>), dim3((unsigned)ceil_div64(pieces, 256)), dim3(256), 0, s, img, img_bs,
+                           batch_index, (bf16*)out, chans, img_size, patch, pieces, U8Norm{});
+    else if (out_dtype == VITED_BF16)
         hipLaunchKernelGGL((patchify_kernel<bf16>), grid, dim3(256), 0, s, img, img_bs, batch_index, (bf16*)out, chans, img_size, patch);
     else if (out_dtype == VITED_F32)
         hipLaunchKernelGGL((patchify_kernel<float>), grid, dim3(256), 0, s, img, img_bs, batch_index, (float*)out, chans, img_size, patch);
@@ -203,8 +248,6 @@
         return VITED_ERR_UNSUPPORTED;
     return vited_check_launch();
 }
-
-struct U8Norm { float scale[4], shift[4]; };
 
 template <typename D>
 __global__ void patchify_u8_kernel(const uint8_t* __restrict__ img, int64_t img_bs, const int64_t* __restrict__ bidx,
@@ -240,7 +283,11 @@
     }
     dim3 grid(img_size / patch, (unsigned)batch);
     hipStream_t s = (hipStream_t)stream;
-    if (out_dtype == VITED_BF16)
+    const int64_t pieces = batch * chans * img_size * (img_size / 8);
+    if (patchify_pieces_ok(img, img_bs, out, out_dtype, patch, 1) && ceil_div64(pieces, 256) <= 0x7fffffff)
+        hipLaunchKernelGGL((patchify_piece_kernel<true>), dim3((unsigned)ceil_div64(pieces, 256)), dim3(256), 0, s, img, img_bs,
+                           batch_index, (bf16*)out, chans, img_size, patch, pieces, nrm);
+    else if (out_dtype == VITED_BF16)
         hipLaunchKernelGGL((patchify_u8_kernel<bf16>), grid, dim3(256), 0, s, img, img_bs, batch_index, (bf16*)out, chans, img_size, patch, nrm);
     else if (out_dtype == VITED_F32)
         hipLaunchKernelGGL((patchify_u8_kernel<float>), grid, dim3(256), 0, s, img, img_bs, batch_index, (float*)out, chans, img_size, patch, nrm);
@@ -317,32 +364,55 @@
     return vited_check_launch();
 }
 
-template <typename D>
-__global__ void slice_rows_cast_kernel(const float* __restrict__ in, D* __restrict__ out, int64_t in_rows,
+template <typename S_, typename D>
+__global__ void slice_rows_cast_kernel(const S_* __restrict__ in, D* __restrict__ out, int64_t in_rows,
                                        int64_t row_offset, int64_t rows, int64_t dim, int64_t total) {
     int64_t i = (int64_t)blockIdx.x * blockDim.x + threadIdx.x;
     const int64_t stride = (int64_t)gridDim.x * blockDim.x;
     const int64_t per_b = rows * dim;
     for (; i < total; i += stride) {
         const int64_t b = i / per_b, rem = i - b * per_b;
-        out[i] = from_f32<D>(in[(b * in_rows + row_offset) * dim + rem]);
-    }
-}
-
-extern "C" int vited_slice_rows_cast(const float* in, void* out, int out_dtype, int64_t batch, int64_t in_rows,
-                                     int64_t row_offset, int64_t rows, int64_t dim, void* stream) {
+        out[i] = from_f32<D>(to_f32(in[(b * in_rows + row_offset) * dim + rem]));
+    }
+}
+
+__global__ void __launch_bounds__(256)
+slice_rows_lp_kernel(const bf16* __restrict__ in, bf16* __restrict__ out, int64_t in_rows, int64_t row_offset, int64_t rows,
+                     int64_t dim8, int64_t pieces) {
+    const int64_t q = (int64_t)blockIdx.x * blockDim.x + threadIdx.x;
+    if (q >= pieces) return;
+    const int64_t per_b = rows * dim8;
+    const int64_t b = q / per_b, rem = q - b * per_b;
+    *(bf16x8*)(out + q * 8) = *(const bf16x8*)(in + ((b * in_rows + row_offset) * dim8 + rem) * 8);
+}
+
+extern "C" int vited_slice_rows_cast_from(const void* in, int in_dtype, void* out, int out_dtype, int64_t batch, int64_t in_rows,
+                                          int64_t row_offset, int64_t rows, int64_t dim, void* stream) {
     if (!in || !out || batch <= 0 || rows <= 0 || dim <= 0 || row_offset < 0 || row_offset + rows > in_rows) return VITED_ERR_BAD_ARG;
     const int64_t total = batch * rows * dim;
     int64_t blocks = ceil_div64(total, 256);
     if (blocks > 8192) blocks = 8192;
     hipStream_t s = (hipStream_t)stream;
-    if (out_dtype == VITED_BF16)
-        hipLaunchKernelGGL((slice_rows_cast_kernel<bf16>), dim3(blocks), dim3(256), 0, s, in, (bf16*)out, in_rows, row_offset, rows, dim, total);
-    else if (out_dtype == VITED_F32)
-        hipLaunchKernelGGL((slice_rows_cast_kernel<float>), dim3(blocks), dim3(256), 0, s, in, (float*)out, in_rows, row_offset, rows, dim, total);
+    if (in_dtype == VITED_BF16 && out_dtype == VITED_BF16) {
+        const int64_t pieces = total / 8;
+        if (dim % 8 == 0 && (((uintptr_t)in | (uintptr_t)out) & 15) == 0 && ceil_div64(pieces, 256) <= 0x7fffffff)
+            hipLaunchKernelGGL(slice_rows_lp_kernel, dim3((unsigned)ceil_div64(pieces, 256)), dim3(256), 0, s, (const bf16*)in, (bf16*)out,
+                               in_rows, row_offset, rows, dim / 8, pieces);
+        else
+            hipLaunchKernelGGL((slice_rows_cast_kernel<bf16, bf16>), dim3(blocks), dim3(256), 0, s, (const bf16*)in, (bf16*)out, in_rows,
+                               row_offset, rows, dim, total);
+    } else if (in_dtype == VITED_F32 && out_dtype == VITED_BF16)
+        hipLaunchKernelGGL((slice_rows_cast_kernel<float, bf16>), dim3(blocks), dim3(256), 0, s, (const float*)in, (bf16*)out, in_rows, row_offset, rows, dim, total);
+    else if (in_dtype == VITED_F32 && out_dtype == VITED_F32)
+        hipLaunchKernelGGL((slice_rows_cast_kernel<float, float>), dim3(blocks), dim3(256), 0, s, (const float*)in, (float*)out, in_rows, row_offset, rows, dim, total);
     else
         return VITED_ERR_UNSUPPORTED;
     return vited_check_launch();
+}
+
+extern "C" int vited_slice_rows_cast(const float* in, void* out, int out_dtype, int64_t batch, int64_t in_rows,
+                                     int64_t row_offset, int64_t rows, int64_t dim, void* stream) {
+    return vited_slice_rows_cast_from(in, VITED_F32, out, out_dtype, batch, in_rows, row_offset, rows, dim, stream);
 }
 
 __global__ void write_cls_row_kernel(float* __restrict__ x, const float* __restrict__ cls, const float* __restrict__ pos,
diff --git a/vit-ed_amd/csrc/gemm.hip b/vit-ed_amd/csrc/gemm.hip
--- a/vit-ed_amd/csrc/gemm.hip
+++ b/vit-ed_amd/csrc/gemm.hip
@@ -153,7 +153,12 @@
     float* bias_slabs = base + splits * ws;
     hipStream_t s = (hipStream_t)stream;
     g_last_gemm_path = 2;
-    int rc = gemm_tn_batch(count, dY, lddy, X, ldx, M, N, K, has_bias, slabs, bias_slabs, s);
+    if (splits == 1) {
+        for (int i = 0; i < count; ++i)
+            if (widths[i] % 4 || nbias[i] % 4 || ((uintptr_t)dW[i] & 15) || ((uintptr_t)dbias[i] & 15)) return VITED_ERR_UNSUPPORTED;
+        return gemm_tn_batch(count, dY, lddy, X, ldx, M, N, K, has_bias, nullptr, nullptr, dW, dbias, accumulate, s);
+    }
+    int rc = gemm_tn_batch(count, dY, lddy, X, ldx, M, N, K, has_bias, slabs, bias_slabs, nullptr, nullptr, accumulate, s);
     if (rc != VITED_OK) return rc;
     return sum_slabs_batch(count, slabs, ws, bias_slabs, bs, splits, widths, dW, nbias, dbias, accumulate, s);
 }
diff --git a/vit-ed_amd/csrc/gemm_kernels.h b/vit-ed_amd/csrc/gemm_kernels.h
--- a/vit-ed_amd/csrc/gemm_kernels.h
+++ b/vit-ed_amd/csrc/gemm_kernels.h
@@ -22,7 +22,8 @@
 void gemm_tn_batch_layout(int count, const int64_t* M, const int64_t* N, const int64_t* K, int64_t* splits, int64_t* slab_stride,
                           int64_t* bias_stride);
 int gemm_tn_batch(int count, const void* const* dY, const int64_t* lddy, const void* const* X, const int64_t* ldx, const int64_t* M,
-                  const int64_t* N, const int64_t* K, const int* has_bias, float* slabs, float* bias_slabs, hipStream_t s);
+                  const int64_t* N, const int64_t* K, const int* has_bias, float* slabs, float* bias_slabs, float* const* dW,
+                  float* const* dbias, int accumulate, hipStream_t s);
 int sum_slabs_batch(int count, const float* slabs, int64_t slab_stride, const float* bias_slabs, int64_t bias_stride, int64_t splits,
                     const int64_t* widths, float* const* dW, const int64_t* nbias, float* const* dbias, int accumulate, hipStream_t s);
 
diff --git a/vit-ed_amd/csrc/gemm_mfma.hip b/vit-ed_amd/csrc/gemm_mfma.hip
--- a/vit-ed_amd/csrc/gemm_mfma.hip
+++ b/vit-ed_amd/csrc/gemm_mfma.hip
@@ -482,7 +482,7 @@
     int count, total_tiles;
 };
 
-template <bool BIAS>
+template <bool BIAS, int DIRECT = 0>
 __global__ void __launch_bounds__(512)
 gemm_tn_wide_kernel(const TwBatch batch, float* __restrict__ out_base, float* __restrict__ bias_base) {
     extern __shared__ __attribute__((aligned(16))) char smem[];
@@ -503,8 +503,8 @@
     const int64_t lddy = pr.lddy, ldx = pr.ldx, M = pr.M, N = pr.N, K = pr.K, rows_per_split = pr.rows_per_split;
     const int tiles_k = pr.tiles_k;
     const bool with_bias = BIAS && pr.has_bias;
-    float* __restrict__ out = out_base + pr.slab_off;
-    float* __restrict__ bias_out = bias_base + pr.bias_off;
+    float* __restrict__ out = DIRECT ? (float*)(uintptr_t)pr.slab_off : out_base + pr.slab_off;
+    float* __restrict__ bias_out = DIRECT ? (float*)(uintptr_t)pr.bias_off : bias_base + pr.bias_off;
     const int64_t n0 = (int64_t)(tile_id / tiles_k) * 128, kc0 = (int64_t)(tile_id % tiles_k) * 384;
     const int64_t mb = (int64_t)split * rows_per_split;
     int64_t me = mb + rows_per_split;
@@ -669,7 +669,16 @@
 #pragma unroll
         for (int j = 0; j < 6; ++j) {
             const int64_t k = kc0 + wc * 96 + j * 16 + fq * 4;
-            if (n < N) *(f32x4*)(o + n * K + k) = acc[i][j];
+            if constexpr (DIRECT) {
+                if (n < N) {
+                    f32x4 v = DIRECT == 2 ? *(const f32x4*)(o + n * K + k) : f32x4{0.f, 0.f, 0.f, 0.f};
+#pragma unroll
+                    for (int e = 0; e < 4; ++e) v[e] += acc[i][j][e];
+                    *(f32x4*)(o + n * K + k) = v;
+                }
+            } else {
+                if (n < N) *(f32x4*)(o + n * K + k) = acc[i][j];
+            }
         }
     }
     if constexpr (BIAS) {
@@ -681,7 +690,11 @@
                 v += __shfl_xor(v, 16);
                 v += __shfl_xor(v, 32);
                 const int64_t n = n0 + wr * 64 + i * 16 + fr;
-                if (fq == 0 && n < N) bo[n] = v;
+                if constexpr (DIRECT) {
+                    if (fq == 0 && n < N) bo[n] = (DIRECT == 2 ? bo[n] : 0.f) + v;
+                } else {
+                    if (fq == 0 && n < N) bo[n] = v;
+                }
             }
         }
     }
@@ -768,6 +781,24 @@
     return VITED_OK;
 }
 
+template <int DIRECT>
+static int launch_tn_wide_direct(const TwBatch& b, bool any_bias, hipStream_t s) {
+    constexpr int LDS = TW_STAGES * TW_STAGE_BYTES;
+    static std::once_flag once;
+    static hipError_t status = hipSuccess;
+    std::call_once(once, [&] {
+        status = hipFuncSetAttribute((const void*)gemm_tn_wide_kernel<true, DIRECT>, hipFuncAttributeMaxDynamicSharedMemorySize, LDS);
+        if (status == hipSuccess)
+            status = hipFuncSetAttribute((const void*)gemm_tn_wide_kernel<false, DIRECT>, hipFuncAttributeMaxDynamicSharedMemorySize, LDS);
+    });
+    if (status != hipSuccess) return VITED_ERR_LAUNCH;
+    if (any_bias)
+        hipLaunchKernelGGL((gemm_tn_wide_kernel<true, DIRECT>), dim3(b.total_tiles, 1), dim3(512), LDS, s, b, (float*)nullptr, (float*)nullptr);
+    else
+        hipLaunchKernelGGL((gemm_tn_wide_kernel<false, DIRECT>), dim3(b.total_tiles, 1), dim3(512), LDS, s, b, (float*)nullptr, (float*)nullptr);
+    return VITED_OK;
+}
+
 static int launch_tn_wide_batch(const TwBatch& b, int64_t splits, bool any_bias, float* out, float* bias_out, hipStream_t s) {
     constexpr int LDS = TW_STAGES * TW_STAGE_BYTES;
     static std::once_flag once;
@@ -831,10 +862,13 @@
 }
 
 int gemm_tn_batch(int count, const void* const* dY, const int64_t* lddy, const void* const* X, const int64_t* ldx, const int64_t* M,
-                  const int64_t* N, const int64_t* K, const int* has_bias, float* slabs, float* bias_slabs, hipStream_t s) {
+                  const int64_t* N, const int64_t* K, const int* has_bias, float* slabs, float* bias_slabs, float* const* dW,
+                  float* const* dbias, int accumulate, hipStream_t s) {
     TwBatch b = {};
     int64_t splits;
     gemm_tn_batch_layout(count, M, N, K, &splits, &b.slab_stride, &b.bias_stride);
+    const bool direct = dW != nullptr;
+    if (direct && (splits != 1 || !dbias)) return VITED_ERR_BAD_ARG;
     int tile = 0;
     int64_t woff = 0, boff = 0;
     bool any_bias = false;
@@ -845,6 +879,10 @@
         p.rows_per_split = ceil_div64(ceil_div64(M[i], splits), 32) * 32;
         p.N = (int)N[i]; p.K = (int)K[i]; p.tiles_k = (int)(K[i] / 384); p.tile0 = tile; p.has_bias = has_bias[i];
         p.slab_off = woff; p.bias_off = boff;
+        if (direct) {
+            if (!dW[i] || ((uintptr_t)dW[i] & 15) || (has_bias[i] && !dbias[i])) return VITED_ERR_BAD_ARG;
+            p.slab_off = (int64_t)(uintptr_t)dW[i]; p.bias_off = (int64_t)(uintptr_t)dbias[i];
+        }
         tile += (int)ceil_div64(N[i], 128) * p.tiles_k;
         woff += N[i] * K[i];
         boff += N[i];
@@ -852,7 +890,8 @@
     }
     b.count = count;
     b.total_tiles = tile;
-    const int rc = launch_tn_wide_batch(b, splits, any_bias, slabs, bias_slabs, s);
+    const int rc = !direct ? launch_tn_wide_batch(b, splits, any_bias, slabs, bias_slabs, s)
+                 : accumulate ? launch_tn_wide_direct<2>(b, any_bias, s) : launch_tn_wide_direct<1>(b, any_bias, s);
     return rc != VITED_OK ? rc : vited_check_launch();
 }
 
diff --git a/vit-ed_amd/csrc/gemm_row.hip b/vit-ed_amd/csrc/gemm_row.hip
--- a/vit-ed_amd/csrc/gemm_row.hip
+++ b/vit-ed_amd/csrc/gemm_row.hip
@@ -23,6 +23,7 @@
     float* partial;
     const float* row_scale;
     const float* lp_scale;
+    unsigned din_period;
 };
 
 template <int MT> struct RowCfg {
@@ -55,7 +56,7 @@
 template <int SC> struct RowFwdIn { f32x4 res[3]; float scale[SC]; };
 template <int SC> struct RowBwdIn { f32x4 x[3], din[3]; float mu, rs; float lps[SC]; };
 
-template <int MODE, int MT, bool SCALED>
+template <int MODE, int MT, bool SCALED, bool PERIODIC = false>
 __global__ void __launch_bounds__(512)
 gemm_row_kernel(const RowArgs a) {
     extern __shared__ __attribute__((aligned(16))) char smem[];
@@ -251,11 +252,18 @@
     auto load_bwd = [&](RowBwdIn<SCALED>& in, int64_t m) {
         const bool ok = m < a.M;
         if constexpr (SCALED) in.lps[0] = ok ? a.lp_scale[m] : 0.f;
+        bool has_in = ok && a.dx_in;
+        int64_t mi = m;
+        if constexpr (PERIODIC) {
+            const unsigned q = (unsigned)m / a.din_period;
+            has_in = has_in && q * a.din_period == (unsigned)m;
+            mi = q;
+        }
 #pragma unroll
         for (int j = 0; j < 3; ++j) {
             const int c = (j * 32 + hl) * 4;
             in.x[j] = ok ? ROW_LOAD((const f32x4*)(a.x + m * a.ldx + c)) : f32x4{0.f, 0.f, 0.f, 0.f};
-            in.din[j] = (ok && a.dx_in) ? ROW_LOAD((const f32x4*)(a.dx_in + m * a.ldxi + c)) : f32x4{0.f, 0.f, 0.f, 0.f};
+            in.din[j] = has_in ? ROW_LOAD((const f32x4*)(a.dx_in + mi * a.ldxi + c)) : f32x4{0.f, 0.f, 0.f, 0.f};
         }
         in.mu = ok ? a.mean_in[m] : 0.f;
         in.rs = ok ? a.rstd_in[m] : 0.f;
@@ -413,9 +421,9 @@
 
 extern "C" int vited_linear_layernorm_supported(int64_t M, int64_t N, int64_t K) { return row_shape_ok(M, N, K) ? 1 : 0; }
 
-template <int MODE, int MT, bool SCALED>
+template <int MODE, int MT, bool SCALED, bool PERIODIC = false>
 static int row_launch_scaled(const RowArgs& a, unsigned tiles, hipStream_t s) {
-    auto kernel = gemm_row_kernel<MODE, MT, SCALED>;
+    auto kernel = gemm_row_kernel<MODE, MT, SCALED, PERIODIC>;
     static std::once_flag once;
     static hipError_t status = hipSuccess;
     std::call_once(once, [&] { status = hipFuncSetAttribute((const void*)kernel, hipFuncAttributeMaxDynamicSharedMemorySize, RowCfg<MT>::LDS_BYTES); });
@@ -426,6 +434,10 @@
 
 template <int MODE, int MT>
 static int row_launch_mt(const RowArgs& a, unsigned tiles, hipStream_t s) {
+    if constexpr (MODE == ROW_MODE_BWD) {
+        if (a.din_period > 1)
+            return a.lp_scale ? row_launch_scaled<MODE, MT, true, true>(a, tiles, s) : row_launch_scaled<MODE, MT, false, true>(a, tiles, s);
+    }
     if (MODE == ROW_MODE_FWD ? a.row_scale != nullptr : a.lp_scale != nullptr) return row_launch_scaled<MODE, MT, true>(a, tiles, s);
     return row_launch_scaled<MODE, MT, false>(a, tiles, s);
 }
@@ -490,8 +502,9 @@
                                     const float* x, int64_t ldx, const float* gamma, const float* mean, const float* rstd,
                                     const float* dx_in, int64_t dx_in_ld, float* dx_out, int64_t dx_out_ld, void* dx_lp, int64_t dx_lp_ld,
                                     const float* lp_scale, float* dgamma, float* dbeta, int accumulate, int64_t M, int64_t N, int64_t K,
-                                    float* workspace, int64_t workspace_bytes, void* stream) {
+                                    float* workspace, int64_t workspace_bytes, void* stream, int64_t dx_in_period = 1) {
     if (lp_scale && !dx_lp) return VITED_ERR_BAD_ARG;
+    if (dx_in_period < 1 || dx_in_period > M || M % dx_in_period || (dx_in_period > 1 && !dx_in)) return VITED_ERR_BAD_ARG;
     if (!dy || !wt || !x || !gamma || !mean || !rstd || !dx_out || M <= 0 || N <= 0 || K <= 0) return VITED_ERR_BAD_ARG;
     if ((dgamma == nullptr) != (dbeta == nullptr)) return VITED_ERR_BAD_ARG;
     if (seg_k <= 0 || K % seg_k || lddy < seg_k || ldwt < K || ldx < N || dx_out_ld < N || (dx_in && dx_in_ld < N) || (dx_lp && dx_lp_ld < N))
@@ -506,6 +519,7 @@
     r.dx_in = dx_in; r.ldxi = dx_in_ld; r.dx = dx_out; r.lddx = dx_out_ld; r.dx_lp = (bf16*)dx_lp; r.ldlp = dx_lp_ld;
     r.partial = workspace;
     r.lp_scale = lp_scale;
+    r.din_period = (unsigned)dx_in_period;
     const int rc = row_launch<ROW_MODE_BWD>(r, (hipStream_t)stream);
     if (rc != VITED_OK || !dgamma) return rc;
     return ln_bwd_finish(workspace, (int)row_tiles(M), ROW_N, dgamma, dbeta, accumulate, (hipStream_t)stream);
@@ -539,3 +553,13 @@
     return linear_layernorm_bwd_impl(dy, lddy, K, 0, wt, ldwt, x, ldx, gamma, mean, rstd, dx_in, dx_in_ld, dx_out, dx_out_ld, dx_lp, dx_lp_ld,
                                      lp_scale, dgamma, dbeta, accumulate, M, N, K, workspace, workspace_bytes, stream);
 }
+
+extern "C" int vited_linear_layernorm_bwd_periodic(const void* dy, int64_t lddy, const void* wt, int64_t ldwt, const float* x, int64_t ldx,
+                                                   const float* gamma, const float* mean, const float* rstd, const float* dx_in,
+                                                   int64_t dx_in_ld, float* dx_out, int64_t dx_out_ld, void* dx_lp, int64_t dx_lp_ld,
+                                                   const float* lp_scale, float* dgamma, float* dbeta, int accumulate, int64_t M, int64_t N,
+                                                   int64_t K, float* workspace, int64_t workspace_bytes, void* stream,
+                                                   int64_t dx_in_period) {
+    return linear_layernorm_bwd_impl(dy, lddy, K, 0, wt, ldwt, x, ldx, gamma, mean, rstd, dx_in, dx_in_ld, dx_out, dx_out_ld, dx_lp, dx_lp_ld,
+                                     lp_scale, dgamma, dbeta, accumulate, M, N, K, workspace, workspace_bytes, stream, dx_in_period);
+}
diff --git a/vit-ed_amd/functions.py b/vit-ed_amd/functions.py
--- a/vit-ed_amd/functions.py
+++ b/vit-ed_amd/functions.py
@@ -330,15 +330,21 @@
     return y, (ops.layernorm_fwd(y, ln[0], ln[1], LN_EPS, rt.act_dtype) if ln is not None else None)
 
 
-def _linear_ln_bwd(rt, dy, h_saved, w, bias, x, gamma, beta, mean, rstd, dx_in=None, dx_out=None, want_lp=True, lp_scale=None):
+def _linear_ln_bwd(rt, dy, h_saved, w, bias, x, gamma, beta, mean, rstd, dx_in=None, dx_out=None, want_lp=True, lp_scale=None,
+                   dx_in_period=1):
     want_lp = want_lp and not rt.exact
     wt, layout = rt.weight_t(w)
-    if layout == B_NK and _row_kernel_ok(rt, dy.shape[0], wt.shape[0], dy.shape[1], dy.dtype, dy, x, dx_in, dx_out):
+    row_kernel = layout == B_NK and _row_kernel_ok(rt, dy.shape[0], wt.shape[0], dy.shape[1], dy.dtype, dy, x, dx_in, dx_out)
+    if dx_in_period != 1 and not row_kernel:
+        dense = torch.zeros((x.shape[0], dx_in.shape[1]), dtype=torch.float32, device=dx_in.device)
+        dense.view(-1, dx_in_period, dx_in.shape[1])[:, 0, :].copy_(dx_in)
+        dx_in, dx_in_period = dense, 1
+    if row_kernel:
         gg, gb = _gtarget(rt, gamma), _gtarget(rt, beta)
         direct = gg is not None and gb is not None
         dx, dx_lp, dg, db = ops.linear_layernorm_bwd(dy, wt, x, gamma, mean, rstd, dx_in=dx_in, dx_out=dx_out, want_lp=want_lp,
                                                      dgamma=gg if direct else None, dbeta=gb if direct else None, defer=rt.ln_queue,
-                                                     lp_scale=lp_scale)
+                                                     lp_scale=lp_scale, dx_in_period=dx_in_period)
         if direct:
             dg = db = None
     else:
@@ -482,19 +488,20 @@
     return x, patches, batch, rows
 
 
-def _patch_tokens_bwd(rt, dx, patches, S, with_cls, batch):
+def _patch_tokens_bwd(rt, dx, patches, S, with_cls, batch, dx_lp=None):
     rows = rt.n2 if with_cls else rt.n1
     dx3 = dx.view(batch, rows, rt.dim)
-    dpos_rows = ops.sum_rows(dx3.view(batch, rows * rt.dim)).view(rows, rt.dim)
-    dpos = torch.zeros_like(S.pos)
+    have_lp = dx_lp is not None and not rt.exact and dx_lp.dtype == rt.act_dtype and dx_lp.shape == dx.shape and dx_lp.is_contiguous()
+    dpos = torch.empty_like(S.pos)
     grads = dict(pos=dpos)
     if with_cls:
-        dpos[0] = dpos_rows
-        grads['cls'] = dpos_rows[0].clone().view_as(S.cls)
-        dtok = ops.slice_rows_cast(dx3, 1, rt.n1, rt.act_dtype)
+        ops.sum_rows(dx3.view(batch, rows * rt.dim), out=dpos.view(-1))
+        grads['cls'] = dpos[0, 0].view_as(S.cls)
+        dtok = ops.slice_rows_cast(dx_lp.view(batch, rows, rt.dim) if have_lp else dx3, 1, rt.n1, rt.act_dtype)
     else:
-        dpos[0, 1:] = dpos_rows
-        dtok = dx if rt.exact else ops.cast(dx, rt.act_dtype)
+        dpos[0, 0].zero_()
+        ops.sum_rows(dx3.view(batch, rows * rt.dim), out=dpos[0, 1:].reshape(-1))
+        dtok = dx if rt.exact else (dx_lp if have_lp else ops.cast(dx, rt.act_dtype))
     grads['pw'], grads['pb'] = _weight_grads(rt, dtok, patches, S.pw, S.pb)
     return grads
 
@@ -549,7 +556,7 @@
                 if rt.tap is not None:
                     rt.tap[f'enc.dx.{i}'] = dx.clone()
                 gblocks[i] = EncBlock(**ga, **gm)
-        gshared = EncShared(**_patch_tokens_bwd(rt, dx, ctx.patches, shared, with_cls=False, batch=batch))
+        gshared = EncShared(**_patch_tokens_bwd(rt, dx, ctx.patches, shared, with_cls=False, batch=batch, dx_lp=dx_lp))
         ctx.tape = ctx.patches = ctx.drop = None
         return (None, None, *_cam_only(rt, flatten_params(gshared, gblocks)))
 
@@ -586,9 +593,8 @@
     dqkv3 = dqkv.view(batch, n, 3 * d)
     ops.attention_bwd(qkv3[:, 0:1, 0:d], qkv3[:, :, d:2 * d], qkv3[:, :, 2 * d:3 * d], o0.view(batch, 1, d), do0.view(batch, 1, d),
                       lse0, rt.heads, rt.scale, dqkv3[:, 0:1, 0:d], dqkv3[:, :, d:2 * d], dqkv3[:, :, 2 * d:3 * d])
-    dres = torch.zeros((batch * n, d), dtype=torch.float32, device=dx.device)
-    dres.view(batch, n, d)[:, 0, :].copy_(dx)
-    dx, dx_lp, dg1, db1, dwqkv, dbqkv = _linear_ln_bwd(rt, dqkv, h1, P.wqkv, P.bqkv, x, P.g1, P.b1, m1, r1, dx_in=dres, lp_scale=lp_scale)
+    dx, dx_lp, dg1, db1, dwqkv, dbqkv = _linear_ln_bwd(rt, dqkv, h1, P.wqkv, P.bqkv, x, P.g1, P.b1, m1, r1, dx_in=dx.contiguous(),
+                                                       lp_scale=lp_scale, dx_in_period=n)
     return dx, dx_lp, dict(g1=dg1, b1=db1, wqkv=dwqkv, bqkv=dbqkv, wproj=dwproj, bproj=dbproj)
 
 
@@ -855,7 +861,7 @@
                 dctx, kv_grads = _context_kv_folded_bwd(rt, dkv_all, ctx.ctxf, ctx.fold[1], ctx.fold[2], blocks)
                 gblocks = [g._replace(**kv) for g, kv in zip(gblocks, kv_grads)]
                 ctx.fold = None
-        gshared = DecShared(**_patch_tokens_bwd(rt, dx, ctx.patches, shared, with_cls=True, batch=batch), gN=dgN, bN=dbN, wh=dwh, bh=dbh)
+        gshared = DecShared(**_patch_tokens_bwd(rt, dx, ctx.patches, shared, with_cls=True, batch=batch, dx_lp=dx_lp), gN=dgN, bN=dbN, wh=dwh, bh=dbh)
         dfeats = dctx.view(b1, rt.n1, d) if ctx.feats_needs_grad and dctx is not None else None
         ctx.tape = ctx.patches = ctx.ctxf = ctx.final = ctx.drop = ctx.seg = None
         return (None, dfeats, None, None, None, *_cam_only(rt, flatten_params(gshared, gblocks)))
diff --git a/vit-ed_amd/ops.py b/vit-ed_amd/ops.py
--- a/vit-ed_amd/ops.py
+++ b/vit-ed_amd/ops.py
@@ -279,10 +279,11 @@
 
 def slice_rows_cast(x: torch.Tensor, row_offset: int, rows: int, dtype: torch.dtype) -> torch.Tensor:
     _need_gpu(x)
-    assert x.dtype == torch.float32 and x.dim() == 3 and x.is_contiguous()
+    assert x.dim() == 3 and x.is_contiguous()
+    assert x.dtype == torch.float32 or (x.dtype == torch.bfloat16 and dtype == torch.bfloat16)
     b, r, d = x.shape
     out = torch.empty((b * rows, d), dtype=dtype, device=x.device)
-    _lib.call('vited_slice_rows_cast', _ptr(x), _ptr(out), _code(dtype), b, r, row_offset, rows, d, _stream())
+    _lib.call('vited_slice_rows_cast_from', _ptr(x), _code(x.dtype), _ptr(out), _code(dtype), b, r, row_offset, rows, d, _stream())
     return out
 
 
@@ -293,11 +294,13 @@
     _lib.call('vited_write_cls_row', _ptr(x), _ptr(cls), _ptr(pos), b, r, d, _stream())
 
 
-def sum_rows(x: torch.Tensor) -> torch.Tensor:
-    _need_gpu(x)
+def sum_rows(x: torch.Tensor, out: torch.Tensor | None = None) -> torch.Tensor:
+    _need_gpu(x, out)
     ld = _rows2d(x)
     b, w = x.shape
-    out = torch.empty(w, dtype=torch.float32, device=x.device)
+    if out is None:
+        out = torch.empty(w, dtype=torch.float32, device=x.device)
+    assert out.dtype == torch.float32 and out.numel() == w and out.is_contiguous()
     ws = _scratch(_lib.load().vited_sum_rows_workspace_bytes(b, w), x.device)
     _lib.call('vited_sum_rows', _ptr(x), _code(x.dtype), ld, _ptr(out), b, w, *ws, _stream())
     return out
@@ -477,7 +480,7 @@
 
 
 def linear_layernorm_bwd(dy, wt, x, gamma, mean, rstd, dx_in=None, dx_out=None, want_lp: bool = False, dgamma=None, dbeta=None,
-                         defer=None, lp_scale=None):
+                         defer=None, lp_scale=None, dx_in_period: int = 1):
     _need_gpu(dy, wt, x, gamma, mean, rstd, dx_in, dx_out, lp_scale)
     assert dy.dtype == wt.dtype == torch.bfloat16 and x.dtype == torch.float32
     segments = 1
@@ -516,7 +519,11 @@
                _rows2d(dx_out), _ptr(dx_lp), n)
     sum_args = (0 if defer is not None else _ptr(dgamma), 0 if defer is not None else _ptr(dbeta), int(accumulate))
     tail = dx_args + sum_args
-    if lp_scale is not None:
+    if dx_in_period != 1:
+        assert segments == 1 and dx_in is not None and m % dx_in_period == 0 and dx_in.shape == (m // dx_in_period, n)
+        _lib.call('vited_linear_layernorm_bwd_periodic', _ptr(dy), lddy, _ptr(wt), ldwt, *dx_args, _ptr(lp_scale), *sum_args, m, n, k, *ws,
+                  _stream(), int(dx_in_period))
+    elif lp_scale is not None:
         _lib.call('vited_linear_layernorm_bwd_scaled', _ptr(dy), lddy, _ptr(wt), ldwt, *dx_args, _ptr(lp_scale), *sum_args, m, n, k, *ws,
                   _stream())
     elif segments > 1:
```
